# MDFahimAnjum/AliasFree-Diffusion-Models-PyTorch

Measured on AMD Instinct MI355X. Metric: train_step_images_per_sec, higher is better.
Workload: dtype f32; 1 GPU; CIFAR-10 32x32x3 synthetic, UNet variant=3 (Config D), batch 256/GPU, T=1000, AdamW lr 3e-4, random-init weights (seed 42); global_batch=256, parallelism=dp1, hip_graph=True, launch_mode=lanes

## Files before the change

### aliasfree-diffusion-models-pytorch_amd/csrc/tok.hip

```cpp
#include "tok_common.h"
#include "tok_h2.h"
#include <algorithm>
#include <cstdint>
#include <mutex>
#include <set>

namespace afd {

template <int KB>
__device__ __forceinline__ f32x16 t_block(const float* __restrict__ Ws, int nb, int l31, int half, const TT<KB>& z, f32x16 acc) {
  constexpr int WS = 32 * KB + 4;
  const float* __restrict__ wr = Ws + (nb * 32 + l31) * WS + 4 * half;
#pragma unroll
  for (int j = 0; j < KB; ++j)
#pragma unroll
    for (int q = 0; q < 4; ++q) {
      const float4 a = *reinterpret_cast<const float4*>(wr + 32 * j + 8 * q);
      acc = __builtin_amdgcn_mfma_f32_32x32x2f32(a.x, z.b[j][4 * q + 0], acc, 0, 0, 0);
      acc = __builtin_amdgcn_mfma_f32_32x32x2f32(a.y, z.b[j][4 * q + 1], acc, 0, 0, 0);
      acc = __builtin_amdgcn_mfma_f32_32x32x2f32(a.z, z.b[j][4 * q + 2], acc, 0, 0, 0);
      acc = __builtin_amdgcn_mfma_f32_32x32x2f32(a.w, z.b[j][4 * q + 3], acc, 0, 0, 0);
    }
  return acc;
}

template <int K>
__device__ __forceinline__ void stage_w(float* __restrict__ Ws, const float* __restrict__ w, int rows, int ldw, int n0, int k0,
                                        bool transposed) {
  constexpr int WS = K + 4;
  if (!transposed) {
    for (int i = threadIdx.x; i < rows * K; i += 256) {
      const int n = i / K, k = i - n * K;
      Ws[n * WS + k] = w[(long)(n0 + n) * ldw + k0 + k];
    }
  } else {
    for (int i = threadIdx.x; i < rows * K; i += 256) {
      const int n = i / K, k = i - n * K;
      Ws[n * WS + k] = w[(long)(k0 + k) * ldw + n0 + n];
    }
  }
}

template <int C>
__global__ __launch_bounds__(256) void tok_head_fwd(const float* __restrict__ x, const float* __restrict__ gamma,
                                                    const float* __restrict__ beta, const float* __restrict__ w,
                                                    const float* __restrict__ bias, float* __restrict__ h_out,
                                                    float* __restrict__ stats_out, float* __restrict__ y, int B, int N, int P,
                                                    float eps, int n_per_wg) {
  constexpr int KB = C / 32, WS = C + 4;
  extern __shared__ __attribute__((aligned(16))) float smem[];
  float* Ws = smem;
  float* bsm = Ws + n_per_wg * WS;
  float* gs = bsm + n_per_wg;
  float* bes = gs + C;
  const int nbase = blockIdx.y * n_per_wg;
  stage_w<C>(Ws, w, n_per_wg, C, nbase, 0, false);
  for (int i = threadIdx.x; i < n_per_wg; i += 256) bsm[i] = bias ? bias[nbase + i] : 0.f;
  for (int i = threadIdx.x; i < C; i += 256) { gs[i] = gamma[i]; bes[i] = beta[i]; }
  __syncthreads();

  const int lane = threadIdx.x & 63, wv = threadIdx.x >> 6, half = lane >> 5, l31 = lane & 31;
  const unsigned total = (unsigned)B * (unsigned)P;
  const int ntile = (int)((total + 31u) / 32u);
  const int tstride = gridDim.x * 4;
  const bool lead = blockIdx.y == 0;
  const int nblk = n_per_wg / 32;

  TT<KB> xc, xn;
  Pix pc, pn;
  int t = blockIdx.x * 4 + wv;
  if (t < ntile) { pc = pix_of(t, l31, total, P); t_load(xc, x, tbase(pc, C, P, half), P, pc.live); }
  for (; t < ntile; t += tstride) {
    const int tn = t + tstride;
    if (tn < ntile) { pn = pix_of(tn, l31, total, P); t_load(xn, x, tbase(pn, C, P, half), P, pn.live); }
    TT<KB> h;
    float mean, rstd;
    t_ln_fwd<KB>(xc, gs, bes, half, eps, h, mean, rstd);
    if (lead) {
      if (h_out) t_store(h, h_out, tbase(pc, C, P, half), P, pc.live);
      if (stats_out && pc.live && half == 0) { stats_out[2 * pc.f] = mean; stats_out[2 * pc.f + 1] = rstd; }
    }
    const unsigned yb = tbase(pc, N, P, half);
    for (int nb = 0; nb < nblk; ++nb) {
      const f32x16 acc = t_block<KB>(Ws, nb, l31, half, h, zero16());
      if (pc.live) {
#pragma unroll
        for (int r = 0; r < 16; ++r) {
          const int nl = nb * 32 + tch(0, r) + 4 * half;
          y[yb + (unsigned)(nbase + nb * 32 + tch(0, r)) * (unsigned)P] = acc[r] + bsm[nl];
        }
      }
    }
    xc = xn; pc = pn;
  }
}

template <int C> struct Chain {
  static constexpr int KB = C / 32, WS = C + 4, SLOT = C * WS;
  static constexpr bool RELOAD = C > 64;
  static constexpr int NSLOT = RELOAD ? 2 : 3;
};

template <int C, bool TRAIN>
__global__ __launch_bounds__(256) void tok_tail_fwd(const float* __restrict__ att, const float* __restrict__ xres,
                                                    const float* __restrict__ wo, const float* __restrict__ bo,
                                                    const float* __restrict__ gamma, const float* __restrict__ beta,
                                                    const float* __restrict__ w1, const float* __restrict__ b1,
                                                    const float* __restrict__ w2, const float* __restrict__ b2,
                                                    float* __restrict__ a_out, float* __restrict__ stats_out,
                                                    float* __restrict__ f_out, float* __restrict__ u_out, float* __restrict__ g_out,
                                                    float* __restrict__ out, int B, int P, float eps) {
  using CH = Chain<C>;
  constexpr int KB = CH::KB;
  extern __shared__ __attribute__((aligned(16))) float smem[];
  float* s0 = smem;
  float* s1 = smem + CH::SLOT;
  float* s2 = CH::RELOAD ? s0 : smem + 2 * CH::SLOT;
  float* vec = smem + CH::NSLOT * CH::SLOT;
  stage_w<C>(s0, wo, C, C, 0, 0, false);
  stage_w<C>(s1, w1, C, C, 0, 0, false);
  if (!CH::RELOAD) stage_w<C>(s2, w2, C, C, 0, 0, false);
  for (int i = threadIdx.x; i < C; i += 256) {
    vec[i] = bo[i]; vec[C + i] = gamma[i]; vec[2 * C + i] = beta[i]; vec[3 * C + i] = b1[i]; vec[4 * C + i] = b2[i];
  }
  __syncthreads();

  const int lane = threadIdx.x & 63, wv = threadIdx.x >> 6, half = lane >> 5, l31 = lane & 31;
  const unsigned total = (unsigned)B * (unsigned)P;
  const int ntile = (int)((total + 31u) / 32u);
  const int tstride = gridDim.x * 4;
  const int t0 = blockIdx.x * 4;
  const int npass = t0 < ntile ? (ntile - t0 + tstride - 1) / tstride : 0;
  for (int pass = 0; pass < npass; ++pass) {
    const int t = t0 + wv + pass * tstride;
    const bool active = t < ntile;
    if (CH::RELOAD && pass > 0) { __syncthreads(); stage_w<C>(s0, wo, C, C, 0, 0, false); __syncthreads(); }
    Pix pc = pix_of(active ? t : 0, l31, total, P);
    pc.live = pc.live && active;
    const unsigned base = tbase(pc, C, P, half);
    TT<KB> a, z;
    if (active) {
      TT<KB> xr;
      t_load(z, att, base, P, pc.live);
      t_load(xr, xres, base, P, pc.live);
#pragma unroll
      for (int nb = 0; nb < KB; ++nb) {
        const f32x16 acc = t_block<KB>(s0, nb, l31, half, z, zero16());
#pragma unroll
        for (int r = 0; r < 16; ++r) a.b[nb][r] = acc[r] + vec[nb * 32 + tch(0, r) + 4 * half] + xr.b[nb][r];
      }
      float mean, rstd;
      t_ln_fwd<KB>(a, vec + C, vec + 2 * C, half, eps, z, mean, rstd);
      if (TRAIN) {
        t_store(a, a_out, base, P, pc.live);
        t_store(z, f_out, base, P, pc.live);
        if (pc.live && half == 0) { stats_out[2 * pc.f] = mean; stats_out[2 * pc.f + 1] = rstd; }
      }
    }
    if (CH::RELOAD) { __syncthreads(); stage_w<C>(s0, w2, C, C, 0, 0, false); }
    TT<KB> g;
    if (active) {
#pragma unroll
      for (int nb = 0; nb < KB; ++nb) {
        const f32x16 acc = t_block<KB>(s1, nb, l31, half, z, zero16());
#pragma unroll
        for (int r = 0; r < 16; ++r) {
          const float u = acc[r] + vec[3 * C + nb * 32 + tch(0, r) + 4 * half];
          if (TRAIN && pc.live) u_out[base + (unsigned)tch(nb, r) * (unsigned)P] = u;
          g.b[nb][r] = gelu_erf(u);
        }
      }
      if (TRAIN) t_store(g, g_out, base, P, pc.live);
    }
    if (CH::RELOAD) __syncthreads();
    if (active) {
#pragma unroll
      for (int nb = 0; nb < KB; ++nb) {
        const f32x16 acc = t_block<KB>(s2, nb, l31, half, g, zero16());
        if (pc.live) {
#pragma unroll
          for (int r = 0; r < 16; ++r)
            out[base + (unsigned)tch(nb, r) * (unsigned)P] = acc[r] + vec[4 * C + nb * 32 + tch(0, r) + 4 * half] + a.b[nb][r];
        }
      }
    }
  }
}

template <int C>
__global__ __launch_bounds__(256) void tok_tail_bwd(const float* __restrict__ dout, const float* __restrict__ u_in,
                                                    const float* __restrict__ a_in, const float* __restrict__ stats,
                                                    const float* __restrict__ gamma, const float* __restrict__ w2,
                                                    const float* __restrict__ w1, const float* __restrict__ wo,
                                                    float* __restrict__ du_out, float* __restrict__ df_out,
                                                    float* __restrict__ da_out, float* __restrict__ datt_out, int B, int P) {
  using CH = Chain<C>;
  constexpr int KB = CH::KB;
  extern __shared__ __attribute__((aligned(16))) float smem[];
  float* s0 = smem;
  float* s1 = smem + CH::SLOT;
  float* s2 = CH::RELOAD ? s0 : smem + 2 * CH::SLOT;
  float* gs = smem + CH::NSLOT * CH::SLOT;
  stage_w<C>(s0, w2, C, C, 0, 0, true);
  stage_w<C>(s1, w1, C, C, 0, 0, true);
  if (!CH::RELOAD) stage_w<C>(s2, wo, C, C, 0, 0, true);
  for (int i = threadIdx.x; i < C; i += 256) gs[i] = gamma[i];
  __syncthreads();

  const int lane = threadIdx.x & 63, wv = threadIdx.x >> 6, half = lane >> 5, l31 = lane & 31;
  const unsigned total = (unsigned)B * (unsigned)P;
  const int ntile = (int)((total + 31u) / 32u);
  const int tstride = gridDim.x * 4;
  const int t0 = blockIdx.x * 4;
  const int npass = t0 < ntile ? (ntile - t0 + tstride - 1) / tstride : 0;
  for (int pass = 0; pass < npass; ++pass) {
    const int t = t0 + wv + pass * tstride;
    const bool active = t < ntile;
    if (CH::RELOAD && pass > 0) { __syncthreads(); stage_w<C>(s0, w2, C, C, 0, 0, true); __syncthreads(); }
    Pix pc = pix_of(active ? t : 0, l31, total, P);
    pc.live = pc.live && active;
    const unsigned base = tbase(pc, C, P, half);
    TT<KB> dy, z;
    if (active) {
      TT<KB> uu;
      t_load(dy, dout, base, P, pc.live);
      t_load(uu, u_in, base, P, pc.live);
#pragma unroll
      for (int nb = 0; nb < KB; ++nb) {
        const f32x16 acc = t_block<KB>(s0, nb, l31, half, dy, zero16());
#pragma unroll
        for (int r = 0; r < 16; ++r) z.b[nb][r] = acc[r] * gelu_erf_grad(uu.b[nb][r]);
      }
      t_store(z, du_out, base, P, pc.live);
    }
    if (CH::RELOAD) { __syncthreads(); stage_w<C>(s0, wo, C, C, 0, 0, true); }
    if (active) {
      TT<KB> df, aa;
      t_load(aa, a_in, base, P, pc.live);
#pragma unroll
      for (int nb = 0; nb < KB; ++nb) df.b[nb] = t_block<KB>(s1, nb, l31, half, z, zero16());
      t_store(df, df_out, base, P, pc.live);
      const float mean = pc.live ? stats[2 * pc.f] : 0.f, rstd = pc.live ? stats[2 * pc.f + 1] : 0.f;
      t_ln_bwd<KB>(df, aa, gs, half, mean, rstd, dy);
      t_store(df, da_out, base, P, pc.live);
      z = df;
    }
    if (CH::RELOAD) __syncthreads();
    if (active) {
#pragma unroll
      for (int nb = 0; nb < KB; ++nb) {
        const f32x16 acc = t_block<KB>(s2, nb, l31, half, z, zero16());
        if (pc.live) {
#pragma unroll
          for (int r = 0; r < 16; ++r) datt_out[base + (unsigned)tch(nb, r) * (unsigned)P] = acc[r];
        }
      }
    }
  }
}

template <int C>
__global__ __launch_bounds__(256) void tok_head_bwd(const float* __restrict__ dqkv, const float* __restrict__ x,
                                                    const float* __restrict__ stats, const float* __restrict__ gamma,
                                                    const float* __restrict__ w_in, const float* __restrict__ dres,
                                                    float* __restrict__ dh_out, float* __restrict__ dx_out, int B, int P) {
  using CH = Chain<C>;
  constexpr int KB = CH::KB;
  extern __shared__ __attribute__((aligned(16))) float smem[];
  float* s0 = smem;
  float* s1 = smem + CH::SLOT;
  float* s2 = CH::RELOAD ? s0 : smem + 2 * CH::SLOT;
  float* gs = smem + CH::NSLOT * CH::SLOT;
  stage_w<C>(s0, w_in, C, C, 0, 0, true);
  stage_w<C>(s1, w_in, C, C, 0, C, true);
  if (!CH::RELOAD) stage_w<C>(s2, w_in, C, C, 0, 2 * C, true);
  for (int i = threadIdx.x; i < C; i += 256) gs[i] = gamma[i];
  __syncthreads();

  const int lane = threadIdx.x & 63, wv = threadIdx.x >> 6, half = lane >> 5, l31 = lane & 31;
  const unsigned total = (unsigned)B * (unsigned)P;
  const int ntile = (int)((total + 31u) / 32u);
  const int tstride = gridDim.x * 4;
  const int t0 = blockIdx.x * 4;
  const int npass = t0 < ntile ? (ntile - t0 + tstride - 1) / tstride : 0;
  for (int pass = 0; pass < npass; ++pass) {
    const int t = t0 + wv + pass * tstride;
    const bool active = t < ntile;
    if (CH::RELOAD && pass > 0) { __syncthreads(); stage_w<C>(s0, w_in, C, C, 0, 0, true); __syncthreads(); }
    Pix pc = pix_of(active ? t : 0, l31, total, P);
    pc.live = pc.live && active;
    const unsigned base = tbase(pc, C, P, half);
    const unsigned qb = tbase(pc, 3 * C, P, half);
    TT<KB> dh, z;
    if (active) {
      t_load(z, dqkv, qb, P, pc.live);
#pragma unroll
      for (int nb = 0; nb < KB; ++nb) dh.b[nb] = t_block<KB>(s0, nb, l31, half, z, zero16());
    }
    if (CH::RELOAD) { __syncthreads(); stage_w<C>(s0, w_in, C, C, 0, 2 * C, true); }
    if (active) {
      t_load(z, dqkv, qb + (unsigned)C * (unsigned)P, P, pc.live);
#pragma unroll
      for (int nb = 0; nb < KB; ++nb) dh.b[nb] = t_block<KB>(s1, nb, l31, half, z, dh.b[nb]);
    }
// ... 58 lines not shown
#pragma unroll
    for (int r = 0; r < 16; ++r) z.b[j][r] = X[(tch(j, r) + 4 * half) * 32 + l31];
}
__device__ __forceinline__ f32x16 b_load(const float* __restrict__ src, unsigned base, unsigned P, bool live) {
  f32x16 v;
#pragma unroll
  for (int r = 0; r < 16; ++r) v[r] = live ? src[base + (unsigned)tch(0, r) * P] : 0.f;
  return v;
}
__device__ __forceinline__ void b_store(const f32x16& v, float* __restrict__ dst, unsigned base, unsigned P, bool live) {
  if (!live) return;
#pragma unroll
  for (int r = 0; r < 16; ++r) dst[base + (unsigned)tch(0, r) * P] = v[r];
}
template <int KB>
__device__ __forceinline__ void t_ln_stats(const TT<KB>& x, float eps, float& mean, float& rstd) {
  constexpr float invC = 1.0f / (32 * KB);
  float s = 0.f;
#pragma unroll
  for (int j = 0; j < KB; ++j)
#pragma unroll
    for (int r = 0; r < 16; ++r) s += x.b[j][r];
  s += __shfl_xor(s, 32, 64);
  mean = s * invC;
  float q = 0.f;
#pragma unroll
  for (int j = 0; j < KB; ++j)
#pragma unroll
    for (int r = 0; r < 16; ++r) { const float d = x.b[j][r] - mean; q = fmaf(d, d, q); }
  q += __shfl_xor(q, 32, 64);
  rstd = 1.0f / sqrtf(q * invC + eps);
}
template <int KB>
__device__ __forceinline__ void t_ln_bwd_core(TT<KB>& dy, const TT<KB>& x, const float* __restrict__ gs, int half, float mean,
                                              float rstd, float& m1, float& m2) {
  constexpr float invC = 1.0f / (32 * KB);
  float s1 = 0.f, s2 = 0.f;
#pragma unroll
  for (int j = 0; j < KB; ++j)
#pragma unroll
    for (int r = 0; r < 16; ++r) {
      const float gv = gs[tch(j, r) + 4 * half] * dy.b[j][r];
      const float xh = (x.b[j][r] - mean) * rstd;
      dy.b[j][r] = gv;
      s1 += gv;
      s2 = fmaf(gv, xh, s2);
    }
  s1 += __shfl_xor(s1, 32, 64);
  s2 += __shfl_xor(s2, 32, 64);
  m1 = s1 * invC; m2 = s2 * invC;
#pragma unroll
  for (int j = 0; j < KB; ++j)
#pragma unroll
    for (int r = 0; r < 16; ++r) {
      const float xh = (x.b[j][r] - mean) * rstd;
      dy.b[j][r] = rstd * (dy.b[j][r] - m1 - xh * m2);
    }
}

template <int C> struct Wide {
  static constexpr int KB = C / 32, NS = C / 32, TPW = 4 / NS;
};

template <int C, int NBW>
__global__ __launch_bounds__(256) void tok_head_fwd_wide(const float* __restrict__ x, const float* __restrict__ gamma,
                                                         const float* __restrict__ beta, const float* __restrict__ w,
                                                         const float* __restrict__ bias, float* __restrict__ h_out,
                                                         float* __restrict__ stats_out, float* __restrict__ y, int B, int P,
                                                         float eps) {
  constexpr int KB = C / 32, N = 3 * C, NGRP = N / 32 / NBW;
  __shared__ float vec[5 * C];
  for (int i = threadIdx.x; i < C; i += 256) { vec[i] = gamma[i]; vec[C + i] = beta[i]; }
  for (int i = threadIdx.x; i < N; i += 256) vec[2 * C + i] = bias ? bias[i] : 0.f;
  const int lane = threadIdx.x & 63, wv = threadIdx.x >> 6, half = lane >> 5, l31 = lane & 31;
  const unsigned total = (unsigned)B * (unsigned)P;
  const int ntile = (int)((total + 31u) / 32u);
  const long gw = (long)blockIdx.x * 4 + wv;
  const int tile = (int)(gw / NGRP), nb0 = (int)(gw - (long)tile * NGRP) * NBW;
  const bool active = tile < ntile;
  Pix pc = pix_of(active ? tile : 0, l31, total, P);
  pc.live = pc.live && active;
  TT<KB> xt, h;
  WA<KB> wa, wb;
  t_load(xt, x, tbase(pc, C, P, half), P, pc.live);
  wa_load(wa, w, nb0 * 32, C, 0, l31, half);
  __syncthreads();
  float mean, rstd;
  t_ln_fwd<KB>(xt, vec, vec + C, half, eps, h, mean, rstd);
  if (nb0 == 0) {
    if (h_out) t_store(h, h_out, tbase(pc, C, P, half), P, pc.live);
    if (stats_out && pc.live && half == 0) { stats_out[2 * pc.f] = mean; stats_out[2 * pc.f + 1] = rstd; }
  }
  const unsigned yb = tbase(pc, N, P, half);
#pragma unroll
  for (int i = 0; i < NBW; ++i) {
    const int nb = nb0 + i;
    if (i + 1 < NBW) wa_load((i & 1) ? wa : wb, w, (nb + 1) * 32, C, 0, l31, half);
    f32x16 acc = wa_block<KB>((i & 1) ? wb : wa, h, zero16());
#pragma unroll
    for (int r = 0; r < 16; ++r) acc[r] += vec[2 * C + nb * 32 + tch(0, r) + 4 * half];
    b_store(acc, y, yb + (unsigned)(nb * 32) * (unsigned)P, P, pc.live);
  }
}

template <int C, bool TRAIN>
__global__ __launch_bounds__(256) void tok_tail_fwd_wide(const float* __restrict__ att, const float* __restrict__ xres,
                                                         const float* __restrict__ wo, const float* __restrict__ bo,
                                                         const float* __restrict__ gamma, const float* __restrict__ beta,
                                                         const float* __restrict__ w1, const float* __restrict__ b1,
                                                         const float* __restrict__ w2, const float* __restrict__ b2,
                                                         float* __restrict__ a_out, float* __restrict__ stats_out,
                                                         float* __restrict__ f_out, float* __restrict__ u_out,
                                                         float* __restrict__ g_out, float* __restrict__ out, int B, int P, float eps) {
  using WD = Wide<C>;
  constexpr int KB = WD::KB;
  __shared__ float X[WD::TPW][C * 32];
  __shared__ float vec[5 * C];
  for (int i = threadIdx.x; i < C; i += 256) {
    vec[i] = bo[i]; vec[C + i] = gamma[i]; vec[2 * C + i] = beta[i]; vec[3 * C + i] = b1[i]; vec[4 * C + i] = b2[i];
  }
  const int lane = threadIdx.x & 63, wv = threadIdx.x >> 6, half = lane >> 5, l31 = lane & 31;
  const int ts = wv / WD::NS, nbk = wv % WD::NS;
  const unsigned total = (unsigned)B * (unsigned)P;
  const int ntile = (int)((total + 31u) / 32u);
  const int tile = blockIdx.x * WD::TPW + ts;
  const bool active = tile < ntile;
  Pix pc = pix_of(active ? tile : 0, l31, total, P);
  pc.live = pc.live && active;
  const unsigned base = tbase(pc, C, P, half), bb = base + (unsigned)(nbk * 32) * (unsigned)P;
  const int cb = nbk * 32 + 4 * half;
  float* Xt = X[ts];
  TT<KB> z;
  WA<KB> wa, wb;
  t_load(z, att, base, P, pc.live);
  const f32x16 xr = b_load(xres, bb, P, pc.live);
  wa_load(wa, wo, nbk * 32, C, 0, l31, half);
  __syncthreads();
  f32x16 ab = wa_block<KB>(wa, z, zero16());
  wa_load(wb, w1, nbk * 32, C, 0, l31, half);
#pragma unroll
  for (int r = 0; r < 16; ++r) ab[r] += vec[cb + tch(0, r)] + xr[r];
  x_put(Xt, nbk, l31, half, ab);
  if (TRAIN) b_store(ab, a_out, bb, P, pc.live);
  __syncthreads();
  x_get<KB>(Xt, l31, half, z);
  float mean, rstd;
  t_ln_stats<KB>(z, eps, mean, rstd);
#pragma unroll
  for (int j = 0; j < KB; ++j)
#pragma unroll
    for (int r = 0; r < 16; ++r) {
      const int c = tch(j, r) + 4 * half;
      z.b[j][r] = (z.b[j][r] - mean) * rstd * vec[C + c] + vec[2 * C + c];
    }
  if (TRAIN) {
    f32x16 fb;
#pragma unroll
    for (int r = 0; r < 16; ++r) fb[r] = (ab[r] - mean) * rstd * vec[C + cb + tch(0, r)] + vec[2 * C + cb + tch(0, r)];
    b_store(fb, f_out, bb, P, pc.live);
    if (nbk == 0 && pc.live && half == 0) { stats_out[2 * pc.f] = mean; stats_out[2 * pc.f + 1] = rstd; }
  }
  __syncthreads();
  f32x16 gb = wa_block<KB>(wb, z, zero16());
  wa_load(wa, w2, nbk * 32, C, 0, l31, half);
#pragma unroll
  for (int r = 0; r < 16; ++r) gb[r] += vec[3 * C + cb + tch(0, r)];
  if (TRAIN) b_store(gb, u_out, bb, P, pc.live);
#pragma unroll
  for (int r = 0; r < 16; ++r) gb[r] = gelu_erf(gb[r]);
  if (TRAIN) b_store(gb, g_out, bb, P, pc.live);
  x_put(Xt, nbk, l31, half, gb);
  __syncthreads();
  x_get<KB>(Xt, l31, half, z);
  f32x16 ob = wa_block<KB>(wa, z, zero16());
#pragma unroll
  for (int r = 0; r < 16; ++r) ob[r] += vec[4 * C + cb + tch(0, r)] + ab[r];
  b_store(ob, out, bb, P, pc.live);
}

template <int C>
__global__ __launch_bounds__(256) void tok_tail_bwd_wide(const float* __restrict__ dout, const float* __restrict__ u_in,
                                                         const float* __restrict__ a_in, const float* __restrict__ stats,
                                                         const float* __restrict__ gamma, const float* __restrict__ w2,
                                                         const float* __restrict__ w1, const float* __restrict__ wo,
                                                         float* __restrict__ du_out, float* __restrict__ df_out,
                                                         float* __restrict__ da_out, float* __restrict__ datt_out, int B, int P) {
  using WD = Wide<C>;
  constexpr int KB = WD::KB;
  __shared__ float X[WD::TPW][C * 32];
  __shared__ float gs[C];
  for (int i = threadIdx.x; i < C; i += 256) gs[i] = gamma[i];
  const int lane = threadIdx.x & 63, wv = threadIdx.x >> 6, half = lane >> 5, l31 = lane & 31;
  const int ts = wv / WD::NS, nbk = wv % WD::NS;
  const unsigned total = (unsigned)B * (unsigned)P;
  const int ntile = (int)((total + 31u) / 32u);
  const int tile = blockIdx.x * WD::TPW + ts;
  const bool active = tile < ntile;
  Pix pc = pix_of(active ? tile : 0, l31, total, P);
  pc.live = pc.live && active;
  const unsigned base = tbase(pc, C, P, half), bb = base + (unsigned)(nbk * 32) * (unsigned)P;
  const int cb = nbk * 32 + 4 * half;
  float* Xt = X[ts];
  TT<KB> z, aa;
  WA<KB> wa, wb;
  t_load(z, dout, base, P, pc.live);
  const f32x16 ub = b_load(u_in, bb, P, pc.live);
  wa_load_t(wa, w2, nbk * 32, C, 0, l31, half);
  f32x16 dub = wa_block<KB>(wa, z, zero16());
  wa_load_t(wb, w1, nbk * 32, C, 0, l31, half);
#pragma unroll
  for (int r = 0; r < 16; ++r) dub[r] *= gelu_erf_grad(ub[r]);
  b_store(dub, du_out, bb, P, pc.live);
  x_put(Xt, nbk, l31, half, dub);
  __syncthreads();
  x_get<KB>(Xt, l31, half, z);
  const f32x16 dfb = wa_block<KB>(wb, z, zero16());
  wa_load_t(wa, wo, nbk * 32, C, 0, l31, half);
  b_store(dfb, df_out, bb, P, pc.live);
  t_load(aa, a_in, base, P, pc.live);
  __syncthreads();
  x_put(Xt, nbk, l31, half, dfb);
  __syncthreads();
  x_get<KB>(Xt, l31, half, z);
  const float mean = pc.live ? stats[2 * pc.f] : 0.f, rstd = pc.live ? stats[2 * pc.f + 1] : 0.f;
  float m1, m2;
  t_ln_bwd_core<KB>(z, aa, gs, half, mean, rstd, m1, m2);
  t_load(aa, dout, base, P, pc.live);
#pragma unroll
  for (int j = 0; j < KB; ++j)
#pragma unroll
    for (int r = 0; r < 16; ++r) z.b[j][r] += aa.b[j][r];
  {
    const f32x16 ab = b_load(a_in, bb, P, pc.live), dob = b_load(dout, bb, P, pc.live);
    f32x16 dab;
#pragma unroll
    for (int r = 0; r < 16; ++r) {
      const float xh = (ab[r] - mean) * rstd;
      dab[r] = rstd * (gs[cb + tch(0, r)] * dfb[r] - m1 - xh * m2) + dob[r];
    }
    b_store(dab, da_out, bb, P, pc.live);
  }
  const f32x16 db = wa_block<KB>(wa, z, zero16());
  b_store(db, datt_out, bb, P, pc.live);
}

template <int C>
__global__ __launch_bounds__(256) void tok_head_bwd_wide(const float* __restrict__ dqkv, const float* __restrict__ x,
                                                         const float* __restrict__ stats, const float* __restrict__ gamma,
                                                         const float* __restrict__ w_in, const float* __restrict__ dres,
                                                         float* __restrict__ dh_out, float* __restrict__ dx_out, int B, int P) {
  using WD = Wide<C>;
  constexpr int KB = WD::KB;
  __shared__ float X[WD::TPW][C * 32];
  __shared__ float gs[C];
  for (int i = threadIdx.x; i < C; i += 256) gs[i] = gamma[i];
  const int lane = threadIdx.x & 63, wv = threadIdx.x >> 6, half = lane >> 5, l31 = lane & 31;
  const int ts = wv / WD::NS, nbk = wv % WD::NS;
  const unsigned total = (unsigned)B * (unsigned)P;
  const int ntile = (int)((total + 31u) / 32u);
  const int tile = blockIdx.x * WD::TPW + ts;
  const bool active = tile < ntile;
  Pix pc = pix_of(active ? tile : 0, l31, total, P);
  pc.live = pc.live && active;
  const unsigned base = tbase(pc, C, P, half), bb = base + (unsigned)(nbk * 32) * (unsigned)P;
  const unsigned qb = tbase(pc, 3 * C, P, half);
  const int cb = nbk * 32 + 4 * half;
  float* Xt = X[ts];
  TT<KB> z;
  WA<KB> wa;
  f32x16 dhb = zero16();
#pragma unroll
  for (int sct = 0; sct < 3; ++sct) {
    t_load(z, dqkv, qb + (unsigned)(sct * C) * (unsigned)P, P, pc.live);
    wa_load_t(wa, w_in, nbk * 32, C, sct * C, l31, half);
    dhb = wa_block<KB>(wa, z, dhb);
  }
  if (dh_out) b_store(dhb, dh_out, bb, P, pc.live);
  x_put(Xt, nbk, l31, half, dhb);
  TT<KB> xx;
  t_load(xx, x, base, P, pc.live);
  __syncthreads();
  x_get<KB>(Xt, l31, half, z);
  const float mean = pc.live ? stats[2 * pc.f] : 0.f, rstd = pc.live ? stats[2 * pc.f + 1] : 0.f;
  float m1, m2;
  t_ln_bwd_core<KB>(z, xx, gs, half, mean, rstd, m1, m2);
  const f32x16 xb = b_load(x, bb, P, pc.live), rb = b_load(dres, bb, P, pc.live);
  f32x16 dxb;
#pragma unroll
  for (int r = 0; r < 16; ++r) {
    const float xh = (xb[r] - mean) * rstd;
    dxb[r] = rstd * (gs[cb + tch(0, r)] * dhb[r] - m1 - xh * m2) + rb[r];
  }
  b_store(dxb, dx_out, bb, P, pc.live);
}

static bool tok_ok(int C) { return C == 32 || C == 64 || C == 128; }
static size_t chain_lds(int C, int nvec) {
  const int nslot = C > 64 ? 2 : 3;
  return sizeof(float) * ((size_t)nslot * C * (C + 4) + (size_t)nvec * C);
}
template <class K> static int set_lds(K kern, size_t lds) { return lds_opt_in(kern, lds); }
static int g_tok_max_wg = 0;
static int g_tok_path = 0;
static bool use_h2(int C, long ntile, int kern) {
  if (C != 64 && C != 128) return false;
  if (g_tok_path >= 4) return true;
  if (g_tok_path != 0) return false;
  if (C == 64) return ntile >= 1024 || (kern == 2 && ntile >= 512);
  return kern != 1 && ntile >= 512;
}
static bool use_wide(int C, long ntile) {
  if (C != 64 && C != 128) return false;
  if (g_tok_max_wg > 0 || g_tok_path == 1) return false;
  if (g_tok_path == 2) return true;
  return C == 128 || ntile < 1024;
}
static unsigned chain_grid(int C, long ntile) {
  const long wg = (ntile + 3) / 4;
  const long cap = g_tok_max_wg > 0 ? g_tok_max_wg : (C > 64 ? 8192 : 1024);
  return (unsigned)std::min<long>(wg, cap);
}

}

using namespace afd;

extern "C" {

int afd_tok_supported(int C) { return tok_ok(C) ? 1 : 0; }
int afd_debug_tok_grid(int max_workgroups) { g_tok_max_wg = max_workgroups; return AFD_OK; }
int afd_debug_tok_path(int mode) {
  AFD_REQUIRE(mode >= 0 && mode <= 6, "afd_debug_tok_path: mode %d not in 0..6", mode);
  g_tok_path = mode;
  tok_h2_debug_tpw(mode == 5 ? 2 : (mode == 6 ? 4 : 0));
  return AFD_OK;
}

int afd_tok_head_fwd(const float* x, const float* gamma, const float* beta, const float* w, const float* bias, float* h_out,
                     float* stats_out, float* qkv, int B, int C, int P, float eps, afd_stream_t st) {
  AFD_REQUIRE(x && gamma && beta && w && qkv && B > 0 && P > 0, "afd_tok_head_fwd: NULL pointer or empty shape");
  AFD_REQUIRE(tok_ok(C), "afd_tok_head_fwd: C=%d not covered (32, 64, 128)", C);
  AFD_REQUIRE((long)B * P * 3 * C < (1L << 31), "afd_tok_head_fwd: tensor too large for 32-bit offsets");
  const int N = 3 * C;
  const long ntile = ((long)B * P + 31) / 32, wg_tiles = (ntile + 3) / 4;
  if (use_h2(C, ntile, 0)) return tok_h2_head_fwd(x, gamma, beta, w, bias, h_out, stats_out, qkv, B, C, P, eps, g_tok_max_wg, as_stream(st));
  if (use_wide(C, ntile) && aligned16(w) && (ntile <= 256 || g_tok_path == 2)) {
    const long waves = ntile * (N / 32);
    const dim3 wgrid((unsigned)((waves + 3) / 4));
    hipStream_t s = as_stream(st);
    if (C == 64) hipLaunchKernelGGL((tok_head_fwd_wide<64, 1>), wgrid, dim3(256), 0, s, x, gamma, beta, w, bias, h_out, stats_out, qkv, B, P, eps);
    else         hipLaunchKernelGGL((tok_head_fwd_wide<128, 1>), wgrid, dim3(256), 0, s, x, gamma, beta, w, bias, h_out, stats_out, qkv, B, P, eps);
    return check_launch("afd_tok_head_fwd");
  }
  int npw = 32;
  for (int cand : {N, 192, 128, 96, 64, 32}) {
    if (cand > N || N % cand != 0) continue;
    if (sizeof(float) * ((size_t)cand * (C + 5) + 2 * C) > 64 * 1024) continue;
    npw = cand;
    if (wg_tiles * (N / cand) >= 256) break;
  }
  const size_t lds = sizeof(float) * ((size_t)npw * (C + 5) + 2 * C);
  const dim3 grid((unsigned)std::min<long>(wg_tiles, g_tok_max_wg > 0 ? g_tok_max_wg : 1024), (unsigned)(N / npw));
  hipStream_t s = as_stream(st);
  switch (C) {
    case 32:  hipLaunchKernelGGL(tok_head_fwd<32>, grid, dim3(256), lds, s, x, gamma, beta, w, bias, h_out, stats_out, qkv, B, N, P, eps, npw); break;
    case 64:  hipLaunchKernelGGL(tok_head_fwd<64>, grid, dim3(256), lds, s, x, gamma, beta, w, bias, h_out, stats_out, qkv, B, N, P, eps, npw); break;
    default:  hipLaunchKernelGGL(tok_head_fwd<128>, grid, dim3(256), lds, s, x, gamma, beta, w, bias, h_out, stats_out, qkv, B, N, P, eps, npw); break;
  }
  return check_launch("afd_tok_head_fwd");
}

int afd_tok_tail_fwd(const float* att, const float* x, const float* wo, const float* bo, const float* gamma, const float* beta,
                     const float* w1, const float* b1, const float* w2, const float* b2, float* a_out, float* stats_out,
                     float* f_out, float* u_out, float* g_out, float* out, int B, int C, int P, float eps, afd_stream_t st) {
  AFD_REQUIRE(att && x && wo && bo && gamma && beta && w1 && b1 && w2 && b2 && out && B > 0 && P > 0,
              "afd_tok_tail_fwd: NULL pointer or empty shape");
  AFD_REQUIRE(tok_ok(C), "afd_tok_tail_fwd: C=%d not covered (32, 64, 128)", C);
  AFD_REQUIRE((long)B * P * C < (1L << 31), "afd_tok_tail_fwd: tensor too large for 32-bit offsets");
  const bool train = a_out != nullptr;
  AFD_REQUIRE(!train || (stats_out && f_out && u_out && g_out), "afd_tok_tail_fwd: a_out given but a saved-tensor pointer is NULL");
  const long ntile = ((long)B * P + 31) / 32;
  hipStream_t s = as_stream(st);
  if (use_h2(C, ntile, 1))
    return tok_h2_tail_fwd(att, x, wo, bo, gamma, beta, w1, b1, w2, b2, a_out, stats_out, f_out, u_out, g_out, out, B, C, P, eps, g_tok_max_wg, s);
  if (use_wide(C, ntile) && aligned16(wo) && aligned16(w1) && aligned16(w2)) {
    const dim3 wgrid((unsigned)((ntile + Wide<64>::TPW - 1) / Wide<64>::TPW)), wgrid128((unsigned)ntile);
#define AFD_TAILW(C_, T_, G_) hipLaunchKernelGGL((tok_tail_fwd_wide<C_, T_>), G_, dim3(256), 0, s, att, x, wo, bo, gamma, beta, w1, b1, w2, b2, \
                                                  a_out, stats_out, f_out, u_out, g_out, out, B, P, eps)
    if (C == 64) { if (train) AFD_TAILW(64, true, wgrid); else AFD_TAILW(64, false, wgrid); }
    else         { if (train) AFD_TAILW(128, true, wgrid128); else AFD_TAILW(128, false, wgrid128); }
#undef AFD_TAILW
    return check_launch("afd_tok_tail_fwd");
  }
  const size_t lds = chain_lds(C, 5);
  const dim3 grid(chain_grid(C, ntile));
#define AFD_TAIL(C_, T_) do { if (int rc = set_lds(tok_tail_fwd<C_, T_>, lds)) return rc; \
    hipLaunchKernelGGL((tok_tail_fwd<C_, T_>), grid, dim3(256), lds, s, att, x, wo, bo, gamma, beta, w1, b1, w2, b2, a_out, stats_out, \
                       f_out, u_out, g_out, out, B, P, eps); } while (0)
  switch (C) {
    case 32:  if (train) AFD_TAIL(32, true); else AFD_TAIL(32, false); break;
    case 64:  if (train) AFD_TAIL(64, true); else AFD_TAIL(64, false); break;
    default:  if (train) AFD_TAIL(128, true); else AFD_TAIL(128, false); break;
  }
#undef AFD_TAIL
  return check_launch("afd_tok_tail_fwd");
}

int afd_tok_tail_bwd(const float* d_out, const float* u, const float* a, const float* stats, const float* gamma, const float* w2,
                     const float* w1, const float* wo, float* du_out, float* df_out, float* da_out, float* datt_out, int B, int C,
                     int P, afd_stream_t st) {
  AFD_REQUIRE(d_out && u && a && stats && gamma && w2 && w1 && wo && du_out && df_out && da_out && datt_out && B > 0 && P > 0,
              "afd_tok_tail_bwd: NULL pointer or empty shape");
  AFD_REQUIRE(tok_ok(C), "afd_tok_tail_bwd: C=%d not covered (32, 64, 128)", C);
  AFD_REQUIRE((long)B * P * C < (1L << 31), "afd_tok_tail_bwd: tensor too large for 32-bit offsets");
  const long ntile = ((long)B * P + 31) / 32;
  hipStream_t s = as_stream(st);
  if (use_h2(C, ntile, 2)) return tok_h2_tail_bwd(d_out, u, a, stats, gamma, w2, w1, wo, du_out, df_out, da_out, datt_out, B, C, P, g_tok_max_wg, s);
  if (use_wide(C, ntile)) {
    if (C == 64) hipLaunchKernelGGL(tok_tail_bwd_wide<64>, dim3((unsigned)((ntile + 1) / 2)), dim3(256), 0, s, d_out, u, a, stats, gamma, w2, w1, wo, du_out, df_out, da_out, datt_out, B, P);
    else         hipLaunchKernelGGL(tok_tail_bwd_wide<128>, dim3((unsigned)ntile), dim3(256), 0, s, d_out, u, a, stats, gamma, w2, w1, wo, du_out, df_out, da_out, datt_out, B, P);
    return check_launch("afd_tok_tail_bwd");
  }
  const size_t lds = chain_lds(C, 1);
  const dim3 grid(chain_grid(C, ntile));
#define AFD_TB(C_) do { if (int rc = set_lds(tok_tail_bwd<C_>, lds)) return rc; \
    hipLaunchKernelGGL(tok_tail_bwd<C_>, grid, dim3(256), lds, s, d_out, u, a, stats, gamma, w2, w1, wo, du_out, df_out, da_out, datt_out, B, P); } while (0)
  switch (C) { case 32: AFD_TB(32); break; case 64: AFD_TB(64); break; default: AFD_TB(128); break; }
#undef AFD_TB
  return check_launch("afd_tok_tail_bwd");
}

int afd_tok_head_bwd(const float* dqkv, const float* x, const float* stats, const float* gamma, const float* w_in,
                     const float* d_res, float* dh_out, float* dx_out, int B, int C, int P, afd_stream_t st) {
  AFD_REQUIRE(dqkv && x && stats && gamma && w_in && d_res && dx_out && B > 0 && P > 0, "afd_tok_head_bwd: NULL pointer or empty shape");
  AFD_REQUIRE(tok_ok(C), "afd_tok_head_bwd: C=%d not covered (32, 64, 128)", C);
  AFD_REQUIRE((long)B * P * 3 * C < (1L << 31), "afd_tok_head_bwd: tensor too large for 32-bit offsets");
  const long ntile = ((long)B * P + 31) / 32;
  hipStream_t s = as_stream(st);
  if (use_h2(C, ntile, 3)) return tok_h2_head_bwd(dqkv, x, stats, gamma, w_in, d_res, dh_out, dx_out, B, C, P, g_tok_max_wg, s);
  if (use_wide(C, ntile)) {
    if (C == 64) hipLaunchKernelGGL(tok_head_bwd_wide<64>, dim3((unsigned)((ntile + 1) / 2)), dim3(256), 0, s, dqkv, x, stats, gamma, w_in, d_res, dh_out, dx_out, B, P);
    else         hipLaunchKernelGGL(tok_head_bwd_wide<128>, dim3((unsigned)ntile), dim3(256), 0, s, dqkv, x, stats, gamma, w_in, d_res, dh_out, dx_out, B, P);
    return check_launch("afd_tok_head_bwd");
  }
  const size_t lds = chain_lds(C, 1);
  const dim3 grid(chain_grid(C, ntile));
#define AFD_HB(C_) do { if (int rc = set_lds(tok_head_bwd<C_>, lds)) return rc; \
    hipLaunchKernelGGL(tok_head_bwd<C_>, grid, dim3(256), lds, s, dqkv, x, stats, gamma, w_in, d_res, dh_out, dx_out, B, P); } while (0)
  switch (C) { case 32: AFD_HB(32); break; case 64: AFD_HB(64); break; default: AFD_HB(128); break; }
#undef AFD_HB
  return check_launch("afd_tok_head_bwd");
}

}
```

### aliasfree-diffusion-models-pytorch_amd/csrc/tok_h2.h

```cpp
#pragma once
#include "common.h"

namespace afd {

int tok_h2_head_fwd(const float* x, const float* gamma, const float* beta, const float* w, const float* bias, float* h_out,
                    float* stats_out, float* qkv, int B, int C, int P, float eps, int max_wg, hipStream_t s);
int tok_h2_tail_fwd(const float* att, const float* x, const float* wo, const float* bo, const float* gamma, const float* beta,
                    const float* w1, const float* b1, const float* w2, const float* b2, float* a_out, float* stats_out,
                    float* f_out, float* u_out, float* g_out, float* out, int B, int C, int P, float eps, int max_wg, hipStream_t s);
int tok_h2_tail_bwd(const float* d_out, const float* u, const float* a, const float* stats, const float* gamma, const float* w2,
                    const float* w1, const float* wo, float* du_out, float* df_out, float* da_out, float* datt_out, int B, int C,
                    int P, int max_wg, hipStream_t s);
int tok_h2_head_bwd(const float* dqkv, const float* x, const float* stats, const float* gamma, const float* w_in,
                    const float* d_res, float* dh_out, float* dx_out, int B, int C, int P, int max_wg, hipStream_t s);
void tok_h2_debug_tpw(int tpw);

}
```

### aliasfree-diffusion-models-pytorch_amd/csrc/tok_h2.hip

```cpp
#include "tok_common.h"
#include "h2_common.h"
#include "tok_h2.h"
#include <algorithm>

namespace afd {

template <int NB>
__device__ __forceinline__ void h_load(TT<NB>& z, const float* __restrict__ src, unsigned base, int P) {
#pragma unroll
  for (int j = 0; j < NB; ++j)
#pragma unroll
    for (int r = 0; r < 16; ++r) z.b[j][r] = (src + (size_t)tch(j, r) * P)[base];
}
template <int NB>
__device__ __forceinline__ void h_store(const TT<NB>& z, float* __restrict__ dst, unsigned base, int P, bool live) {
  if (!live) return;
#pragma unroll
  for (int j = 0; j < NB; ++j)
#pragma unroll
    for (int r = 0; r < 16; ++r) (dst + (size_t)tch(j, r) * P)[base] = z.b[j][r];
}

template <int KB> struct HP { h8 a[2 * KB], b[2 * KB]; };

template <int KB>
__device__ __forceinline__ float hp_split(const TT<KB>& z, HP<KB>& p) {
  float m = 0.f;
#pragma unroll
  for (int j = 0; j < KB; ++j)
#pragma unroll
    for (int r = 0; r < 16; ++r) m = fmaxf(m, fabsf(z.b[j][r]));
  m = fmaxf(m, __shfl_xor(m, 32, 64));
  const float s = h2_scale_for(m);
#pragma unroll
  for (int k = 0; k < 2 * KB; ++k) {
    float x[8];
#pragma unroll
    for (int e = 0; e < 8; ++e) x[e] = z.b[k >> 1][8 * (k & 1) + e];
    h2_split8(x, s, p.a[k], p.b[k]);
  }
  return h2_inv_pow2(s);
}

template <int KB>
__device__ __forceinline__ f32x16 hp_block(const h8* __restrict__ img, int nb, int l31, int half, const HP<KB>& z) {
  constexpr int C = 32 * KB, NG = C / 8;
  const h8* __restrict__ w0 = img + half * C + nb * 32 + l31;
  const h8* __restrict__ w1 = w0 + NG * C;
  f32x16 acc = zero16();
#pragma unroll
  for (int k = 0; k < 2 * KB; ++k) {
    const h8 a1 = w0[2 * k * C], a2 = w1[2 * k * C];
    acc = __builtin_amdgcn_mfma_f32_32x32x16_f16(a2, z.a[k], acc, 0, 0, 0);
    acc = __builtin_amdgcn_mfma_f32_32x32x16_f16(a1, z.b[k], acc, 0, 0, 0);
    acc = __builtin_amdgcn_mfma_f32_32x32x16_f16(a1, z.a[k], acc, 0, 0, 0);
  }
  return acc;
}

template <int C> struct H2Lds {
  static constexpr int NG = C / 8, REC = 2 * NG * C;
  static constexpr bool RELOAD = C > 64;
  static constexpr int NSLOT = RELOAD ? 2 : 3;
  h8* img[3];
  float* winv[3];
  unsigned* rmax[3];
  float* vec;
  __device__ __forceinline__ void init(unsigned char* base) {
    h8* i0 = reinterpret_cast<h8*>(base);
    float* w0 = reinterpret_cast<float*>(i0 + NSLOT * REC);
    unsigned* r0 = reinterpret_cast<unsigned*>(w0 + NSLOT * C);
#pragma unroll
    for (int m = 0; m < 3; ++m) {
      const int s = m % NSLOT;
      img[m] = i0 + s * REC; winv[m] = w0 + s * C; rmax[m] = r0 + s * C;
    }
    vec = reinterpret_cast<float*>(r0 + NSLOT * C);
  }
  static size_t bytes(int nvec) { return (size_t)NSLOT * REC * 16 + (size_t)NSLOT * C * 8 + (size_t)nvec * C * 4; }
};

struct WSrc { const float* w; int ldw, n0, k0; };

template <int C, int NT> struct Stg {
  static constexpr int NG = C / 8, NR = C * NG / NT;
  float x[NR][8];
  static __device__ __forceinline__ void rec(int r, bool transposed, int& n, int& G) {
    const int i = (int)threadIdx.x + r * NT;
    if (transposed) { n = i % C; G = i / C; }
    else {
      const int lo = i & 63, hi = i >> 6;
      n = (hi % (C / 8)) * 8 + (lo & 7);
      G = (hi / (C / 8)) * 8 + (lo >> 3);
    }
  }
  __device__ __forceinline__ void load(const WSrc& q, bool transposed) {
#pragma unroll
    for (int r = 0; r < NR; ++r) {
      int n, G;
      rec(r, transposed, n, G);
      const int kb = 16 * (G >> 1) + 4 * (G & 1);
#pragma unroll
      for (int e = 0; e < 8; ++e) {
        const int k = kb + 8 * (e >> 2) + (e & 3);
        x[r][e] = transposed ? q.w[(long)(q.k0 + k) * q.ldw + q.n0 + n] : q.w[(long)(q.n0 + n) * q.ldw + q.k0 + k];
      }
    }
  }
  __device__ __forceinline__ void maxima(unsigned* __restrict__ rmax, bool transposed) const {
#pragma unroll
    for (int r = 0; r < NR; ++r) {
      int n, G;
      rec(r, transposed, n, G);
      float m = 0.f;
#pragma unroll
      for (int e = 0; e < 8; ++e) m = fmaxf(m, fabsf(x[r][e]));
      atomicMax(&rmax[n], __float_as_uint(m));
    }
  }
  __device__ __forceinline__ void store(h8* __restrict__ img, float* __restrict__ winv, const unsigned* __restrict__ rmax,
                                        bool transposed) const {
#pragma unroll
    for (int r = 0; r < NR; ++r) {
      int n, G;
      rec(r, transposed, n, G);
      const float sc = h2_scale_for(__uint_as_float(rmax[n]));
      h8 p0, p1;
      h2_split8(x[r], sc, p0, p1);
      img[G * C + n] = p0;
      img[(NG + G) * C + n] = p1;
      if (G == 0) winv[n] = h2_inv_pow2(sc);
    }
  }
};

template <int C, int NT, int M0, int CNT>
__device__ __forceinline__ void h2_stage(const H2Lds<C>& L, const WSrc* src, bool transposed) {
  Stg<C, NT> st[CNT];
#pragma unroll
  for (int i = 0; i < CNT; ++i) st[i].load(src[i], transposed);
#pragma unroll
  for (int i = 0; i < CNT; ++i)
    for (int c = threadIdx.x; c < C; c += NT) L.rmax[M0 + i][c] = 0u;
  __syncthreads();
#pragma unroll
  for (int i = 0; i < CNT; ++i) st[i].maxima(L.rmax[M0 + i], transposed);
  __syncthreads();
#pragma unroll
  for (int i = 0; i < CNT; ++i) st[i].store(L.img[M0 + i], L.winv[M0 + i], L.rmax[M0 + i], transposed);
  __builtin_amdgcn_sched_barrier(0);
}
template <int C, int NT>
__device__ __forceinline__ void h2_stage_first(const H2Lds<C>& L, const WSrc* src, bool transposed) {
  if (H2Lds<C>::RELOAD) h2_stage<C, NT, 0, 2>(L, src, transposed);
  else h2_stage<C, NT, 0, 3>(L, src, transposed);
}
template <int C, int NT, int M>
__device__ __forceinline__ void h2_stage_one(const H2Lds<C>& L, const WSrc* src, bool transposed) {
  h2_stage<C, NT, M, 1>(L, src + M, transposed);
}

struct Walk { int lane, wv, half, l31, ntile, tstride, t0, npass; unsigned total; };
template <int TPW> __device__ __forceinline__ Walk walk_of(int B, int P) {
  Walk k;
  k.lane = threadIdx.x & 63; k.wv = threadIdx.x >> 6; k.half = k.lane >> 5; k.l31 = k.lane & 31;
  k.total = (unsigned)B * (unsigned)P;
  k.ntile = (int)((k.total + 31u) / 32u);
  k.tstride = gridDim.x * TPW;
  k.t0 = blockIdx.x * TPW;
  k.npass = k.t0 < k.ntile ? (k.ntile - k.t0 + k.tstride - 1) / k.tstride : 0;
  return k;
}

extern __shared__ __attribute__((aligned(16))) unsigned char h2_smem[];

template <int C, int TPW>
__global__ __launch_bounds__(64 * TPW) void tok_h2_head_fwd_k(const float* __restrict__ x, const float* __restrict__ gamma,
                                                               const float* __restrict__ beta, const float* __restrict__ w,
                                                               const float* __restrict__ bias, float* __restrict__ h_out,
                                                               float* __restrict__ stats_out, float* __restrict__ y, int B, int P,
                                                               float eps) {
  using LD = H2Lds<C>;
  constexpr int KB = C / 32, NT = 64 * TPW;
  LD L;
  L.init(h2_smem);
  float* vec = L.vec;
  const Walk k = walk_of<TPW>(B, P);
  const int half = k.half, l31 = k.l31;
  const WSrc src[3] = {{w, C, 0, 0}, {w, C, C, 0}, {w, C, 2 * C, 0}};
  h2_stage_first<C, NT>(L, src, false);
  for (int i = threadIdx.x; i < C; i += NT) { vec[i] = gamma[i]; vec[C + i] = beta[i]; }
  for (int i = threadIdx.x; i < 3 * C; i += NT) vec[2 * C + i] = bias ? bias[i] : 0.f;
  __syncthreads();
  for (int pass = 0; pass < k.npass; ++pass) {
    const int t = k.t0 + k.wv + pass * k.tstride;
    const bool active = t < k.ntile;
    if (LD::RELOAD && pass > 0) { __syncthreads(); h2_stage_one<C, NT, 0>(L, src, false); __syncthreads(); }
    Pix pc = pix_of(active ? t : 0, l31, k.total, P);
    pc.live = pc.live && active;
    const unsigned yb = tbase(pc, 3 * C, P, half);
    HP<KB> hp;
    float is = 0.f;
    if (active) {
      const unsigned base = tbase(pc, C, P, half);
      TT<KB> xc, h;
      h_load(xc, x, base, P);
      float mean, rstd;
      t_ln_fwd<KB>(xc, vec, vec + C, half, eps, h, mean, rstd);
      if (h_out) h_store(h, h_out, base, P, pc.live);
      if (stats_out && pc.live && half == 0) { stats_out[2 * pc.f] = mean; stats_out[2 * pc.f + 1] = rstd; }
      is = hp_split<KB>(h, hp);
    }
#pragma unroll
    for (int sl = 0; sl < 3; ++sl) {
      if (LD::RELOAD && sl == 1) { __syncthreads(); h2_stage_one<C, NT, 2>(L, src, false); }
      if (LD::RELOAD && sl == 2) __syncthreads();
      if (active) {
#pragma unroll
        for (int nb = 0; nb < KB; ++nb) {
          const f32x16 acc = hp_block<KB>(L.img[sl], nb, l31, half, hp);
          if (pc.live) {
#pragma unroll
            for (int r = 0; r < 16; ++r) {
              const int c = nb * 32 + tch(0, r) + 4 * half;
              (y + (size_t)(sl * C + nb * 32 + tch(0, r)) * P)[yb] = acc[r] * is * L.winv[sl][c] + vec[2 * C + sl * C + c];
            }
          }
        }
      }
    }
  }
}

template <int C, int TPW, bool TRAIN>
__global__ __launch_bounds__(64 * TPW) void tok_h2_tail_fwd_k(const float* __restrict__ att, const float* __restrict__ xres,
                                                               const float* __restrict__ wo, const float* __restrict__ bo,
                                                               const float* __restrict__ gamma, const float* __restrict__ beta,
                                                               const float* __restrict__ w1, const float* __restrict__ b1,
                                                               const float* __restrict__ w2, const float* __restrict__ b2,
                                                               float* __restrict__ a_out, float* __restrict__ stats_out,
                                                               float* __restrict__ f_out, float* __restrict__ u_out,
                                                               float* __restrict__ g_out, float* __restrict__ out, int B, int P,
                                                               float eps) {
  using LD = H2Lds<C>;
  constexpr int KB = C / 32, NT = 64 * TPW;
  LD L;
  L.init(h2_smem);
  float* vec = L.vec;
  const Walk k = walk_of<TPW>(B, P);
  const int half = k.half, l31 = k.l31;
  const WSrc src[3] = {{wo, C, 0, 0}, {w1, C, 0, 0}, {w2, C, 0, 0}};
  h2_stage_first<C, NT>(L, src, false);
  for (int i = threadIdx.x; i < C; i += NT) {
    vec[i] = bo[i]; vec[C + i] = gamma[i]; vec[2 * C + i] = beta[i]; vec[3 * C + i] = b1[i]; vec[4 * C + i] = b2[i];
  }
  __syncthreads();
  for (int pass = 0; pass < k.npass; ++pass) {
    const int t = k.t0 + k.wv + pass * k.tstride;
    const bool active = t < k.ntile;
    if (LD::RELOAD && pass > 0) { __syncthreads(); h2_stage_one<C, NT, 0>(L, src, false); __syncthreads(); }
    Pix pc = pix_of(active ? t : 0, l31, k.total, P);
    pc.live = pc.live && active;
    const unsigned base = tbase(pc, C, P, half);
    TT<KB> a;
    HP<KB> hp;
    float is = 0.f;
    if (active) {
      TT<KB> z, xr;
      h_load(z, att, base, P);
      h_load(xr, xres, base, P);
      is = hp_split<KB>(z, hp);
#pragma unroll
      for (int nb = 0; nb < KB; ++nb) {
        const f32x16 acc = hp_block<KB>(L.img[0], nb, l31, half, hp);
#pragma unroll
        for (int r = 0; r < 16; ++r) {
          const int c = nb * 32 + tch(0, r) + 4 * half;
          a.b[nb][r] = acc[r] * is * L.winv[0][c] + vec[c] + xr.b[nb][r];
        }
      }
      float mean, rstd;
      t_ln_fwd<KB>(a, vec + C, vec + 2 * C, half, eps, z, mean, rstd);
      if (TRAIN) {
        h_store(a, a_out, base, P, pc.live);
        h_store(z, f_out, base, P, pc.live);
        if (pc.live && half == 0) { stats_out[2 * pc.f] = mean; stats_out[2 * pc.f + 1] = rstd; }
      }
      is = hp_split<KB>(z, hp);
    }
    if (LD::RELOAD) { __syncthreads(); h2_stage_one<C, NT, 2>(L, src, false); }
    if (active) {
      TT<KB> g;
#pragma unroll
      for (int nb = 0; nb < KB; ++nb) {
        const f32x16 acc = hp_block<KB>(L.img[1], nb, l31, half, hp);
        TT<1> ub;
#pragma unroll
        for (int r = 0; r < 16; ++r) {
          const int c = nb * 32 + tch(0, r) + 4 * half;
          ub.b[0][r] = acc[r] * is * L.winv[1][c] + vec[3 * C + c];
          g.b[nb][r] = gelu_erf(ub.b[0][r]);
        }
        if (TRAIN) h_store(ub, u_out + (size_t)(32 * nb) * P, base, P, pc.live);
      }
      if (TRAIN) h_store(g, g_out, base, P, pc.live);
      is = hp_split<KB>(g, hp);
    }
    if (LD::RELOAD) __syncthreads();
    if (active) {
#pragma unroll
      for (int nb = 0; nb < KB; ++nb) {
        TT<1> ar;
        if (TRAIN && KB > 2) h_load(ar, a_out + (size_t)(32 * nb) * P, base, P);
        else ar.b[0] = a.b[nb];
        const f32x16 acc = hp_block<KB>(L.img[2], nb, l31, half, hp);
        if (pc.live) {
#pragma unroll
          for (int r = 0; r < 16; ++r) {
            const int c = nb * 32 + tch(0, r) + 4 * half;
            (out + (size_t)tch(nb, r) * P)[base] = acc[r] * is * L.winv[2][c] + vec[4 * C + c] + ar.b[0][r];
          }
        }
      }
    }
  }
}

template <int C, int TPW>
__global__ __launch_bounds__(64 * TPW) void tok_h2_tail_bwd_k(const float* __restrict__ dout, const float* __restrict__ u_in,
                                                               const float* __restrict__ a_in, const float* __restrict__ stats,
                                                               const float* __restrict__ gamma, const float* __restrict__ w2,
                                                               const float* __restrict__ w1, const float* __restrict__ wo,
                                                               float* __restrict__ du_out, float* __restrict__ df_out,
                                                               float* __restrict__ da_out, float* __restrict__ datt_out, int B,
                                                               int P) {
  using LD = H2Lds<C>;
  constexpr int KB = C / 32, NT = 64 * TPW;
  LD L;
  L.init(h2_smem);
  float* gs = L.vec;
  const Walk k = walk_of<TPW>(B, P);
  const int half = k.half, l31 = k.l31;
  const WSrc src[3] = {{w2, C, 0, 0}, {w1, C, 0, 0}, {wo, C, 0, 0}};
  h2_stage_first<C, NT>(L, src, true);
  for (int i = threadIdx.x; i < C; i += NT) gs[i] = gamma[i];
  __syncthreads();
  for (int pass = 0; pass < k.npass; ++pass) {
    const int t = k.t0 + k.wv + pass * k.tstride;
    const bool active = t < k.ntile;
    if (LD::RELOAD && pass > 0) { __syncthreads(); h2_stage_one<C, NT, 0>(L, src, true); __syncthreads(); }
    Pix pc = pix_of(active ? t : 0, l31, k.total, P);
    pc.live = pc.live && active;
    const unsigned base = tbase(pc, C, P, half);
    HP<KB> hp;
    float is = 0.f;
    if (active) {
      TT<KB> z, uu;
      h_load(z, dout, base, P);
      h_load(uu, u_in, base, P);
      is = hp_split<KB>(z, hp);
#pragma unroll
      for (int nb = 0; nb < KB; ++nb) {
        const f32x16 acc = hp_block<KB>(L.img[0], nb, l31, half, hp);
#pragma unroll
        for (int r = 0; r < 16; ++r)
          z.b[nb][r] = acc[r] * is * L.winv[0][nb * 32 + tch(0, r) + 4 * half] * gelu_erf_grad(uu.b[nb][r]);
      }
      h_store(z, du_out, base, P, pc.live);
      is = hp_split<KB>(z, hp);
    }
    if (LD::RELOAD) { __syncthreads(); h2_stage_one<C, NT, 2>(L, src, true); }
    if (active) {
      TT<KB> df, aa, dd;
#pragma unroll
      for (int nb = 0; nb < KB; ++nb) {
        const f32x16 acc = hp_block<KB>(L.img[1], nb, l31, half, hp);
#pragma unroll
        for (int r = 0; r < 16; ++r) df.b[nb][r] = acc[r] * is * L.winv[1][nb * 32 + tch(0, r) + 4 * half];
      }
      h_store(df, df_out, base, P, pc.live);
      h_load(dd, dout, base, P);
      h_load(aa, a_in, base, P);
      const float mean = pc.live ? stats[2 * pc.f] : 0.f, rstd = pc.live ? stats[2 * pc.f + 1] : 0.f;
      t_ln_bwd<KB>(df, aa, gs, half, mean, rstd, dd);
      h_store(df, da_out, base, P, pc.live);
      is = hp_split<KB>(df, hp);
    }
    if (LD::RELOAD) __syncthreads();
    if (active) {
#pragma unroll
      for (int nb = 0; nb < KB; ++nb) {
        const f32x16 acc = hp_block<KB>(L.img[2], nb, l31, half, hp);
        if (pc.live) {
#pragma unroll
          for (int r = 0; r < 16; ++r)
            (datt_out + (size_t)tch(nb, r) * P)[base] = acc[r] * is * L.winv[2][nb * 32 + tch(0, r) + 4 * half];
        }
      }
    }
  }
}

template <int C, int TPW>
__global__ __launch_bounds__(64 * TPW) void tok_h2_head_bwd_k(const float* __restrict__ dqkv, const float* __restrict__ x,
                                                               const float* __restrict__ stats, const float* __restrict__ gamma,
                                                               const float* __restrict__ w_in, const float* __restrict__ dres,
                                                               float* __restrict__ dh_out, float* __restrict__ dx_out, int B,
                                                               int P) {
  using LD = H2Lds<C>;
  constexpr int KB = C / 32, NT = 64 * TPW;
  LD L;
  L.init(h2_smem);
  float* gs = L.vec;
  const Walk k = walk_of<TPW>(B, P);
  const int half = k.half, l31 = k.l31;
  const WSrc src[3] = {{w_in, C, 0, 0}, {w_in, C, 0, C}, {w_in, C, 0, 2 * C}};
  h2_stage_first<C, NT>(L, src, true);
  for (int i = threadIdx.x; i < C; i += NT) gs[i] = gamma[i];
  __syncthreads();
  for (int pass = 0; pass < k.npass; ++pass) {
    const int t = k.t0 + k.wv + pass * k.tstride;
    const bool active = t < k.ntile;
    if (LD::RELOAD && pass > 0) { __syncthreads(); h2_stage_one<C, NT, 0>(L, src, true); __syncthreads(); }
    Pix pc = pix_of(active ? t : 0, l31, k.total, P);
    pc.live = pc.live && active;
    const unsigned base = tbase(pc, C, P, half);
    const unsigned qb = tbase(pc, 3 * C, P, half);
    TT<KB> dh;
#pragma unroll
    for (int sl = 0; sl < 3; ++sl) {
      if (LD::RELOAD && sl == 1) { __syncthreads(); h2_stage_one<C, NT, 2>(L, src, true); }
      if (LD::RELOAD && sl == 2) __syncthreads();
      if (active) {
        TT<KB> z;
        HP<KB> hp;
        h_load(z, dqkv + (size_t)(sl * C) * P, qb, P);
        const float is = hp_split<KB>(z, hp);
#pragma unroll
        for (int nb = 0; nb < KB; ++nb) {
          const f32x16 acc = hp_block<KB>(L.img[sl], nb, l31, half, hp);
#pragma unroll
          for (int r = 0; r < 16; ++r) {
            const float v = acc[r] * is * L.winv[sl][nb * 32 + tch(0, r) + 4 * half];
            dh.b[nb][r] = sl == 0 ? v : dh.b[nb][r] + v;
          }
        }
      }
    }
    if (active) {
      if (dh_out) h_store(dh, dh_out, base, P, pc.live);
      TT<KB> xx, rr;
      h_load(xx, x, base, P);
      h_load(rr, dres, base, P);
      const float mean = pc.live ? stats[2 * pc.f] : 0.f, rstd = pc.live ? stats[2 * pc.f + 1] : 0.f;
      t_ln_bwd<KB>(dh, xx, gs, half, mean, rstd, rr);
      h_store(dh, dx_out, base, P, pc.live);
    }
  }
}

static int g_h2_tpw = 0;
void tok_h2_debug_tpw(int tpw) { g_h2_tpw = tpw; }
static int h2_tpw(long ntile) { (void)ntile; return g_h2_tpw ? g_h2_tpw : 4; }
static unsigned h2_grid(int C, long ntile, int tpw, int max_wg) {
  const long wg = (ntile + tpw - 1) / tpw;
  const long cap = max_wg > 0 ? max_wg : (C > 64 ? 256 : 768);
  return (unsigned)std::min<long>(wg, cap);
}

#define AFD_H2_LAUNCH(KERN, NVEC, ...)                                                                              \
  do {                                                                                                              \
    const size_t lds = H2Lds<KC>::bytes(NVEC);                                                                      \
    if (int rc = lds_opt_in(KERN, lds)) return rc;                                                                  \
    hipLaunchKernelGGL(KERN, dim3(h2_grid(KC, ntile, KT, max_wg)), dim3(64 * KT), lds, s, __VA_ARGS__);             \
  } while (0)
#define AFD_H2_SWITCH(BODY)                                                                                         \
  do {                                                                                                              \
    if (C == 64) { constexpr int KC = 64; if (tpw == 4) { constexpr int KT = 4; BODY; } else { constexpr int KT = 2; BODY; } } \
    else         { constexpr int KC = 128; constexpr int KT = 4; BODY; }                                             \
  } while (0)

int tok_h2_head_fwd(const float* x, const float* gamma, const float* beta, const float* w, const float* bias, float* h_out,
                    float* stats_out, float* qkv, int B, int C, int P, float eps, int max_wg, hipStream_t s) {
  const long ntile = ((long)B * P + 31) / 32;
  const int tpw = h2_tpw(ntile);
  AFD_H2_SWITCH(AFD_H2_LAUNCH((tok_h2_head_fwd_k<KC, KT>), 5, x, gamma, beta, w, bias, h_out, stats_out, qkv, B, P, eps));
  return check_launch("afd_tok_head_fwd");
}

int tok_h2_tail_fwd(const float* att, const float* x, const float* wo, const float* bo, const float* gamma, const float* beta,
                    const float* w1, const float* b1, const float* w2, const float* b2, float* a_out, float* stats_out,
                    float* f_out, float* u_out, float* g_out, float* out, int B, int C, int P, float eps, int max_wg, hipStream_t s) {
  const long ntile = ((long)B * P + 31) / 32;
  const int tpw = h2_tpw(ntile);
  if (a_out)
    AFD_H2_SWITCH(AFD_H2_LAUNCH((tok_h2_tail_fwd_k<KC, KT, true>), 5, att, x, wo, bo, gamma, beta, w1, b1, w2, b2, a_out, stats_out,
                                f_out, u_out, g_out, out, B, P, eps));
  else
    AFD_H2_SWITCH(AFD_H2_LAUNCH((tok_h2_tail_fwd_k<KC, KT, false>), 5, att, x, wo, bo, gamma, beta, w1, b1, w2, b2, a_out, stats_out,
                                f_out, u_out, g_out, out, B, P, eps));
  return check_launch("afd_tok_tail_fwd");
}

int tok_h2_tail_bwd(const float* d_out, const float* u, const float* a, const float* stats, const float* gamma, const float* w2,
                    const float* w1, const float* wo, float* du_out, float* df_out, float* da_out, float* datt_out, int B, int C,
                    int P, int max_wg, hipStream_t s) {
  const long ntile = ((long)B * P + 31) / 32;
  const int tpw = h2_tpw(ntile);
  AFD_H2_SWITCH(AFD_H2_LAUNCH((tok_h2_tail_bwd_k<KC, KT>), 1, d_out, u, a, stats, gamma, w2, w1, wo, du_out, df_out, da_out, datt_out,
                              B, P));
  return check_launch("afd_tok_tail_bwd");
}

int tok_h2_head_bwd(const float* dqkv, const float* x, const float* stats, const float* gamma, const float* w_in,
                    const float* d_res, float* dh_out, float* dx_out, int B, int C, int P, int max_wg, hipStream_t s) {
  const long ntile = ((long)B * P + 31) / 32;
  const int tpw = h2_tpw(ntile);
  AFD_H2_SWITCH(AFD_H2_LAUNCH((tok_h2_head_bwd_k<KC, KT>), 1, dqkv, x, stats, gamma, w_in, d_res, dh_out, dx_out, B, P));
  return check_launch("afd_tok_head_bwd");
}

#undef AFD_H2_SWITCH
#undef AFD_H2_LAUNCH

}
```

### aliasfree-diffusion-models-pytorch_amd/csrc/wino.hip

```cpp
#include <cstdlib>
#include "conv_forms.h"
#include "bf3_weights.h"
#include "h2_common.h"

namespace afd {

using f32x4 = __attribute__((ext_vector_type(4))) float;
using f32x2 = __attribute__((ext_vector_type(2))) float;

template <int S, int NT> struct WGeo {
  static constexpr int W = S, TPR = S / 2, TPI = TPR * TPR;
  static constexpr int TI = NT <= TPI ? 1 : NT / TPI;
  static constexpr int TROWS = NT <= TPI ? NT / TPR : TPR;
  static constexpr int GPI = NT <= TPI ? TPI / NT : 1;
  static constexpr int PXR = 2 * TROWS, Wp = S + 2, IMG = (PXR + 2) * Wp, RS = TI * IMG;
  static constexpr int RSP = RS + ((32 - RS % 64) + 64) % 64;
  static_assert(NT % TPR == 0 && (NT <= TPI ? TPI % NT == 0 : NT % TPI == 0), "tile group must be whole tile rows or whole images");
};

template <int OFF0, int OFF1>
__device__ __forceinline__ void lds_issue_pair(f32x2& a, f32x2& b, unsigned base) {
  asm volatile("ds_read_b64 %0, %2 offset:%3\n\tds_read_b64 %1, %2 offset:%4" : "=&v"(a), "=&v"(b) : "v"(base), "n"(OFF0), "n"(OFF1));
}
template <int N>
__device__ __forceinline__ void lds_wait(f32x2& a, f32x2& b) {
  asm volatile("s_waitcnt lgkmcnt(%2)" : "+v"(a), "+v"(b) : "n"(N));
}

__device__ __forceinline__ int kperm8(int k) { return 2 * (k & 3) + (k >> 2); }

__device__ __forceinline__ void wino_weights_block(const float* __restrict__ w, float* __restrict__ Uf, float* __restrict__ Ud,
                                                   int Cin, int Cout, int blk, int lane) {
  const int nci8 = Cin >> 3;
  if (blk >= nci8 * (Cout >> 3)) return;
  const int ci = (blk % nci8) * 8 + (lane & 7), co = (blk / nci8) * 8 + (lane >> 3);
  const float* p = w + ((long)co * Cin + ci) * 9;
  float g[9];
#pragma unroll
  for (int t = 0; t < 9; ++t) g[t] = p[t];
  float t[4][3], u[16];
#pragma unroll
  for (int c = 0; c < 3; ++c) {
    const float g0 = g[c], g1 = g[3 + c], g2 = g[6 + c];
    t[0][c] = g0;
    t[1][c] = 0.5f * (g0 + g1 + g2);
    t[2][c] = 0.5f * (g0 - g1 + g2);
    t[3][c] = g2;
  }
#pragma unroll
  for (int i = 0; i < 4; ++i) {
    const float a = t[i][0], b = t[i][1], c = t[i][2];
    u[4 * i + 0] = a;
    u[4 * i + 1] = 0.5f * (a + b + c);
    u[4 * i + 2] = 0.5f * (a - b + c);
    u[4 * i + 3] = c;
  }
  if (Uf) {
    float* o = Uf + ((long)(ci >> 3) * 16 * Cout + co) * 8 + kperm8(ci & 7);
    const long xs = (long)Cout * 8;
#pragma unroll
    for (int xi = 0; xi < 16; ++xi) o[xi * xs] = u[xi];
  }
  if (Ud) {
    float* o = Ud + ((long)(co >> 3) * 16 * Cin + ci) * 8 + kperm8(co & 7);
    const long xs = (long)Cin * 8;
#pragma unroll
    for (int i = 0; i < 4; ++i)
#pragma unroll
      for (int j = 0; j < 4; ++j) {
        const int pi = i == 0 ? 3 : (i == 3 ? 0 : i), pj = j == 0 ? 3 : (j == 3 ? 0 : j);
        o[(4 * i + j) * xs] = u[4 * pi + pj];
      }
  }
}

__global__ __launch_bounds__(256) void wino_weights(const float* __restrict__ w, float* __restrict__ Uf, float* __restrict__ Ud,
                                                    int Cin, int Cout) {
  wino_weights_block(w, Uf, Ud, Cin, Cout, blockIdx.x * 4 + (threadIdx.x >> 6), threadIdx.x & 63);
}


__global__ __launch_bounds__(256) void wino_weights_batched(const afd_wino_desc* __restrict__ descs, const int* __restrict__ wg_desc) {
  const afd_wino_desc d = descs[wg_desc[blockIdx.x]];
  const int blk = (blockIdx.x - d.first_wg) * 4 + (threadIdx.x >> 6), lane = threadIdx.x & 63;
  float* wf = (d.kinds & 1) ? nullptr : d.u_fwd; float* wd = (d.kinds & 2) ? nullptr : d.u_dgrad;
  if (wf || wd) wino_weights_block(d.w, wf, wd, d.Cin, d.Cout, blk, lane);
  void* bf = (d.kinds & 1) ? d.u_fwd : nullptr; void* bd = (d.kinds & 2) ? d.u_dgrad : nullptr;
  if (bf || bd) {
    if (d.kinds & 4) bf3_weights_block(d.w, static_cast<__bf16*>(bf), static_cast<__bf16*>(bd), d.Cin, d.Cout, blk, lane);
    else h2_weights_block(d.w, bf, bd, d.Cin, d.Cout, blk, lane);
  }
}
__global__ __launch_bounds__(256) void h2_wscale_batched(const afd_wino_desc* __restrict__ descs, const int* __restrict__ wg_desc) {
  const afd_wino_desc d = descs[wg_desc[blockIdx.x]];
  if (d.kinds & 4) return;
  void* bf = (d.kinds & 1) ? d.u_fwd : nullptr; void* bd = (d.kinds & 2) ? d.u_dgrad : nullptr;
  const int nw = 4 * ((d.Cin * d.Cout / 64 + 3) / 4);
  if (bf || bd) h2_wscale_rows(d.w, bf, bd, d.Cin, d.Cout, (blockIdx.x - d.first_wg) * 4 + (threadIdx.x >> 6), nw, threadIdx.x & 63);
}

template <int GEO, int BN, int NT>
__global__ __launch_bounds__(BN * NT / 8, BN * NT == 4096 ? 1 : 2) void conv_wino(const float* __restrict__ x, const float* __restrict__ U,
                                                    const float* __restrict__ bias, const float* __restrict__ res,
                                                    float* __restrict__ y, int B, int K, int N, int act, int items) {
  using G = WGeo<GEO, NT>;
  constexpr int KC = 8, SU = 10, NTH = BN * NT / 8;
  constexpr int W = G::W, H = G::W, HW = W * W, Wp = G::Wp, IMG = G::IMG, RS = G::RS, RSP = G::RSP;
  constexpr int NPOS = (RS + NTH - 1) / NTH;
  constexpr int NUV = 16 * BN * 2 / NTH;
  extern __shared__ __attribute__((aligned(16))) float smem[];
  constexpr int BUF = 16 * BN * SU + KC * RSP;
  float* Us = smem;
  float* Rs = Us + 16 * BN * SU;
  const int tid = threadIdx.x, lane = tid & 63, wv = tid >> 6;
  const int NB = N / BN;

  unsigned rsrc[NPOS]; unsigned rvalid = 0; unsigned usrc0 = 0;
  constexpr int XSTEP = NTH / (2 * BN);
  static_assert(NTH % (2 * BN) == 0 && XSTEP * NUV == 16, "U chunk must split into whole xi planes per pass");
  const int u_h = tid & 1, u_n = (tid >> 1) % BN, u_xi = tid / (2 * BN);
  const int udst0 = (((u_n >> 4) * 16 + u_xi) * 16 + (u_n & 15)) * SU + 4 * u_h;
  const long ustep = (long)XSTEP * N * 8;
  auto plan = [&](int w) {
    const int tg = w / NB, n0 = (w % NB) * BN;
    const int b0 = (G::TI == 1) ? tg / G::GPI : tg * G::TI;
    const int row0 = (G::TI == 1) ? (tg % G::GPI) * G::PXR : 0;
    rvalid = 0;
#pragma unroll
    for (int e = 0; e < NPOS; ++e) {
      const int pos = tid + NTH * e;
      bool ok = false; unsigned src = 0;
      if (pos < RS) {
        const int ti = pos / IMG, rem = pos % IMG;
        const int yy = row0 + rem / Wp - 1, xx = rem % Wp - 1, b = b0 + ti;
        ok = b < B && yy >= 0 && yy < H && xx >= 0 && xx < W;
        if (ok) src = (unsigned)(b * K) * (unsigned)HW + (unsigned)(yy * W + xx);
      }
      rsrc[e] = src; rvalid |= (ok ? 1u : 0u) << e;
    }
    usrc0 = (unsigned)((u_xi * N + n0 + u_n) * 8 + 4 * u_h);
  };
  const int wn = wv % (BN / 32), wt = wv / (BN / 32);
  const int li = lane & 15, lq = lane >> 4;
  const int tt = wt * 16 + li;
  const int poff = (tt / (G::TROWS * G::TPR)) * IMG + 2 * ((tt / G::TPR) % G::TROWS) * Wp + 2 * (tt % G::TPR);

  struct Regs { float r[NPOS][KC]; f32x4 u[NUV]; unsigned ok; };
  Regs S0, S1;
  auto fetch = [&](Regs& S, int c) {
    const float* __restrict__ xk = x + (long)c * KC * HW;
    const float* __restrict__ uk = U + (long)c * 16 * N * 8;
#pragma unroll
    for (int e = 0; e < NUV; ++e) S.u[e] = *reinterpret_cast<const f32x4*>(uk + e * ustep + usrc0);
#pragma unroll
    for (int e = 0; e < NPOS; ++e)
      if (tid + NTH * e < RS) {
#pragma unroll
        for (int kc = 0; kc < KC; ++kc) S.r[e][kc] = (xk + kc * HW)[rsrc[e]];
      }
    S.ok = rvalid;
  };
  auto commit = [&](const Regs& S, int stage) {
    float* Us = smem + stage * BUF;
    float* Rs = Us + 16 * BN * SU;
#pragma unroll
    for (int e = 0; e < NUV; ++e) {
      float2* d = reinterpret_cast<float2*>(Us + udst0 + e * (XSTEP * 16 * SU));
      d[0] = make_float2(S.u[e][0], S.u[e][1]);
      d[1] = make_float2(S.u[e][2], S.u[e][3]);
    }
#pragma unroll
    for (int e = 0; e < NPOS; ++e)
      if (tid + NTH * e < RS) {
        const bool ok = (S.ok >> e) & 1u;
#pragma unroll
        for (int kc = 0; kc < KC; ++kc) Rs[kc * RSP + tid + NTH * e] = ok ? S.r[e][kc] : 0.f;
      }
  };
  auto patch = [&](const float* Rs, int k, float (&v)[16]) {
    const float* r = Rs + k * RSP + poff;
    float d[4][4];
#pragma unroll
    for (int a = 0; a < 4; ++a) {
      const float2 lo = *reinterpret_cast<const float2*>(r + a * Wp);
      const float2 hi = *reinterpret_cast<const float2*>(r + a * Wp + 2);
      d[a][0] = lo.x; d[a][1] = lo.y; d[a][2] = hi.x; d[a][3] = hi.y;
    }
    float w[4][4];
#pragma unroll
    for (int j = 0; j < 4; ++j) {
      w[0][j] = d[0][j] - d[2][j];
      w[1][j] = d[1][j] + d[2][j];
      w[2][j] = d[2][j] - d[1][j];
      w[3][j] = d[1][j] - d[3][j];
    }
#pragma unroll
    for (int i = 0; i < 4; ++i) {
      v[4 * i + 0] = w[i][0] - w[i][2];
      v[4 * i + 1] = w[i][1] + w[i][2];
      v[4 * i + 2] = w[i][2] - w[i][1];
      v[4 * i + 3] = w[i][1] - w[i][3];
    }
  };
  const unsigned ap = (unsigned)(size_t)(Us + (wn * 2 * 256 + li) * SU + 2 * lq);
  const int o_ti = tt / (G::TROWS * G::TPR), o_ty = (tt / G::TPR) % G::TROWS, o_tx = tt % G::TPR;
  const int nchunks = K / KC;

  for (int w = blockIdx.x; w < items; w += gridDim.x) {
    plan(w);
    fetch(S0, 0);
    if (nchunks > 1) fetch(S1, 1);
    f32x4 acc[16][2];
#pragma unroll
    for (int xi = 0; xi < 16; ++xi)
#pragma unroll
      for (int h = 0; h < 2; ++h) acc[xi][h] = f32x4{0.f, 0.f, 0.f, 0.f};

    auto multiply = [&](int st) {
      const float* Rc = Rs + st * BUF;
      const unsigned apc = ap + (unsigned)(st * BUF * 4);
      f32x2 alo[2], ahi[2];
      lds_issue_pair<0, 256 * SU * 4>(alo[0], ahi[0], apc);
      float v0[16], v1[16];
      patch(Rc, lq, v0);
      patch(Rc, lq + 4, v1);
#pragma unroll
      for (int xi = 0; xi < 16; ++xi) {
        constexpr int STEP = 16 * SU * 4;
        f32x2& lo = alo[xi & 1]; f32x2& hi = ahi[xi & 1];
        if (xi < 15) {
          switch (xi) {
#define AFD_NEXT(X) case X: lds_issue_pair<(X + 1) * STEP, (X + 1) * STEP + 256 * SU * 4>(alo[(X + 1) & 1], ahi[(X + 1) & 1], apc); break;
            AFD_NEXT(0) AFD_NEXT(1) AFD_NEXT(2) AFD_NEXT(3) AFD_NEXT(4) AFD_NEXT(5) AFD_NEXT(6) AFD_NEXT(7)
            AFD_NEXT(8) AFD_NEXT(9) AFD_NEXT(10) AFD_NEXT(11) AFD_NEXT(12) AFD_NEXT(13) AFD_NEXT(14)
#undef AFD_NEXT
          }
          lds_wait<2>(lo, hi);
        } else {
          lds_wait<0>(lo, hi);
        }
        acc[xi][0] = __builtin_amdgcn_mfma_f32_16x16x4f32(lo[0], v0[xi], acc[xi][0], 0, 0, 0);
        acc[xi][1] = __builtin_amdgcn_mfma_f32_16x16x4f32(hi[0], v0[xi], acc[xi][1], 0, 0, 0);
        acc[xi][0] = __builtin_amdgcn_mfma_f32_16x16x4f32(lo[1], v1[xi], acc[xi][0], 0, 0, 0);
        acc[xi][1] = __builtin_amdgcn_mfma_f32_16x16x4f32(hi[1], v1[xi], acc[xi][1], 0, 0, 0);
      }
    };

    __syncthreads();
    commit(S0, 0);
    if (nchunks > 2) fetch(S0, 2);
    __syncthreads();
    for (int c = 0; c < nchunks; c += 2) {
      multiply(0);
      if (c + 1 < nchunks) {
        commit(S1, 1);
        if (c + 3 < nchunks) fetch(S1, c + 3);
        __syncthreads();
        multiply(1);
        if (c + 2 < nchunks) {
          commit(S0, 0);
          if (c + 4 < nchunks) fetch(S0, c + 4);
          __syncthreads();
        }
      }
    }

    const int tg = w / NB, n0 = (w % NB) * BN;
    const int ob = ((G::TI == 1) ? tg / G::GPI : tg * G::TI) + o_ti;
    const int row0 = (G::TI == 1) ? (tg % G::GPI) * G::PXR : 0;
    if (ob < B) {
      const int opix = (row0 + 2 * o_ty) * W + 2 * o_tx;
#pragma unroll
      for (int h = 0; h < 2; ++h)
#pragma unroll
        for (int r = 0; r < 4; ++r) {
          const int n = n0 + wn * 32 + 16 * h + 4 * lq + r;
          float tcol[4][2];
#pragma unroll
          for (int i = 0; i < 4; ++i) {
            const float m0 = acc[4 * i + 0][h][r], m1 = acc[4 * i + 1][h][r], m2 = acc[4 * i + 2][h][r], m3 = acc[4 * i + 3][h][r];
            tcol[i][0] = (m0 + m1) + m2;
            tcol[i][1] = (m1 - m2) - m3;
          }
          float y00 = (tcol[0][0] + tcol[1][0]) + tcol[2][0], y01 = (tcol[0][1] + tcol[1][1]) + tcol[2][1];
          float y10 = (tcol[1][0] - tcol[2][0]) - tcol[3][0], y11 = (tcol[1][1] - tcol[2][1]) - tcol[3][1];
          const unsigned idx = (unsigned)((ob * N + n) * HW + opix);
          if (bias) { const float bb = bias[n]; y00 += bb; y01 += bb; y10 += bb; y11 += bb; }
          if (act == 1) { y00 = gelu_erf(y00); y01 = gelu_erf(y01); y10 = gelu_erf(y10); y11 = gelu_erf(y11); }
          if (res) {
            const float2 r0 = *reinterpret_cast<const float2*>(res + idx), r1 = *reinterpret_cast<const float2*>(res + idx + W);
            y00 += r0.x; y01 += r0.y; y10 += r1.x; y11 += r1.y;
          }
          *reinterpret_cast<float2*>(y + idx) = make_float2(y00, y01);
          *reinterpret_cast<float2*>(y + idx + W) = make_float2(y10, y11);
        }
    }
  }
}

template <int S>
__global__ __launch_bounds__(256, 2) void conv_wino_sk(const float* __restrict__ x, const float* __restrict__ U,
                                                       const float* __restrict__ bias, const float* __restrict__ res,
                                                       float* __restrict__ y, int B, int K, int N, int act) {
  using G = WGeo<S, 16>;
  static_assert(G::GPI == 1, "tile groups must be whole images");
  constexpr int KC = 8, W = S, HW = S * S, Wp = G::Wp, IMG = G::IMG, RS = G::RS, RSP = G::RSP, TI = G::TI;
  constexpr int UPC = TI * S * (S / 4);
  static_assert(UPC == 16, "one chunk = 128 float4 pieces per wave");
  constexpr int DEPTH = 8;
  extern __shared__ __attribute__((aligned(16))) float smem[];
  const int lane = threadIdx.x & 63, wv = threadIdx.x >> 6;
  float* Rs = smem + wv * (KC * RSP);
  float* red = smem + 4 * KC * RSP;
  const int n0 = blockIdx.x * 32, tg = blockIdx.y, b0 = tg * TI;
  const int li = lane & 15, lq = lane >> 4;
  const int poff = (li / (G::TROWS * G::TPR)) * IMG + 2 * ((li / G::TPR) % G::TROWS) * Wp + 2 * (li % G::TPR);
  const int KS = K / 4, nchunks = KS / KC, kw = wv * KS;

  for (int i = lane; i < KC * RSP; i += 64) Rs[i] = 0.f;

  unsigned rsrc[2]; int rdst[2]; bool rok[2];
#pragma unroll
  for (int e = 0; e < 2; ++e) {
    const int u = lane + 64 * e, ch = u / UPC, q = u % UPC;
    const int ti = q / (S * (S / 4)), rr = (q / (S / 4)) % S, x4 = q % (S / 4);
    rok[e] = b0 + ti < B;
    rsrc[e] = rok[e] ? (unsigned)(((b0 + ti) * K + kw + ch) * HW + rr * W + 4 * x4) : 0u;
    rdst[e] = ch * RSP + ti * IMG + (rr + 1) * Wp + 1 + 4 * x4;
  }
  f32x4 rreg[2];
  auto fetch = [&](int c) {
    const float* xk = x + (long)c * KC * HW;
#pragma unroll
    for (int e = 0; e < 2; ++e) rreg[e] = *reinterpret_cast<const f32x4*>(xk + rsrc[e]);
  };
  auto commit = [&]() {
#pragma unroll
    for (int e = 0; e < 2; ++e) {
      float* d = Rs + rdst[e];
      const bool ok = rok[e];
      d[0] = ok ? rreg[e][0] : 0.f; d[1] = ok ? rreg[e][1] : 0.f; d[2] = ok ? rreg[e][2] : 0.f; d[3] = ok ? rreg[e][3] : 0.f;
    }
  };
  auto patch = [&](int k, float (&v)[16]) {
    const float* r = Rs + k * RSP + poff;
    float d[4][4];
#pragma unroll
    for (int a = 0; a < 4; ++a) {
      const float2 lo = *reinterpret_cast<const float2*>(r + a * Wp);
      const float2 hi = *reinterpret_cast<const float2*>(r + a * Wp + 2);
      d[a][0] = lo.x; d[a][1] = lo.y; d[a][2] = hi.x; d[a][3] = hi.y;
    }
    float w[4][4];
#pragma unroll
    for (int j = 0; j < 4; ++j) {
      w[0][j] = d[0][j] - d[2][j];
      w[1][j] = d[1][j] + d[2][j];
      w[2][j] = d[2][j] - d[1][j];
      w[3][j] = d[1][j] - d[3][j];
    }
#pragma unroll
    for (int i = 0; i < 4; ++i) {
      v[4 * i + 0] = w[i][0] - w[i][2];
      v[4 * i + 1] = w[i][1] + w[i][2];
      v[4 * i + 2] = w[i][2] - w[i][1];
      v[4 * i + 3] = w[i][1] - w[i][3];
    }
  };
  const float* ua = U + ((long)(kw / KC) * 16 * N + n0 + li) * 8 + 2 * lq;
  const long xstep = (long)N * 8;
  const int total = nchunks * 16;
  f32x2 abuf[DEPTH][2];
  auto aload = [&](int g, int slot) {
    const float* p = ua + (long)g * xstep;
    abuf[slot][0] = *reinterpret_cast<const f32x2*>(p);
    abuf[slot][1] = *reinterpret_cast<const f32x2*>(p + 128);
  };

  f32x4 acc[16][2];
#pragma unroll
  for (int xi = 0; xi < 16; ++xi)
#pragma unroll
    for (int h = 0; h < 2; ++h) acc[xi][h] = f32x4{0.f, 0.f, 0.f, 0.f};

#pragma unroll
  for (int g = 0; g < DEPTH; ++g) aload(g, g);
  fetch(0);
  for (int c = 0; c < nchunks; ++c) {
    commit();
    if (c + 1 < nchunks) fetch(c + 1);
    float v0[16], v1[16];
    patch(lq, v0);
    patch(lq + 4, v1);
#pragma unroll
    for (int xi = 0; xi < 16; ++xi) {
      const f32x2 lo = abuf[xi % DEPTH][0], hi = abuf[xi % DEPTH][1];
      const int gn = c * 16 + xi + DEPTH;
      if (gn < total) aload(gn, xi % DEPTH);
      __builtin_amdgcn_sched_barrier(0);
      acc[xi][0] = __builtin_amdgcn_mfma_f32_16x16x4f32(lo[0], v0[xi], acc[xi][0], 0, 0, 0);
// ... 371 lines not shown
```

### aliasfree-diffusion-models-pytorch_amd/ops.py

```python
import weakref

import numpy as np
import os
import torch

from ._lib import AfdError, lib

GN_EPS = 1e-5
LN_EPS = 1e-5
NULL_LABEL = -1


_raw_stream = getattr(torch._C, "_cuda_getCurrentRawStream", None)
_get_device = getattr(torch._C, "_cuda_getDevice", None) or torch.cuda.current_device


def _stream():
    if _raw_stream is not None:
        return _raw_stream(_get_device())
    return torch.cuda.current_stream().cuda_stream


def _chk(*tensors):
    for t in tensors:
# ... 116 lines not shown
    def backward(ctx, dy):
        (x,) = ctx.saved_tensors
        B, C, H, W = x.shape
        dy = _c(dy)
        dx = torch.empty_like(x)
        ws = _act_ws(B, C, H, W, ctx.tu.N, 1, x.device)
        lib().afd_filt_act_bwd(_p(x), _p(dy), _p(dx), B, C, H, W, None, None, None, None,
                               ctx.tu.ptr, ctx.td.ptr, ctx.tu.N, _p(ws), None, _stream())
        return dx, None, None


class _GradMode:
    inplace = False
    side = None
    sides = []
    turn = 0
    pending = []
    launched = []
    batch = 8
    on_write = None
    fold_hint = None
    folds = []
    fold_writes = []
    flushes = 0
    lane_of = {}
    fold_every = 2


def _wrote(*params):
    cb = _GradMode.on_write
    if cb is not None:
        cb([q for q in params if q is not None])


FOLD_DESC = "<QQqqqqii"


def fold_desc(part_ptr, dst_ptr, n, splits, stride=None, inner=None, rstride=1, accumulate=1):
    import struct
    return struct.pack(FOLD_DESC, part_ptr, dst_ptr, n, n if stride is None else stride, n if inner is None else inner, rstride,
                       splits, accumulate)


def fold_now(descs, stream=None):
    import ctypes
    buf = ctypes.create_string_buffer(descs, len(descs))
    lib().afd_fold_batched(ctypes.addressof(buf), len(descs) // 56, _stream() if stream is None else stream)


def defer_to_side_stream(fn, *keep, writes=()):
    _GradMode.pending.append((fn, keep, writes))
    if len(_GradMode.pending) >= _GradMode.batch:
        flush_wgrads()


FOLD_MAX = 56


def fold_batches(descs, limit=FOLD_MAX):
    assert len(descs) % 56 == 0 and limit > 0
    out, cur, seen = [], [], set()
    for o in range(0, len(descs), 56):
        d = descs[o:o + 56]
        dst = d[8:16]
        if dst in seen or len(cur) == limit:
            out.append(b"".join(cur))
            cur, seen = [], set()
        cur.append(d)
        seen.add(dst)
    if cur:
        out.append(b"".join(cur))
    return out


def deal_lane(keys, lane_of, turn, n_lanes):
    known = [lane_of[k] for k in keys if k in lane_of]
    lane = known[0] if known else turn % n_lanes
    conflict = any(l != lane for l in known)
    for k in keys:
        lane_of[k] = lane
    return lane, conflict


def _grad_keys(params):
    return [q.grad.data_ptr() for q in params if q is not None and q.grad is not None]


def _launch_folds():
    G = _GradMode
    for k, side in enumerate(G.sides):
        if G.folds[k]:
            for batch in fold_batches(b"".join(G.folds[k])):
                fold_now(batch, side.cuda_stream)
            G.folds[k] = []
    done = G.fold_writes
    G.fold_writes, G.flushes = [], 0
    return done


def _launch_lanes(lanes, done):
    G = _GradMode
    cur = torch.cuda.current_stream()
    for k, (side, items) in enumerate(zip(G.sides, lanes)):
        if not items:
            continue
        side.wait_stream(cur)
        with torch.cuda.stream(side):
            h = side.cuda_stream
            for fn, keep, ws in items:
                descs = fn(h) if fn is not None else keep[0]
                if descs and G.fold_every == 0:
                    for batch in fold_batches(descs):
                        fold_now(batch, h)
                    done.extend(ws)
                elif descs:
                    G.folds[k].append(descs)
                    G.fold_writes.extend(ws)
                else:
                    done.extend(ws)


def flush_wgrads(final=False):
    G = _GradMode
    sides, q = G.sides, G.pending
    if not q and not (final and any(G.folds)):
        return
    if len(G.folds) != len(sides):
        G.folds = [[] for _ in sides]
    done = []
    lanes = [[] for _ in sides]
    for item in q:
        lane, conflict = deal_lane(_grad_keys(item[2]), G.lane_of, G.turn, len(sides))
        G.turn += 1
        if conflict:
            _launch_lanes(lanes, done)
            done.extend(_launch_folds())
            lanes = [[] for _ in sides]
            for a in sides:
                for b in sides:
                    if a is not b:
                        a.wait_stream(b)
        lanes[lane].append(item)
    _launch_lanes(lanes, done)
    G.launched.extend(q)
    G.pending = []
    G.flushes += 1
    if any(G.folds) and (final or G.flushes >= max(1, G.fold_every) or (G.fold_hint is not None and G.fold_hint(G.fold_writes + done))):
        done.extend(_launch_folds())
    if G.on_write is not None and done:
        _wrote(*done)


class inplace_param_grads:

    def __init__(self, side_stream=None, batch=8, on_write=None, fold_hint=None, fold_every=None):
        self.side_stream, self.batch, self.on_write, self.fold_hint = side_stream, batch, on_write, fold_hint
        self.fold_every = int(os.environ.get("AFD_FOLD_EVERY", 2)) if fold_every is None else fold_every

    def __enter__(self):
        G = _GradMode
        self.prev = (G.inplace, G.side, G.sides, G.on_write, G.fold_hint, G.fold_every)
        ss = self.side_stream
        self.streams = [] if ss is None else (list(ss) if isinstance(ss, (list, tuple)) else [ss])
        G.inplace, G.batch, G.on_write, G.fold_hint, G.fold_every = True, self.batch, self.on_write, self.fold_hint, max(0, self.fold_every)
        G.sides, G.side, G.turn = self.streams, (self.streams[0] if self.streams else None), 0
        G.folds, G.fold_writes, G.flushes, G.lane_of = [[] for _ in self.streams], [], 0, {}

    def __exit__(self, exc_type, *a):
        G = _GradMode
        if self.streams:
            if exc_type is not None:
                G.pending, G.folds, G.fold_writes = [], [[] for _ in self.streams], []
            flush_wgrads(final=True)
            for st in self.streams:
                torch.cuda.current_stream().wait_stream(st)
            G.launched = []
        G.lane_of = {}
        G.inplace, G.side, G.sides, G.on_write, G.fold_hint, G.fold_every = self.prev


def _direct(*params):
    if not _GradMode.inplace:
        return False
    for q in params:
        if q is None:
            continue
        g = q.grad
        if g is None or not g.is_contiguous() or g.dtype != torch.float32:
            return False
    return True


def _gn_param_targets(C, gamma, beta, device):
    if gamma is not None and beta is not None and _direct(gamma, beta):
        return gamma.grad, beta.grad, 1, (None, None)
    out = torch.empty(2, C, device=device, dtype=torch.float32)
    return out[0], out[1], 0, (out[0], out[1])


class GroupNorm1(_Fn):

    @staticmethod
    def forward(ctx, x, gamma, beta, res, emb, act):
        _chk(x, gamma, beta, res, emb)
        x, res, emb = _c(x), _c(res), _c(emb)
        B, C, H, W = x.shape
        y = torch.empty_like(x)
        stats = torch.empty(B, 2, device=x.device, dtype=torch.float32)
        lib().afd_groupnorm1_fwd(_p(x), _p(y), _p(stats), B, C, H * W, GN_EPS, _p(gamma), _p(beta), _p(res), act,
                                 _p(emb), _stream())
        ctx.save_for_backward(x, gamma, beta, res, stats)
        ctx.act, ctx.has_emb = act, emb is not None
        return y

    @staticmethod
    def backward(ctx, dy):
        x, gamma, beta, res, stats = ctx.saved_tensors
        B, C, H, W = x.shape
        dy = _c(dy)
        dx = torch.empty_like(x)
        dres = None
        if res is not None:
            dres = dy if ctx.act == 0 else torch.empty_like(x)
        part = torch.empty(B * C * 2, device=x.device, dtype=torch.float32)
        demb = torch.empty(B, C, device=x.device, dtype=torch.float32) if ctx.has_emb else None
        dg, db, acc, (dgamma, dbeta) = _gn_param_targets(C, gamma, beta, x.device)
        defer = acc and _GradMode.side is not None
        lib().afd_groupnorm1_bwd(_p(x), _p(dy), _p(stats), B, C, H * W, _p(gamma), _p(beta), _p(res), ctx.act,
                                 _p(dx), _p(dres) if (res is not None and ctx.act == 1) else None, _p(part), _p(demb), 0,
                                 None if defer else _p(dg), None if defer else _p(db), acc, _stream())
        if defer:
            pp = _p(part)
            defer_to_side_stream(None, fold_desc(pp, _p(dg), C, B, stride=2 * C) + fold_desc(pp + 4 * C, _p(db), C, B, stride=2 * C),
                                 part, writes=(gamma, beta))
        elif acc:
            _wrote(gamma, beta)
        return dx, dgamma, dbeta, dres, demb, None


class GroupNormFiltAct(_Fn):

    @staticmethod
    def forward(ctx, x, gamma, beta, res, tu, td):
        _chk(x, gamma, beta, res)
        x, res = _c(x), _c(res)
        B, C, H, W = x.shape
        stats = torch.empty(B, 2, device=x.device, dtype=torch.float32)
        L = lib()
        y = torch.empty_like(x)
        if L.afd_filt_act_fwd_gn_supported(C, H, W, tu.N):
            L.afd_filt_act_fwd_gn(_p(x), _p(y), B, C, H, W, GN_EPS, _p(stats), _p(gamma), _p(beta), _p(res), tu.ptr, td.ptr, tu.N,
                                  _stream())
        else:
            L.afd_groupnorm1_fwd(_p(x), None, _p(stats), B, C, H * W, GN_EPS, None, None, None, 0, None, _stream())
            ws = _act_ws(B, C, H, W, tu.N, 0, x.device)
            L.afd_filt_act_fwd(_p(x), _p(y), B, C, H, W, _p(stats), _p(gamma), _p(beta), _p(res), tu.ptr, td.ptr, tu.N,
                               _p(ws), _stream())
        ctx.save_for_backward(x, gamma, beta, res, stats)
        ctx.tu, ctx.td = tu, td
        return y

    @staticmethod
    def backward(ctx, dy):
        x, gamma, beta, res, stats = ctx.saved_tensors
        B, C, H, W = x.shape
        dy = _c(dy)
        L = lib()
        if L.afd_filt_act_fwd_gn_supported(C, H, W, ctx.tu.N):
            dx = torch.empty_like(x)
            dres = torch.empty_like(x) if res is not None else None
            part = torch.empty(B * C * 2, device=x.device, dtype=torch.float32)
            L.afd_filt_act_bwd_gn(_p(x), _p(dy), _p(dx), _p(dres), B, C, H, W, _p(stats), _p(gamma), _p(beta), _p(res),
                                  ctx.tu.ptr, ctx.td.ptr, ctx.tu.N, _p(part), _stream())
            dg, db, acc, (dgamma, dbeta) = _gn_param_targets(C, gamma, beta, x.device)
            if acc and _GradMode.side is not None:
                pp = _p(part)
                defer_to_side_stream(None, fold_desc(pp, _p(dg), C, B, stride=2 * C) + fold_desc(pp + 4 * C, _p(db), C, B, stride=2 * C),
                                     part, writes=(gamma, beta))
            else:
                L.afd_colsum2(_p(part), _p(dg), _p(db), B, C, acc, _stream())
                if acc:
                    _wrote(gamma, beta)
            return dx, dgamma, dbeta, dres, None, None
        dv = torch.empty_like(x)
        ws = _act_ws(B, C, H, W, ctx.tu.N, 1, x.device)
        part = torch.empty(B * C * 2, device=x.device, dtype=torch.float32)
        fused = ws is None
        L.afd_filt_act_bwd(_p(x), _p(dy), _p(dv), B, C, H, W, _p(stats), _p(gamma), _p(beta), _p(res),
                           ctx.tu.ptr, ctx.td.ptr, ctx.tu.N, _p(ws), _p(part) if fused else None, _stream())
        dx = torch.empty_like(x)
        dg, db, acc, (dgamma, dbeta) = _gn_param_targets(C, gamma, beta, x.device)
        L.afd_groupnorm1_bwd(_p(x), _p(dv), _p(stats), B, C, H * W, _p(gamma), _p(beta), None, 0,
                             _p(dx), None, _p(part), None, 1 if fused else 0, _p(dg), _p(db), acc, _stream())
        if acc:
            _wrote(gamma, beta)
        return dx, dgamma, dbeta, (dv if res is not None else None), None, None


def _kind_of(kinds, dgrad):
    direct = kinds >> dgrad & 1
    return direct | (kinds & 4 if direct else 0)


class _WinoWeights:
    epoch = 0
    store = {}
    max_entries = 4096
    recording = None
    active_plan = None

    @classmethod
    def get(cls, w, nbytes, dgrad, kinds=0):
        plan = cls.active_plan
        if plan is not None:
            u = plan.lookup(w, nbytes, dgrad, kinds)
            if u is not None:
                return u, 1
        if cls.recording is not None:
            rec = cls.recording.setdefault(id(w), [w, 0, 0, 0])
            rec[1 + dgrad] = nbytes
            rec[3] = kinds
        capturing = torch.cuda.is_current_stream_capturing()
        key = (id(w), dgrad, _stream())
        stamp = (w._version, cls.epoch, w.data_ptr(), nbytes, _kind_of(kinds, dgrad))
        if not capturing:
            hit = cls.store.get(key)
            if hit is not None and hit[0]() is w and hit[2] == stamp:
                return hit[1], 1
        u = torch.empty(nbytes // 4, device=w.device, dtype=torch.float32)
        if not capturing:
            if len(cls.store) > cls.max_entries:
                cls.store.clear()
            try:
                cls.store[key] = (weakref.ref(w), u, stamp)
            except TypeError:
                pass
        return u, 0


class WinoStepPlan:

    def __init__(self, requests):
        import struct
        reqs = [r for r in requests.values() if r[1] or r[2]]
        self.ok = bool(reqs)
        if not self.ok:
            return
        dev = reqs[0][0].device
        self.buf = torch.empty(sum(r[1] + r[2] for r in reqs) // 4, device=dev, dtype=torch.float32)
        self.map, descs, wg, off = {}, b"", [], 0
        for i, (w, nf, nd, kinds) in enumerate(reqs):
            Cout, Cin = w.shape[0], w.shape[1]
            uf = self.buf[off:off + nf // 4] if nf else None
            off += nf // 4
            ud = self.buf[off:off + nd // 4] if nd else None
            off += nd // 4
            self.map[id(w)] = (weakref.ref(w), w.data_ptr(), uf, ud, kinds)
            n_wg = (Cin * Cout // 64 + 3) // 4
            descs += struct.pack("<QQQiiii", w.data_ptr(), uf.data_ptr() if nf else 0, ud.data_ptr() if nd else 0, Cin, Cout, len(wg), kinds)
            wg += [i] * n_wg
        self.n_wg = len(wg)
        self.descs = torch.frombuffer(bytearray(descs), dtype=torch.uint8).to(dev)
        self.wg = torch.tensor(wg, dtype=torch.int32).to(dev)

    def valid(self):
        return self.ok and all(r() is not None and r().data_ptr() == ptr for (r, ptr, _, _, _) in self.map.values())

    def launch(self):
        lib().afd_conv3x3_wino_weights_batched(_p(self.descs), _p(self.wg), self.n_wg, _stream())

    def lookup(self, w, nbytes, dgrad, kinds=0):
        e = self.map.get(id(w))
        if e is None or e[0]() is not w or _kind_of(e[4], dgrad) != _kind_of(kinds, dgrad):
            return None
        u = e[3] if dgrad else e[2]
        return u if (u is not None and u.numel() * 4 == nbytes) else None


def bump_param_epoch():
    _WinoWeights.epoch += 1
    if _WinoWeights.store:
        _WinoWeights.store.clear()


def _conv_fwd(x, w, bias, res, y, B, Cin, Cout, H, W, ks, act, want_dgrad=False):
    L = lib()
    nb = L.afd_conv3x3_wino_workspace_bytes(B, Cin, Cout, H, W, 0) if ks == 3 else 0
    nd = L.afd_conv3x3_wino_workspace_bytes(B, Cin, Cout, H, W, 1) if (ks == 3 and want_dgrad) else 0
    ud = None
    if nb:
        kinds = L.afd_conv3x3_weight_kinds(B, Cin, Cout, H, W)
        u, ready = _WinoWeights.get(w, nb, 0, kinds)
        if nd:
            ud, dready = _WinoWeights.get(w, nd, 1, kinds)
            if not (ready and dready):
                L.afd_conv3x3_wino_weights(_p(w), _p(u), _p(ud), Cin, Cout, kinds, _stream())
                ready = 1
        L.afd_conv3x3_wino_fwd(_p(x), _p(w), _p(bias), _p(res), _p(y), B, Cin, Cout, H, W, act, _p(u), ready, kinds, _stream())
    else:
        L.afd_conv_fwd(_p(x), _p(w), _p(bias), _p(res), _p(y), B, Cin, Cout, H, W, ks, act, _stream())
    return (ud, kinds) if ud is not None else None


class Conv(_Fn):

    @staticmethod
    def forward(ctx, x, w, bias, res, w_param=None, b_param=None, fork=False):
        _chk(x, w, bias, res)
        x, w, res = _c(x), _c(w), _c(res)
        B, Cin, H, W = x.shape
        Cout, ks = w.shape[0], w.shape[-1]
        y = torch.empty(B, Cout, H, W, device=x.device, dtype=torch.float32)
        ctx.u_dgrad = _conv_fwd(x, w, bias, res, y, B, Cin, Cout, H, W, ks, 0, want_dgrad=x.requires_grad)
        ctx.save_for_backward(x, w)
        ctx.has_bias, ctx.has_res = bias is not None, res is not None
        ctx.w_param, ctx.b_param = w_param, b_param
        return (y, x.view_as(x)) if fork else y

    @staticmethod
    def backward(ctx, dy, dfork=None):
        x, w = ctx.saved_tensors
        B, Cin, H, W = x.shape
        Cout, ks = w.shape[0], w.shape[-1]
        dy = _c(dy)
        L = lib()
        dx = dw = db = None
        if ctx.needs_input_grad[0]:
            dx = torch.empty_like(x)
            dfork = _c(dfork)
            nb = L.afd_conv3x3_wino_workspace_bytes(B, Cin, Cout, H, W, 1) if ks == 3 else 0
            if nb:
                if ctx.u_dgrad is not None:
                    (u, kinds), ready = ctx.u_dgrad, 1
                else:
                    kinds = L.afd_conv3x3_weight_kinds(B, Cin, Cout, H, W)
                    u, ready = _WinoWeights.get(w, nb, 1, kinds)
                L.afd_conv3x3_wino_dgrad(_p(dy), _p(w), _p(dx), _p(dfork), B, Cin, Cout, H, W, _p(u), ready, kinds, _stream())
            else:
                L.afd_conv_dgrad(_p(dy), _p(w), _p(dx), B, Cin, Cout, H, W, ks, _stream())
                if dfork is not None:
                    L.afd_add(_p(dx), _p(dfork), _p(dx), dx.numel(), _stream())
        if ctx.needs_input_grad[1] or (ctx.has_bias and ctx.needs_input_grad[2]):
            nbytes = L.afd_conv_wgrad_workspace_bytes(B, Cin, Cout, H, W, ks)
            ws = torch.empty(max(nbytes // 4, 1), device=x.device, dtype=torch.float32)
            wp, bp = ctx.w_param, ctx.b_param
            if wp is not None and (bp is not None or not ctx.has_bias) and _direct(wp, bp) and wp.grad.numel() == w.numel():
                side = _GradMode.side
                if side is None:
                    L.afd_conv_wgrad(_p(x), _p(dy), _p(wp.grad), _p(bp.grad) if bp is not None else None,
                                     B, Cin, Cout, H, W, ks, 1, _p(ws), _stream())
                    _wrote(wp, bp)
                else:
                    dwp, dbp = _p(wp.grad), (_p(bp.grad) if bp is not None else None)
                    defer_to_side_stream(lambda st, x=x, dy=dy, ws=ws: _wgrad_partials(x, dy, dwp, dbp, B, Cin, Cout, H, W, ks, ws, st),
                                         x, dy, ws, writes=(wp, bp))
            else:
                dw = torch.empty_like(w)
                db = torch.empty(Cout, device=x.device, dtype=torch.float32) if ctx.has_bias else None
                L.afd_conv_wgrad(_p(x), _p(dy), _p(dw), _p(db), B, Cin, Cout, H, W, ks, 0, _p(ws), _stream())
        return dx, dw, db, (dy if ctx.has_res else None), None, None, None


def conv(x, w, bias=None, res=None, w_param=None, b_param=None, fork=False):
    if w_param is None and isinstance(w, torch.nn.Parameter):
        w_param = w
    if b_param is None and isinstance(bias, torch.nn.Parameter):
        b_param = bias
    return Conv.apply(x, w, bias, res, w_param, b_param, fork)


def conv_infer(x, w, bias=None, res=None, act=0):
    _chk(x, w, bias, res)
    x, w, res = _c(x), _c(w), _c(res)
    B, Cin, H, W = x.shape
    Cout, ks = w.shape[0], w.shape[-1]
    y = torch.empty(B, Cout, H, W, device=x.device, dtype=torch.float32)
    _conv_fwd(x, w, bias, res, y, B, Cin, Cout, H, W, ks, act)
    return y


class LayerNormC(_Fn):

    @staticmethod
    def forward(ctx, x, gamma, beta):
        _chk(x, gamma, beta)
        x = _c(x)
        B, C, H, W = x.shape
        y = torch.empty_like(x)
        stats = torch.empty(B, H * W, 2, device=x.device, dtype=torch.float32)
        lib().afd_layernorm_c_fwd(_p(x), _p(y), _p(stats), B, C, H * W, LN_EPS, _p(gamma), _p(beta), _stream())
        ctx.save_for_backward(x, gamma, stats)
        ctx.beta_param = beta
        return y, x.view_as(x)

    @staticmethod
    def backward(ctx, dy, dres):
        x, gamma, stats = ctx.saved_tensors
        B, C, H, W = x.shape
        if dy is None:
            return dres, None, None
        dy, dres = _c(dy), _c(dres)
        dx = torch.empty_like(x)
        L = lib()
        if _direct(gamma, ctx.beta_param):
            L.afd_layernorm_c_bwd(_p(x), _p(dy), _p(stats), B, C, H * W, _p(gamma), _p(dx), _p(dres), None, None, None, 0, _stream())
            _ln_param_grads(x, dy, stats, gamma, ctx.beta_param, B, C, H * W)
            return dx, None, None
        part = torch.empty(B, 2, C, device=x.device, dtype=torch.float32)
        dg, db, acc, (dgamma, dbeta) = _gn_param_targets(C, gamma, ctx.beta_param, x.device)
        L.afd_layernorm_c_bwd(_p(x), _p(dy), _p(stats), B, C, H * W, _p(gamma), _p(dx), _p(dres), _p(part), _p(dg), _p(db), acc,
                              _stream())
        return dx, dgamma, dbeta


def layernorm_c(x, gamma, beta):
    return LayerNormC.apply(x, gamma, beta)[0]


class Attention(_Fn):

    @staticmethod
    def forward(ctx, qkv, heads):
        _chk(qkv)
        qkv = _c(qkv)
        B, C3, H, W = qkv.shape
        C, L = C3 // 3, H * W
        o = torch.empty(B, C, H, W, device=qkv.device, dtype=torch.float32)
        lse = torch.empty(B, heads, L, device=qkv.device, dtype=torch.float32)
        lib().afd_attn_fwd(_p(qkv), _p(o), _p(lse), B, heads, C // heads, L, _stream())
        ctx.save_for_backward(qkv, o, lse)
        ctx.heads = heads
        return o

    @staticmethod
    def backward(ctx, do):
        qkv, o, lse = ctx.saved_tensors
        B, C3, H, W = qkv.shape
        C, L = C3 // 3, H * W
        do = _c(do)
        dqkv = torch.empty_like(qkv)
        delta = torch.empty_like(lse)
        lib().afd_attn_bwd(_p(qkv), _p(o), _p(do), _p(lse), _p(dqkv), _p(delta), B, ctx.heads, C // ctx.heads, L, _stream())
        return dqkv, None


def tok_supported(C):
    return bool(lib().afd_tok_supported(int(C)))


def _wgrad_partials(x, dy, dwp, dbp, B, Cin, Cout, H, W, ks, ws, st):
    import ctypes
    buf = ctypes.create_string_buffer(112)
    n = ctypes.c_int(0)
    lib().afd_conv_wgrad_partials(_p(x), _p(dy), dwp, dbp, B, Cin, Cout, H, W, ks, 1, _p(ws), ctypes.addressof(buf), ctypes.addressof(n), st)
    return buf.raw[:56 * n.value]


def _linear_grads(x, dy, w, b, B, C_in, C_out, H, W, need_w=True):
    L = lib()
    nbytes = L.afd_conv_wgrad_workspace_bytes(B, C_in, C_out, H, W, 1)
    ws = torch.empty(max(nbytes // 4, 1), device=x.device, dtype=torch.float32)
    if _direct(w, b):
        dwp, dbp = _p(w.grad), (_p(b.grad) if b is not None else None)
        if _GradMode.side is not None:
            defer_to_side_stream(lambda st, x=x, dy=dy, ws=ws: _wgrad_partials(x, dy, dwp, dbp, B, C_in, C_out, H, W, 1, ws, st),
                                 x, dy, ws, writes=(w, b))
        else:
            L.afd_conv_wgrad(_p(x), _p(dy), dwp, dbp, B, C_in, C_out, H, W, 1, 1, _p(ws), _stream())
            _wrote(w, b)
        return None, None
    dw = torch.empty_like(w)
    db = torch.empty(C_out, device=x.device, dtype=torch.float32) if b is not None else None
    L.afd_conv_wgrad(_p(x), _p(dy), _p(dw), _p(db), B, C_in, C_out, H, W, 1, 0, _p(ws), _stream())
    return dw, db


def _ln_param_grads(x, dy, stats, gamma, beta, B, C, HW):
    L = lib()
    part = torch.empty(B, 2, C, device=x.device, dtype=torch.float32)
    dg, db, acc, (dgamma, dbeta) = _gn_param_targets(C, gamma, beta, x.device)
    pdg, pdb = _p(dg), _p(db)
    if acc and _GradMode.side is not None:
        def fn(st, x=x, dy=dy, stats=stats, part=part):
            L.afd_layernorm_c_bwd_partials(_p(x), _p(dy), _p(stats), B, C, HW, _p(part), st)
            pp = _p(part)
            return fold_desc(pp, pdg, C, B, stride=2 * C) + fold_desc(pp + 4 * C, pdb, C, B, stride=2 * C)
        defer_to_side_stream(fn, x, dy, stats, part, writes=(gamma, beta))
    else:
        L.afd_layernorm_c_bwd_params(_p(x), _p(dy), _p(stats), B, C, HW, _p(part), pdg, pdb, acc, _stream())
        if acc:
            _wrote(gamma, beta)
    return dgamma, dbeta


class AttnHead(_Fn):

    @staticmethod
    def forward(ctx, x, gamma, beta, w_in, b_in):
        _chk(x, gamma, beta, w_in, b_in)
        x = _c(x)
        B, C, H, W = x.shape
        train = not isinstance(ctx, _NoCtx)
        qkv = torch.empty(B, 3 * C, H, W, device=x.device, dtype=torch.float32)
        h = torch.empty_like(x) if train else None
        stats = torch.empty(B, H * W, 2, device=x.device, dtype=torch.float32) if train else None
        lib().afd_tok_head_fwd(_p(x), _p(gamma), _p(beta), _p(w_in), _p(b_in), _p(h), _p(stats), _p(qkv), B, C, H * W, LN_EPS, _stream())
        ctx.save_for_backward(x, h, stats, gamma, w_in)
        ctx.params = (beta, b_in)
        return qkv, x.view_as(x)

    @staticmethod
    def backward(ctx, dqkv, dres):
        x, h, stats, gamma, w_in = ctx.saved_tensors
        beta, b_in = ctx.params
        B, C, H, W = x.shape
        dqkv = _c(dqkv)
        if dres is None:
            dres = torch.zeros_like(x)
        dres = _c(dres)
        dx = torch.empty_like(x)
        dh = torch.empty_like(x)
        lib().afd_tok_head_bwd(_p(dqkv), _p(x), _p(stats), _p(gamma), _p(w_in), _p(dres), _p(dh), _p(dx), B, C, H * W, _stream())
        dw, db = _linear_grads(h, dqkv, w_in, b_in, B, C, 3 * C, H, W)
        dgamma, dbeta = _ln_param_grads(x, dh, stats, gamma, beta, B, C, H * W)
        return dx, dgamma, dbeta, dw, db


class AttnTail(_Fn):

    @staticmethod
    def forward(ctx, att, x, wo, bo, gamma, beta, w1, b1, w2, b2):
        _chk(att, x, wo, bo, gamma, beta, w1, b1, w2, b2)
        att, x = _c(att), _c(x)
        B, C, H, W = att.shape
        out = torch.empty_like(att)
        if not isinstance(ctx, _NoCtx):
            a, f, u, g = (torch.empty_like(att) for _ in range(4))
            stats = torch.empty(B, H * W, 2, device=att.device, dtype=torch.float32)
        else:
            a = f = u = g = stats = None
        lib().afd_tok_tail_fwd(_p(att), _p(x), _p(wo), _p(bo), _p(gamma), _p(beta), _p(w1), _p(b1), _p(w2), _p(b2),
                               _p(a), _p(stats), _p(f), _p(u), _p(g), _p(out), B, C, H * W, LN_EPS, _stream())
        ctx.save_for_backward(att, a, stats, f, u, g, gamma, wo, w1, w2)
        ctx.params = (bo, beta, b1, b2)
        return out

    @staticmethod
    def backward(ctx, dout):
        att, a, stats, f, u, g, gamma, wo, w1, w2 = ctx.saved_tensors
        bo, beta, b1, b2 = ctx.params
        B, C, H, W = att.shape
        dout = _c(dout)
        du, df, da, datt = (torch.empty_like(att) for _ in range(4))
        lib().afd_tok_tail_bwd(_p(dout), _p(u), _p(a), _p(stats), _p(gamma), _p(w2), _p(w1), _p(wo),
                               _p(du), _p(df), _p(da), _p(datt), B, C, H * W, _stream())
        dw2, db2 = _linear_grads(g, dout, w2, b2, B, C, C, H, W)
        dw1, db1 = _linear_grads(f, du, w1, b1, B, C, C, H, W)
        dwo, dbo = _linear_grads(att, da, wo, bo, B, C, C, H, W)
        dgamma, dbeta = _ln_param_grads(a, df, stats, gamma, beta, B, C, H * W)
        return datt, da, dwo, dbo, dgamma, dbeta, dw1, db1, dw2, db2


class Gelu(_Fn):
    @staticmethod
    def forward(ctx, x):
        _chk(x)
        x = _c(x)
        y = torch.empty_like(x)
        lib().afd_gelu_fwd(_p(x), _p(y), x.numel(), _stream())
        ctx.save_for_backward(x)
        return y

    @staticmethod
    def backward(ctx, dy):
        (x,) = ctx.saved_tensors
        dy = _c(dy)
        dx = torch.empty_like(x)
        lib().afd_gelu_bwd(_p(x), _p(dy), _p(dx), x.numel(), _stream())
        return dx


class MaxPool2(_Fn):
    @staticmethod
    def forward(ctx, x):
        _chk(x)
        x = _c(x)
        B, C, H, W = x.shape
        y = torch.empty(B, C, H // 2, W // 2, device=x.device, dtype=torch.float32)
        lib().afd_maxpool2_fwd(_p(x), _p(y), B, C, H, W, _stream())
        ctx.save_for_backward(x)
        return y

    @staticmethod
    def backward(ctx, dy):
        (x,) = ctx.saved_tensors
        B, C, H, W = x.shape
        dy = _c(dy)
        dx = torch.empty_like(x)
        lib().afd_maxpool2_bwd(_p(x), _p(dy), _p(dx), B, C, H, W, _stream())
        return dx


class UpCat(_Fn):

    @staticmethod
    def forward(ctx, x, skip, taps, mode):
        _chk(x, skip)
        x, skip = _c(x), _c(skip)
        B, C, H, W = x.shape
        Cs = skip.shape[1]
        assert skip.shape[2] == 2 * H and skip.shape[3] == 2 * W
        plane = 4 * H * W
        out = torch.empty(B, Cs + C, 2 * H, 2 * W, device=x.device, dtype=torch.float32)
        L = lib()
        up_ptr = out.data_ptr() + 4 * Cs * plane
        bs = (Cs + C) * plane
        if mode == "filt":
            L.afd_filt_up2_fwd(_p(x), up_ptr, B, C, H, W, 0, bs, taps.ptr, taps.N, _stream())
        else:
            L.afd_bilinear_up2_fwd(_p(x), up_ptr, B, C, H, W, bs, _stream())
        L.afd_copy_batched(_p(skip), _p(out), B, Cs * plane, 0, bs, _stream())
        ctx.taps, ctx.mode, ctx.dims = taps, mode, (B, C, Cs, H, W)
        return out

    @staticmethod
    def backward(ctx, dout):
        B, C, Cs, H, W = ctx.dims
        dout = _c(dout)
        plane = 4 * H * W
        bs = (Cs + C) * plane
        L = lib()
        dx = torch.empty(B, C, H, W, device=dout.device, dtype=torch.float32)
        up_ptr = dout.data_ptr() + 4 * Cs * plane
        if ctx.mode == "filt":
            L.afd_filt_up2_bwd(up_ptr, _p(dx), B, C, H, W, bs, 0, ctx.taps.ptr, ctx.taps.N, _stream())
        else:
            L.afd_bilinear_up2_bwd(up_ptr, _p(dx), B, C, H, W, bs, _stream())
        return dx, dout[:, :Cs], None, None


def pos_encoding(t, inv_freq):
    if not t.is_cuda:
        raise AfdError("afdm: timesteps must live on the HIP device")
    t = t.contiguous()
    B, half = t.shape[0], inv_freq.shape[0]
    out = torch.empty(B, 2 * half, device=t.device, dtype=torch.float32)
    lib().afd_pos_encoding(_p(t), _p(inv_freq), _p(out), B, half, _stream())
    return out


class EmbedAdd(_Fn):

    @staticmethod
    def forward(ctx, temb, table, y):
        _chk(temb, table)
        if not y.is_cuda or y.dtype != torch.long:
            raise AfdError("afdm: class labels must be an int64 tensor on the HIP device")
        temb, table, y = _c(temb), _c(table), _c(y)
        B, D = temb.shape
        if table.shape[1] != D or y.shape[0] != B:
            raise AfdError(f"afdm: label embedding shape mismatch (temb {tuple(temb.shape)}, table {tuple(table.shape)}, y {tuple(y.shape)})")
        out = torch.empty_like(temb)
        lib().afd_label_embed_add_fwd(_p(temb), _p(table), _p(y), _p(out), B, D, table.shape[0], _stream())
        ctx.save_for_backward(y)
        ctx.table = table if isinstance(table, torch.nn.Parameter) else None
        ctx.K = table.shape[0]
        return out

    @staticmethod
    def backward(ctx, dout):
        (y,) = ctx.saved_tensors
        dout = _c(dout)
        B, D = dout.shape
        dtemb = dout if ctx.needs_input_grad[0] else None
        if not ctx.needs_input_grad[1]:
            return dtemb, None, None
        tp = ctx.table
        if tp is not None and _direct(tp):
            lib().afd_embed_add_bwd(_p(dout), _p(y), _p(tp.grad), B, D, ctx.K, 1, _stream())
            _wrote(tp)
            return dtemb, None, None
        dtable = torch.empty(ctx.K, D, device=dout.device, dtype=torch.float32)
        lib().afd_embed_add_bwd(_p(dout), _p(y), _p(dtable), B, D, ctx.K, 0, _stream())
        return dtemb, dtable, None


class SiluLinear(_Fn):

    @staticmethod
    def forward(ctx, temb, w, bias):
        _chk(temb, w, bias)
        temb, w = _c(temb), _c(w)
        B, K = temb.shape
        N = w.shape[0]
        out = torch.empty(B, N, device=temb.device, dtype=torch.float32)
        lib().afd_silu_linear_fwd(_p(temb), _p(w), _p(bias), _p(out), B, K, N, _stream())
        ctx.save_for_backward(temb, w)
        ctx.params = (w if isinstance(w, torch.nn.Parameter) else None, bias if isinstance(bias, torch.nn.Parameter) else None)
        ctx.has_bias = bias is not None
        return out

    @staticmethod
    def backward(ctx, dout):
        temb, w = ctx.saved_tensors
        dout = _c(dout)
        dtemb = torch.zeros_like(temb) if ctx.needs_input_grad[0] else None
        return (dtemb,) + _silu_linear_param_grads(temb, w, dout, dtemb, ctx.params, ctx.has_bias)


def _silu_linear_param_grads(temb, w, dout, dtemb, params, has_bias):
    B, K = temb.shape
    N = w.shape[0]
    wp, bp = params
    if wp is not None and (bp is not None or not has_bias) and _direct(wp, bp):
        pw, pb = _p(wp.grad), (_p(bp.grad) if bp is not None else None)
        if dtemb is None and _GradMode.side is not None:
            defer_to_side_stream(lambda st, temb=temb, w=w, dout=dout: lib().afd_silu_linear_bwd(
                _p(temb), _p(w), _p(dout), pw, pb, None, B, K, N, 1, st), temb, w, dout, writes=(wp, bp))
        else:
            lib().afd_silu_linear_bwd(_p(temb), _p(w), _p(dout), pw, pb, _p(dtemb), B, K, N, 1, _stream())
            _wrote(wp, bp)
        return None, None
    dw = torch.empty_like(w)
    db = torch.empty(N, device=w.device, dtype=torch.float32) if has_bias else None
    lib().afd_silu_linear_bwd(_p(temb), _p(w), _p(dout), _p(dw), _p(db), _p(dtemb), B, K, N, 0, _stream())
    return dw, db


def silu_linear_batched(temb, layers):
    import ctypes, struct
    ws, bs = [w for w, _ in layers], [b for _, b in layers]
    _chk(temb, *ws, *bs)
    temb = _c(temb)
    B, K = temb.shape
    with torch.no_grad():
        outs = [torch.empty(B, w.shape[0], device=temb.device, dtype=torch.float32) for w in ws]
    desc = b"".join(struct.pack("<QQQi4x", _p(w) or 0, _p(b) or 0, _p(o), w.shape[0]) for w, b, o in zip(ws, bs, outs))
    buf = ctypes.create_string_buffer(desc, len(desc))
    lib().afd_silu_linear_fwd_batched(_p(temb), ctypes.addressof(buf), len(ws), B, K, _stream())
    return outs


def gather_rows_batched(idx, tables):
    import ctypes, struct
    _chk(*tables)
    B, rows = idx.shape[0], tables[0].shape[0]
    outs = [torch.empty(B, t.shape[1], device=t.device, dtype=torch.float32) for t in tables]
    desc = b"".join(struct.pack("<QQQi4x", _p(t), 0, _p(o), t.shape[1]) for t, o in zip(tables, outs))
    buf = ctypes.create_string_buffer(desc, len(desc))
    lib().afd_gather_rows_batched(_p(idx), ctypes.addressof(buf), len(tables), B, rows, _stream())
    return outs


class SiluLinearPre(_Fn):

    @staticmethod
    def forward(ctx, out, temb, w, bias):
        ctx.save_for_backward(temb, w)
        ctx.params = (w if isinstance(w, torch.nn.Parameter) else None, bias if isinstance(bias, torch.nn.Parameter) else None)
        ctx.has_bias = bias is not None
        return out.view_as(out)

    @staticmethod
    def backward(ctx, dout):
        temb, w = ctx.saved_tensors
        return (None, None) + _silu_linear_param_grads(temb, w, _c(dout), None, ctx.params, ctx.has_bias)


def noise_images(x, eps, t, alpha_hat):
    _chk(x, eps, alpha_hat)
    x, eps = _c(x), _c(eps)
    out = torch.empty_like(x)
    lib().afd_noise_images(_p(x), _p(eps), _p(t.contiguous()), _p(alpha_hat), _p(out), x.shape[0],
                           x.numel() // x.shape[0], _stream())
    return out


def _step_args(what, x, eps, noise, table, out, out2=None, guided=False, x0=None, mask=None, masked=False):
    _chk(x, eps, noise, table, out, out2, x0)
    n = x.numel()
    ne = 2 * n if guided else n
    if eps.numel() != ne:
        raise AfdError(f"afdm: {what} needs eps{'2' if guided else ''} of {ne} elements (got {eps.numel()})")
    for o in (x, eps, noise, table, out, out2):
        if o is not None and not o.is_contiguous():
            raise AfdError(f"afdm: {what}: every tensor must be contiguous")
        if o is not None and o is not eps and o is not table and o.numel() != n:
            raise AfdError(f"afdm: {what}: x / noise / outputs must hold {n} elements")
    if masked:
        if x0.numel() != n or not x0.is_contiguous():
            raise AfdError(f"afdm: {what}: x0 must be a contiguous tensor of {n} elements")
        if not mask.is_cuda or mask.dtype != torch.uint8 or mask.numel() != n or not mask.is_contiguous():
            raise AfdError(f"afdm: {what}: mask must be a contiguous uint8 device tensor of {n} elements")
    return n


def _ddim_host_t(what, alpha_hat, t, t_prev, eta):
    t, t_prev, eta = int(t), int(t_prev), float(eta)
    if not 0 <= t_prev < t < alpha_hat.numel():
        raise AfdError(f"afdm: {what} needs 0 <= t_prev < t < {alpha_hat.numel()} (got t = {t}, t_prev = {t_prev})")
    if not eta >= 0:
        raise AfdError(f"afdm: {what} needs eta >= 0 (got {eta})")
    return t, t_prev, eta


def _ddim_dev_t(what, t_dev, t_prev_dev):
    for v in (t_dev, t_prev_dev):
        if not v.is_cuda or v.dtype != torch.long or v.numel() < 1:
            raise AfdError(f"afdm: {what}: t_dev / t_prev_dev must be int64 device tensors (element 0 is read)")


def _step(what, x, eps, noise, tables, index, out, eta=None, cfg_scale=None, out2=None, x0=None, mask=None, masked=False, dev=False,
          var=False):
    ddim, guided = eta is not None, cfg_scale is not None
    out = torch.empty_like(x) if out is None else out
    n = _step_args(what, x, eps, noise, tables[0] if ddim else None, out, out2, guided, x0, mask, masked)
    if var:
        sig = tables[1]
        _chk(sig)
        if tuple(sig.shape) != tuple(tables[0].shape) or not sig.is_contiguous():
            raise AfdError(f"afdm: {what}: sig must be a contiguous table of alpha_hat's shape {tuple(tables[0].shape)}")
    if ddim and dev:
        _ddim_dev_t(what, *index)
        eta = float(eta)
    elif ddim:
        *index, eta = _ddim_host_t(what, tables[0], *index, eta)
    index = [_p(v) if dev else int(v) for v in index]
    name = ("afd_ddim_step" if ddim else "afd_denoise_step") + "_var" * var + "_masked" * masked + "_cfg" * guided + "_dev" * dev
    args = [_p(x), _p(eps), _p(noise)] + ([_p(x0), _p(mask)] if masked else []) + [_p(t) for t in tables] + index
    args += ([eta] if ddim else []) + ([float(cfg_scale)] if guided else []) + [_p(out)] + ([_p(out2)] if guided else [])
    getattr(lib(), name)(*args, n, _stream())
    return out


def denoise_step(x, eps_pred, noise, alpha, alpha_hat, beta, i, out=None):
    return _step("denoise step", _c(x), _c(eps_pred), _c(noise), (alpha, alpha_hat, beta), (i,), out)


def denoise_step_dev(x, eps_pred, noise, alpha, alpha_hat, beta, t_dev, out):
    return _step("denoise step", x, eps_pred, noise, (alpha, alpha_hat, beta), (t_dev,), out, dev=True)


def denoise_step_cfg(x, eps2, noise, alpha, alpha_hat, beta, i, cfg_scale, out=None, out2=None):
    return _step("guided denoise step", x, eps2, noise, (alpha, alpha_hat, beta), (i,), out, cfg_scale=cfg_scale, out2=out2)


def denoise_step_cfg_dev(x, eps2, noise, alpha, alpha_hat, beta, t_dev, cfg_scale, out, out2=None):
    return _step("guided denoise step", x, eps2, noise, (alpha, alpha_hat, beta), (t_dev,), out, cfg_scale=cfg_scale, out2=out2, dev=True)


def ddim_step(x, eps, noise, alpha_hat, t, t_prev, eta, out=None):
    return _step("DDIM step", x, eps, noise, (alpha_hat,), (t, t_prev), out, eta=eta)


def ddim_step_dev(x, eps, noise, alpha_hat, t_dev, t_prev_dev, eta, out):
    return _step("DDIM step", x, eps, noise, (alpha_hat,), (t_dev, t_prev_dev), out, eta=eta, dev=True)


# ... 1169 lines not shown
```

### include/afd.h

```cpp
#ifndef AFD_H_
#define AFD_H_

#include <stddef.h>
#include <stdint.h>

#ifdef __cplusplus
extern "C" {
#endif

#define AFD_OK 0
#define AFD_EINVAL 1
#define AFD_ELAUNCH 2
#define AFD_MAX_TAPS 15

typedef void* afd_stream_t;

const char* afd_version(void);
const char* afd_last_error(void);
int afd_device_count(void);

int afd_lowpass_kernel(double omega_c, int N, int has_beta, double beta, float* taps_out);

int afd_filt_up2_fwd(const float* x, float* y, int B, int C, int H, int W, long x_bstride, long y_bstride,
                     const float* taps, int N, afd_stream_t stream);
int afd_filt_up2_bwd(const float* dy, float* dx, int B, int C, int H, int W, long dy_bstride, long dx_bstride,
                     const float* taps, int N, afd_stream_t stream);

int afd_filt_down2_fwd(const float* x, float* y, int B, int C, int H, int W, long x_bstride, long y_bstride,
                       const float* taps, int N, afd_stream_t stream);
int afd_filt_down2_bwd(const float* dy, float* dx, int B, int C, int H, int W, long dy_bstride, long dx_bstride,
                       const float* taps, int N, afd_stream_t stream);

size_t afd_filt_act_workspace_bytes(int B, int C, int H, int W, int N, int backward);
int afd_filt_act_fwd(const float* x, float* y, int B, int C, int H, int W,
                     const float* stats, const float* gamma, const float* beta, const float* res,
                     const float* taps_up, const float* taps_down, int N,
                     void* workspace, afd_stream_t stream);
size_t afd_filt_act_fwd_gn_supported(int C, int H, int W, int N);
int afd_filt_act_fwd_gn(const float* x, float* y, int B, int C, int H, int W, float eps, float* stats_out,
                        const float* gamma, const float* beta, const float* res,
                        const float* taps_up, const float* taps_down, int N, afd_stream_t stream);
int afd_filt_act_bwd_gn(const float* x, const float* dy, float* dx, float* dres, int B, int C, int H, int W, const float* stats,
                        const float* gamma, const float* beta, const float* res, const float* taps_up, const float* taps_down, int N,
                        float* gn_partials, afd_stream_t stream);
int afd_filt_act_bwd(const float* x, const float* dy, float* dv, int B, int C, int H, int W,
                     const float* stats, const float* gamma, const float* beta, const float* res,
                     const float* taps_up, const float* taps_down, int N,
                     void* workspace, float* gn_partials, afd_stream_t stream);

int afd_groupnorm1_fwd(const float* x, float* y, float* stats_out, int B, int C, int HW, float eps,
                       const float* gamma, const float* beta, const float* res, int act, const float* emb,
                       afd_stream_t stream);
int afd_debug_norm_path(int mode);
int afd_groupnorm1_bwd(const float* x, const float* dy, const float* stats, int B, int C, int HW,
                       const float* gamma, const float* beta, const float* res, int act,
                       float* dx, float* dres, float* dgamma_dbeta_partial , float* demb ,
                       int have_partials ,
                       float* dgamma , float* dbeta , int accumulate, afd_stream_t stream);
int afd_colsum(const float* in, float* out, int rows, int cols, int accumulate, afd_stream_t stream);
int afd_colsum_strided(const float* in, long row_stride, float* out, int rows, int cols, int accumulate, afd_stream_t stream);
int afd_colsum2(const float* in, float* out_a, float* out_b, int rows, int C, int accumulate, afd_stream_t stream);

int afd_debug_conv_path(int mode);
int afd_debug_conv_state(long* values, int n);
int afd_conv_fwd(const float* x, const float* w, const float* bias, const float* res, float* y,
                 int B, int Cin, int Cout, int H, int W, int ksize, int act, afd_stream_t stream);
int afd_conv_dgrad(const float* dy, const float* w, float* dx,
                   int B, int Cin, int Cout, int H, int W, int ksize, afd_stream_t stream);
size_t afd_conv_wgrad_workspace_bytes(int B, int Cin, int Cout, int H, int W, int ksize);
int afd_conv_wgrad_form(int B, int Cin, int Cout, int H, int W, int ksize);
int afd_conv_wgrad3_plan(int B, int Cin, int Cout, int H, int W, int* info);
int afd_conv_wgrad(const float* x, const float* dy, float* dw, float* dbias ,
                   int B, int Cin, int Cout, int H, int W, int ksize, int accumulate,
                   void* workspace, afd_stream_t stream);

typedef struct afd_fold_desc {
  const float* part;
  float* dst;
  long n;
  long stride;
  long inner, rstride;
  int splits;
  int accumulate;
} afd_fold_desc;
int afd_fold_batched(const afd_fold_desc* descs, int n, afd_stream_t stream);
int afd_conv_wgrad_partials(const float* x, const float* dy, float* dw, float* dbias ,
                            int B, int Cin, int Cout, int H, int W, int ksize, int accumulate,
                            void* workspace, afd_fold_desc* folds_out, int* n_folds, afd_stream_t stream);

size_t afd_conv3x3_wino_workspace_bytes(int B, int Cin, int Cout, int H, int W, int dgrad);
int afd_conv3x3_wino_weights(const float* w, float* u_fwd, float* u_dgrad, int Cin, int Cout, int kinds, afd_stream_t stream);
int afd_conv3x3_weight_kinds(int B, int Cin, int Cout, int H, int W);
typedef struct afd_wino_desc {
  const float* w;
  float* u_fwd;
  float* u_dgrad;
  int Cin, Cout, first_wg, kinds;
} afd_wino_desc;
int afd_conv3x3_wino_weights_batched(const afd_wino_desc* descs, const int* wg_desc, int n_wg, afd_stream_t stream);
int afd_conv3x3_wino_fwd(const float* x, const float* w, const float* bias, const float* res, float* y,
                         int B, int Cin, int Cout, int H, int W, int act, void* workspace, int weights_ready, int kinds,
                         afd_stream_t stream);
int afd_conv3x3_wino_dgrad(const float* dy, const float* w, float* dx, const float* add_to_dx ,
                           int B, int Cin, int Cout, int H, int W, void* workspace, int weights_ready, int kinds,
                           afd_stream_t stream);

int afd_layernorm_c_fwd(const float* x, float* y, float* stats_out, int B, int C, int HW, float eps,
                        const float* gamma, const float* beta, afd_stream_t stream);
int afd_layernorm_c_bwd(const float* x, const float* dy, const float* stats, int B, int C, int HW,
                        const float* gamma, float* dx, const float* add_to_dx ,
                        float* dgamma_dbeta_partial ,
                        float* dgamma , float* dbeta , int accumulate,
                        afd_stream_t stream);
int afd_layernorm_c_bwd_params(const float* x, const float* dy, const float* stats, int B, int C, int HW,
                               float* dgamma_dbeta_partial , float* dgamma, float* dbeta, int accumulate,
                               afd_stream_t stream);
int afd_layernorm_c_bwd_partials(const float* x, const float* dy, const float* stats, int B, int C, int HW, float* part,
                                 afd_stream_t stream);

int afd_debug_attn_rows(int rows);
int afd_attn_fwd(const float* qkv, float* o, float* lse, int B, int heads, int d, int L, afd_stream_t stream);
int afd_attn_bwd(const float* qkv, const float* o, const float* d_o, const float* lse, float* dqkv,
                 float* delta_workspace , int B, int heads, int d, int L, afd_stream_t stream);

int afd_tok_supported(int C);
int afd_debug_tok_grid(int max_workgroups);
int afd_debug_tok_path(int mode);
int afd_tok_head_fwd(const float* x, const float* gamma, const float* beta, const float* w_in, const float* b_in,
                     float* h_out, float* stats_out, float* qkv, int B, int C, int P, float eps, afd_stream_t stream);
int afd_tok_tail_fwd(const float* att, const float* x, const float* w_o, const float* b_o, const float* gamma, const float* beta,
                     const float* w_1, const float* b_1, const float* w_2, const float* b_2,
                     float* a_out, float* stats_out, float* f_out, float* u_out, float* g_out, float* out,
                     int B, int C, int P, float eps, afd_stream_t stream);
int afd_tok_tail_bwd(const float* d_out, const float* u, const float* a, const float* stats, const float* gamma,
                     const float* w_2, const float* w_1, const float* w_o,
                     float* du_out, float* df_out, float* da_out, float* datt_out, int B, int C, int P, afd_stream_t stream);
int afd_tok_head_bwd(const float* dqkv, const float* x, const float* stats, const float* gamma, const float* w_in,
                     const float* d_res, float* dh_out, float* dx_out, int B, int C, int P, afd_stream_t stream);

int afd_gelu_fwd(const float* x, float* y, long n, afd_stream_t stream);
int afd_gelu_bwd(const float* x, const float* dy, float* dx, long n, afd_stream_t stream);
int afd_maxpool2_fwd(const float* x, float* y, int B, int C, int H, int W, afd_stream_t stream);
int afd_maxpool2_bwd(const float* x, const float* dy, float* dx, int B, int C, int H, int W, afd_stream_t stream);
int afd_bilinear_up2_fwd(const float* x, float* y, int B, int C, int H, int W, long y_bstride, afd_stream_t stream);
int afd_bilinear_up2_bwd(const float* dy, float* dx, int B, int C, int H, int W, long dy_bstride, afd_stream_t stream);
int afd_copy_batched(const float* src, float* dst, int B, long n, long src_bstride, long dst_bstride, afd_stream_t stream);
int afd_add(const float* a, const float* b, float* y, long n, afd_stream_t stream);

int afd_pos_encoding(const int64_t* t, const float* inv_freq, float* temb, int B, int half, afd_stream_t stream);
int afd_silu_linear_fwd(const float* temb, const float* w, const float* bias, float* out,
                        int B, int K, int N, afd_stream_t stream);
int afd_silu_linear_bwd(const float* temb, const float* w, const float* dout, float* dw, float* dbias,
                        float* dtemb , int B, int K, int N, int accumulate, afd_stream_t stream);
typedef struct afd_silu_desc {
  const float* w;
  const float* bias;
  float* out;
  int N;
} afd_silu_desc;
int afd_silu_linear_fwd_batched(const float* temb, const afd_silu_desc* descs, int n, int B, int K, afd_stream_t stream);
int afd_gather_rows_batched(const int64_t* idx, const afd_silu_desc* descs, int n, int B, int rows, afd_stream_t stream);

int afd_embed_add_fwd(const float* temb, const float* table, const int64_t* y, float* out, int B, int D, int num_classes,
                      afd_stream_t stream);
int afd_label_embed_add_fwd(const float* temb, const float* table, const int64_t* y, float* out, int B, int D, int num_classes,
                            afd_stream_t stream);
int afd_embed_add_bwd(const float* dout, const int64_t* y, float* dtable, int B, int D, int num_classes, int accumulate,
                      afd_stream_t stream);

int afd_noise_images(const float* x, const float* eps, const int64_t* t, const float* alpha_hat,
                     float* x_t, int B, long per_sample, afd_stream_t stream);
int afd_denoise_step(const float* x, const float* eps_pred, const float* noise ,
                     const float* alpha, const float* alpha_hat, const float* beta, int i,
                     float* x_out, long n, afd_stream_t stream);
int afd_denoise_step_dev(const float* x, const float* eps_pred, const float* noise,
                         const float* alpha, const float* alpha_hat, const float* beta, const int64_t* t_dev,
                         float* x_out, long n, afd_stream_t stream);
int afd_denoise_step_cfg(const float* x, const float* eps2, const float* noise ,
                         const float* alpha, const float* alpha_hat, const float* beta, int i, float cfg_scale,
                         float* x_out, float* x_out2, long n, afd_stream_t stream);
int afd_denoise_step_cfg_dev(const float* x, const float* eps2, const float* noise,
                             const float* alpha, const float* alpha_hat, const float* beta, const int64_t* t_dev, float cfg_scale,
                             float* x_out, float* x_out2, long n, afd_stream_t stream);
int afd_ddim_step(const float* x, const float* eps, const float* noise , const float* alpha_hat, int t, int t_prev,
                  float eta, float* x_out, long n, afd_stream_t stream);
int afd_ddim_step_dev(const float* x, const float* eps, const float* noise, const float* alpha_hat, const int64_t* t_dev,
                      const int64_t* t_prev_dev, float eta, float* x_out, long n, afd_stream_t stream);
int afd_ddim_step_cfg(const float* x, const float* eps2, const float* noise, const float* alpha_hat, int t, int t_prev, float eta,
                      float cfg_scale, float* x_out, float* x_out2, long n, afd_stream_t stream);
int afd_ddim_step_cfg_dev(const float* x, const float* eps2, const float* noise, const float* alpha_hat, const int64_t* t_dev,
                          const int64_t* t_prev_dev, float eta, float cfg_scale, float* x_out, float* x_out2, long n,
                          afd_stream_t stream);
int afd_ddim_step_var(const float* x, const float* eps, const float* noise , const float* alpha_hat,
                      const float* sig, int t, int t_prev, float eta, float* x_out, long n, afd_stream_t stream);
int afd_ddim_step_var_dev(const float* x, const float* eps, const float* noise, const float* alpha_hat, const float* sig,
                          const int64_t* t_dev, const int64_t* t_prev_dev, float eta, float* x_out, long n, afd_stream_t stream);
int afd_ddim_step_var_cfg(const float* x, const float* eps2, const float* noise, const float* alpha_hat, const float* sig, int t,
                          int t_prev, float eta, float cfg_scale, float* x_out, float* x_out2, long n, afd_stream_t stream);
int afd_ddim_step_var_cfg_dev(const float* x, const float* eps2, const float* noise, const float* alpha_hat, const float* sig,
                              const int64_t* t_dev, const int64_t* t_prev_dev, float eta, float cfg_scale, float* x_out,
                              float* x_out2, long n, afd_stream_t stream);
int afd_ddim_invert_step(const float* x, const float* eps, const float* alpha_hat, int s, int u, float* x_out, long n,
                         afd_stream_t stream);
int afd_ddim_invert_step_dev(const float* x, const float* eps, const float* alpha_hat, const int64_t* s_dev, const int64_t* u_dev,
                             float* x_out, long n, afd_stream_t stream);
int afd_ddim_invert_step_cfg(const float* x, const float* eps2, const float* alpha_hat, int s, int u, float cfg_scale, float* x_out,
                             float* x_out2, long n, afd_stream_t stream);
int afd_ddim_invert_step_cfg_dev(const float* x, const float* eps2, const float* alpha_hat, const int64_t* s_dev,
                                 const int64_t* u_dev, float cfg_scale, float* x_out, float* x_out2, long n, afd_stream_t stream);
int afd_dpmpp_step(const float* x, const float* eps, const float* x0_prev , const float* coef, float* x_out,
                   float* x0_out, long n, afd_stream_t stream);
int afd_dpmpp_step_cfg(const float* x, const float* eps2, const float* x0_prev, const float* coef, float cfg_scale, float* x_out,
                       float* x_out2, float* x0_out, long n, afd_stream_t stream);
int afd_unipc_step(const float* x, const float* eps, float* xc, float* hist, const float* coef, float* x_out, long n,
                   afd_stream_t stream);
int afd_unipc_step_cfg(const float* x, const float* eps2, float* xc, float* hist, const float* coef, float cfg_scale, float* x_out,
                       float* x_out2, long n, afd_stream_t stream);
int afd_noise_images_gather(const float* x0, long n_img, const int64_t* img, const float* eps, const int64_t* t, const float* alpha_hat,
                            float* x_t, long rows, long per, afd_stream_t stream);
int afd_vlb_terms(const float* x0, long n_img, const int64_t* img, const float* x_t, const float* eps, const float* eps_hat,
                  const int64_t* t, const double* coef, long T, const float* alpha, const float* alpha_hat, const float* beta,
                  double* term, double* sq, long rows, long per, afd_stream_t stream);
int afd_vlb_prior(const float* x0, double half_ah, double* out, long n_img, long per, afd_stream_t stream);
int afd_denoise_step_masked(const float* x, const float* eps_pred, const float* noise, const float* x0, const uint8_t* mask,
                            const float* alpha, const float* alpha_hat, const float* beta, int i, float* x_out, long n,
                            afd_stream_t stream);
int afd_denoise_step_masked_dev(const float* x, const float* eps_pred, const float* noise, const float* x0, const uint8_t* mask,
                                const float* alpha, const float* alpha_hat, const float* beta, const int64_t* t_dev, float* x_out,
                                long n, afd_stream_t stream);
int afd_denoise_step_masked_cfg(const float* x, const float* eps2, const float* noise, const float* x0, const uint8_t* mask,
                                const float* alpha, const float* alpha_hat, const float* beta, int i, float cfg_scale, float* x_out,
                                float* x_out2, long n, afd_stream_t stream);
int afd_denoise_step_masked_cfg_dev(const float* x, const float* eps2, const float* noise, const float* x0, const uint8_t* mask,
                                    const float* alpha, const float* alpha_hat, const float* beta, const int64_t* t_dev,
                                    float cfg_scale, float* x_out, float* x_out2, long n, afd_stream_t stream);
int afd_ddim_step_masked(const float* x, const float* eps, const float* noise, const float* x0, const uint8_t* mask,
                         const float* alpha_hat, int t, int t_prev, float eta, float* x_out, long n, afd_stream_t stream);
int afd_ddim_step_masked_dev(const float* x, const float* eps, const float* noise, const float* x0, const uint8_t* mask,
                             const float* alpha_hat, const int64_t* t_dev, const int64_t* t_prev_dev, float eta, float* x_out, long n,
                             afd_stream_t stream);
int afd_ddim_step_masked_cfg(const float* x, const float* eps2, const float* noise, const float* x0, const uint8_t* mask,
                             const float* alpha_hat, int t, int t_prev, float eta, float cfg_scale, float* x_out, float* x_out2, long n,
                             afd_stream_t stream);
int afd_ddim_step_masked_cfg_dev(const float* x, const float* eps2, const float* noise, const float* x0, const uint8_t* mask,
                                 const float* alpha_hat, const int64_t* t_dev, const int64_t* t_prev_dev, float eta, float cfg_scale,
                                 float* x_out, float* x_out2, long n, afd_stream_t stream);
int afd_renoise(const float* x, const float* noise, const float* alpha_hat, int t_from, int t_to, float* x_out, long n,
                afd_stream_t stream);
int afd_lowpass_refine(const float* x, const float* ref, const float* noise , const float* alpha_hat,
                       int t_prev, const float* taps , int N, int levels, float* x_out,
                       float* x_out2 , long planes, int S, afd_stream_t stream);
int afd_lowpass_refine_dev(const float* x, const float* ref, const float* noise, const float* alpha_hat, const int64_t* t_prev_dev,
                           const float* taps , int N, int levels, float* x_out, float* x_out2 ,
                           long planes, int S, afd_stream_t stream);
int afd_quantize_u8(const float* x, uint8_t* out, long n, afd_stream_t stream);

size_t afd_rotate_workspace_bytes(long planes, int H, int W);
int afd_affine_spline3_wrap(const float* x, float* y, long planes, int H, int W, const double* matrix4, const double* offset2,
                            void* workspace, afd_stream_t stream);
int afd_spline3_prefilter_wrap(const float* x, double* coef, long planes, int H, int W, afd_stream_t stream);
int afd_affine_spline3_wrap_rows(const double* coef, long n_src, const int64_t* img, const double* affine, long K, const int64_t* k,
                                 float* out, long rows, int C, int H, int W, afd_stream_t stream);
int afd_eq_terms(const double* coef, long n_src, const int64_t* img, const double* affine, long K, const int64_t* k, const float* g,
                 double margin, double* out, long rows, int C, int H, int W, afd_stream_t stream);

int afd_mse_fwd(const float* pred, const float* target, float* loss_out, float* workspace, long n, afd_stream_t stream);
int afd_mse_bwd(const float* pred, const float* target, const float* dloss, float* dpred, long n, afd_stream_t stream);

#define AFD_PRED_EPS 0
#define AFD_PRED_V 1
#define AFD_PRED_X0 2
int afd_objective_loss_fwd(const float* pred, const float* x0, const float* eps, const int64_t* t, const float* alpha_hat,
                           const float* w_or_null, int kind, float* loss_out, float* workspace, long B, long chw,
                           afd_stream_t stream);
int afd_objective_loss_bwd(const float* pred, const float* x0, const float* eps, const int64_t* t, const float* alpha_hat,
                           const float* w_or_null, int kind, const float* dloss, float* dpred, long B, long chw,
                           afd_stream_t stream);
int afd_pred_to_eps(const float* out, const float* x_t, const int64_t* t, const float* alpha_hat, int kind, float* eps_out, long B,
                    long chw, afd_stream_t stream);

int afd_distill_mid(const float* out1, const float* z_t, const int64_t* t, const int64_t* t_mid, const float* alpha_hat, int kind,
                    float* z_mid, long B, long chw, afd_stream_t stream);
int afd_distill_target(const float* out2, const float* z_mid, const float* z_t, const int64_t* t, const int64_t* t_mid,
                       const int64_t* t_prev, const float* alpha_hat, int kind, float* x_tilde, float* eps_tilde, long B, long chw,
                       afd_stream_t stream);

int afd_consistency_fn(const float* out, const float* z, const int64_t* t, const float* alpha_hat, const double* coef, int kind,
                       float* f_out, long B, long chw, afd_stream_t stream);
int afd_consistency_target(const float* out_tgt, const float* z_prev, const float* z_t, const int64_t* t, const int64_t* t_prev,
                           const float* alpha_hat, const double* coef, int kind, float* x_tilde, float* eps_tilde, long B, long chw,
                           afd_stream_t stream);
int afd_consistency_step(const float* out, const float* z, const float* noise_or_null, const float* alpha_hat, const double* coef,
                         int kind, int t, int t_next, float* x_out, long n_rows, long chw, afd_stream_t stream);
int afd_consistency_step_dev(const float* out, const float* z, const float* noise_or_null, const float* alpha_hat, const double* coef,
                             int kind, const int64_t* t_dev, const int64_t* t_next_dev, float* x_out, long n_rows, long chw,
                             afd_stream_t stream);

int afd_lvar_loss_fwd(const float* out2, const float* x0, const float* eps, const int64_t* t, const float* alpha,
                      const float* alpha_hat, const float* beta, const double* lv_coef, const float* w_or_null, int kind,
                      double vlb_scale, float* loss_out, double* sums_out_or_null, float* workspace, long B, long chw,
                      afd_stream_t stream);
int afd_lvar_loss_bwd(const float* out2, const float* x0, const float* eps, const int64_t* t, const float* alpha,
                      const float* alpha_hat, const float* beta, const double* lv_coef, const float* w_or_null, int kind,
                      double vlb_scale, const float* dloss, float* dout2, long B, long chw, afd_stream_t stream);
int afd_split_pred(const float* out2, const float* x_t, const int64_t* t, const float* alpha_hat, int kind, float* eps_out,
                   float* v_out_or_null, long B, long chw, afd_stream_t stream);
int afd_denoise_step_lvar(const float* x, const float* out2, const float* noise_or_null, const float* alpha, const float* alpha_hat,
                          const float* beta, const double* lv_coef, int kind, int i, float* x_out, long B, long chw,
                          afd_stream_t stream);
int afd_denoise_step_lvar_dev(const float* x, const float* out2, const float* noise_or_null, const float* alpha,
                              const float* alpha_hat, const float* beta, const double* lv_coef, int kind, const int64_t* t_dev,
                              float* x_out, long B, long chw, afd_stream_t stream);
int afd_denoise_step_lvar_cfg(const float* x, const float* out2, const float* noise_or_null, const float* alpha,
                              const float* alpha_hat, const float* beta, const double* lv_coef, int kind, int i, float cfg_scale,
                              float* x_out, float* x_out2, long B, long chw, afd_stream_t stream);
int afd_denoise_step_lvar_cfg_dev(const float* x, const float* out2, const float* noise_or_null, const float* alpha,
                                  const float* alpha_hat, const float* beta, const double* lv_coef, int kind, const int64_t* t_dev,
                                  float cfg_scale, float* x_out, float* x_out2, long B, long chw, afd_stream_t stream);
int afd_vlb_terms_lvar(const float* x0, long n_img, const int64_t* img, const float* x_t, const float* eps, const float* out2,
                       const int64_t* t, const double* lv_coef, long T, const float* alpha, const float* alpha_hat,
                       const float* beta, int kind, double* term, double* sq, long rows, long per, afd_stream_t stream);

int afd_loss_rows(const float* pred, const float* x0, const float* eps, const int64_t* t, const float* alpha_hat,
                  const float* w_or_null, int kind, double* rows, long B, long chw, afd_stream_t stream);
int afd_lvar_loss_rows(const float* out2, const float* x0, const float* eps, const int64_t* t, const float* alpha,
                       const float* alpha_hat, const float* beta, const double* lv_coef, const float* w_or_null, int kind,
                       double vlb_scale, double* rows, long B, long chw, afd_stream_t stream);
int afd_tsampler_tick(const int64_t* t, const double* rows, long B, double* hist, int* count, long T, long H, long lo,
                      double uniform_prob, const float* w_base_or_null, double* prob, double* cdf, float* wtab,
                      float* vwtab_or_null, int* warm, afd_stream_t stream);
int afd_tsampler_draw(const double* cdf, const double* u, long lo, long T, int64_t* t_out, long B, afd_stream_t stream);
int afd_lvar_loss_fwd_tw(const float* out2, const float* x0, const float* eps, const int64_t* t, const float* alpha,
                         const float* alpha_hat, const float* beta, const double* lv_coef, const float* w_or_null,
                         const float* vw_or_null, int kind, double vlb_scale, float* loss_out, double* sums_out_or_null,
                         float* workspace, long B, long chw, afd_stream_t stream);
int afd_lvar_loss_bwd_tw(const float* out2, const float* x0, const float* eps, const int64_t* t, const float* alpha,
                         const float* alpha_hat, const float* beta, const double* lv_coef, const float* w_or_null,
                         const float* vw_or_null, int kind, double vlb_scale, const float* dloss, float* dout2, long B, long chw,
                         afd_stream_t stream);
int afd_adamw_tick(float* state, float beta1, float beta2, afd_stream_t stream);
int afd_adamw_step(float* p, const float* g, float* m, float* v, long n, const float* state,
                   float lr, float beta1, float beta2, float eps, float weight_decay, float grad_scale,
                   afd_stream_t stream);

int afd_ema_step(float* ema, const float* p, long n, int copy, float beta, float one_minus_beta, afd_stream_t stream);
int afd_adamw_ema_tick(float* adam_state, float beta1, float beta2, int* ema_state, int start, afd_stream_t stream);
int afd_adamw_ema_step(float* p, const float* g, float* m, float* v, long n_active, const float* adam_state, float lr,
                       float beta1, float beta2, float eps, float weight_decay, float grad_scale, float* ema, long n_ema,
                       const int* ema_state, float beta, float one_minus_beta, afd_stream_t stream);

#define AFD_LR_CONSTANT 0
#define AFD_LR_LINEAR 1
#define AFD_LR_COSINE 2
typedef struct afd_opt_ctl {
  double base_lr;
  long warmup, total;
  int kind;
  double min_ratio;
  double max_norm;
  int skip_nonfinite;
} afd_opt_ctl;
int afd_grad_sqnorm_n_partials(void);
int afd_grad_sqnorm_partials(const float* g, long n, float grad_scale, double* partials, int n_partials, afd_stream_t stream);
int afd_adamw_ctl_tick(float* adam_state, float beta1, float beta2, int* ema_state, int ema_start, const double* partials,
                       int n_partials, const afd_opt_ctl* cfg, double* ctl, afd_stream_t stream);
int afd_adamw_ctl_step(float* p, const float* g, float* m, float* v, long n_active, const float* adam_state, const double* ctl,
                       float beta1, float beta2, float eps, float weight_decay, float grad_scale, float* ema, long n_ema,
                       const int* ema_state, float beta, float one_minus_beta, afd_stream_t stream);

int afd_replay_build(void* hip_graph, void** out_handle, int* counts);
int afd_replay_run(void* handle, afd_stream_t main_stream, afd_stream_t side_stream);
int afd_replay_free(void* handle);

int afd_batch_gather_u8(const uint8_t* data, long N, long C, long H, long W, const int64_t* idx, const uint8_t* flip_or_null,
                        const float* table, float* x, const int64_t* labels_or_null, int64_t* y_or_null, long B,
                        afd_stream_t stream);
int afd_batch_gather_f32(const float* data, long N, long C, long H, long W, const int64_t* idx, const uint8_t* flip_or_null,
                         float* x, const int64_t* labels_or_null, int64_t* y_or_null, long B, afd_stream_t stream);

size_t afd_nn_search_workspace_bytes(long N, long D, long n, long k, int f32);
int afd_nn_search_u8(const uint8_t* data, long N, long D, const uint8_t* queries, long n, const int64_t* exclude_or_null, long k,
                     int64_t* idx, int64_t* dist, void* workspace, size_t workspace_bytes, afd_stream_t stream);
int afd_nn_search_f32(const float* data, long N, long D, const float* queries, long n, const int64_t* exclude_or_null, long k,
                      int64_t* idx, float* dist, void* workspace, size_t workspace_bytes, afd_stream_t stream);

size_t afd_spectrum_workspace_bytes(long n, long C, long H, long W);
int afd_power_spectrum_u8(const uint8_t* images, const float* table, long n, long C, long H, long W, const double* win_h_or_null,
                          const double* win_w_or_null, int remove_mean, const int* bins_or_null, long R, double* power_or_null,
                          double* radial_or_null, void* workspace, size_t workspace_bytes, afd_stream_t stream);
int afd_power_spectrum_f32(const float* images, long n, long C, long H, long W, const double* win_h_or_null,
                           const double* win_w_or_null, int remove_mean, const int* bins_or_null, long R, double* power_or_null,
                           double* radial_or_null, void* workspace, size_t workspace_bytes, afd_stream_t stream);

size_t afd_feature_moments_workspace_bytes(long n, long D);
int afd_feature_moments_f32(const float* X, long n, long D, double* sum, double* outer, int accumulate, void* workspace,
                            size_t workspace_bytes, afd_stream_t stream);
size_t afd_poly_mmd_workspace_bytes(long S, long m, long D);
int afd_poly_mmd_sums_f32(const float* A, long na, const float* B, long nb, long D, const int64_t* ia, const int64_t* ib, long S, long m,
                          int degree, double gamma, double coef0, double* sums, void* workspace, size_t workspace_bytes,
                          afd_stream_t stream);

size_t afd_kth_neighbour_workspace_bytes(long n, long D, long k);
int afd_kth_neighbour_f32(const float* X, long n, long D, long k, double* radius2, void* workspace, size_t workspace_bytes,
                          afd_stream_t stream);
size_t afd_ball_membership_workspace_bytes(long nq, long nr, long D);
int afd_ball_membership_f32(const float* Q, long nq, const float* R, long nr, long D, const double* radius2,
                            const int64_t* exclude_or_null, int* count_or_null, int64_t* nearest_or_null, double* nearest_d2_or_null,
                            void* workspace, size_t workspace_bytes, afd_stream_t stream);

int afd_pair_quality_f32(const float* a, const float* b, long planes, int C, int H, int W, const double* win, int K, double c1,
                         double c2, const uint8_t* region_or_null, long region_rows, double* out, double* ssim_map_or_null,
                         afd_stream_t stream);
int afd_pair_quality_u8(const uint8_t* a, const uint8_t* b, long planes, int C, int H, int W, const double* win, int K, double c1,
                        double c2, const uint8_t* region_or_null, long region_rows, double* out, double* ssim_map_or_null,
                        afd_stream_t stream);

int afd_slerp_rows(const float* a, const float* b, const float* w, float* out, long pairs, long W, long row, afd_stream_t stream);

int afd_linop_apply(const float* x, float* y, const float* kernel , int K, int stride, const float* mask_or_null,
                    int mask_channels, long B, int C, int H, int W, afd_stream_t stream);
int afd_linop_adjoint(const float* r, float* g, const float* kernel , int K, int stride, const float* mask_or_null,
                      int mask_channels, long B, int C, int H, int W, afd_stream_t stream);
int afd_dps_residual(const float* x_t, const float* out, const int64_t* t_rows, const float* alpha_hat, int prediction, const float* y,
                     const float* kernel , int K, int stride, const float* mask_or_null, int mask_channels,
                     float* g, double* sums, long B, int C, int H, int W, afd_stream_t stream);
int afd_dps_correct(float* x, const float* g, const float* v, const double* sums, const int64_t* t_rows, const float* alpha_hat,
                    int prediction, double zeta, long B, int C, long HW, afd_stream_t stream);

int afd_ode_trace_rows(const float* v, const float* w_or_null, double cvv, double cvw, double* acc, long rows, long per,
                       afd_stream_t stream);
int afd_ode_heun_step(const float* x, const float* eps_s, const float* eps_u, const float* alpha_hat, int s, int u, float* x_out, long n,
                      afd_stream_t stream);

int afd_eps_sqnorm_rows(const float* eps, double* rows, long B, long chw, afd_stream_t stream);
int afd_eps_sqnorm_rows_cfg(const float* eps2, float cfg_scale, double* rows, long B, long chw, afd_stream_t stream);

#ifdef __cplusplus
}
#endif
#endif
```

Baseline: 40970 images/s.

## Prebuild split-half weight images for token kernels once per step

Token-block kernels (LN+QKV head, attention-out/MLP tail, and their backward passes) currently convert fp32 weights into split-fp16 LDS images inside every workgroup. The step plan now builds these images once per optimizer step in a shared buffer, and the kernels copy them straight into LDS. The h2 path selection also widens to cases where prebuilt images are available. This adds plan bookkeeping, per-slab descriptors and padding, and relies on the images staying in sync with weight updates.

```diff
diff --git a/aliasfree-diffusion-models-pytorch_amd/csrc/tok.hip b/aliasfree-diffusion-models-pytorch_amd/csrc/tok.hip
--- a/aliasfree-diffusion-models-pytorch_amd/csrc/tok.hip
+++ b/aliasfree-diffusion-models-pytorch_amd/csrc/tok.hip
@@ -1,5 +1,6 @@
 #include "tok_common.h"
 #include "tok_h2.h"
+#include "tok_image.h"
 #include <algorithm>
 #include <cstdint>
 #include <mutex>
@@ -664,12 +665,14 @@
 template <class K> static int set_lds(K kern, size_t lds) { return lds_opt_in(kern, lds); }
 static int g_tok_max_wg = 0;
 static int g_tok_path = 0;
-static bool use_h2(int C, long ntile, int kern) {
+static int g_tok_images = 1;
+static bool use_h2(int C, long ntile, int kern, bool fed) {
   if (C != 64 && C != 128) return false;
   if (g_tok_path >= 4) return true;
   if (g_tok_path != 0) return false;
-  if (C == 64) return ntile >= 1024 || (kern == 2 && ntile >= 512);
-  return kern != 1 && ntile >= 512;
+  if (ntile < 512) return false;
+  if (C == 64) return ntile >= 1024 || kern == 2 || (fed && kern == 0);
+  return kern != 1 || fed;
 }
 static bool use_wide(int C, long ntile) {
   if (C != 64 && C != 128) return false;
@@ -677,6 +680,12 @@
   if (g_tok_path == 2) return true;
   return C == 128 || ntile < 1024;
 }
+struct TokImg {
+  const void* m[3];
+  TokImg(const void* a, const void* b, const void* c) : m{a, b, c} {}
+  const void* const* get() const { return (g_tok_images && m[0] && m[1] && m[2]) ? m : nullptr; }
+  bool aligned() const { return !((uintptr_t)m[0] & 15) && !((uintptr_t)m[1] & 15) && !((uintptr_t)m[2] & 15); }
+};
 static unsigned chain_grid(int C, long ntile) {
   const long wg = (ntile + 3) / 4;
   const long cap = g_tok_max_wg > 0 ? g_tok_max_wg : (C > 64 ? 8192 : 1024);
@@ -692,20 +701,33 @@
 int afd_tok_supported(int C) { return tok_ok(C) ? 1 : 0; }
 int afd_debug_tok_grid(int max_workgroups) { g_tok_max_wg = max_workgroups; return AFD_OK; }
 int afd_debug_tok_path(int mode) {
-  AFD_REQUIRE(mode >= 0 && mode <= 6, "afd_debug_tok_path: mode %d not in 0..6", mode);
+  AFD_REQUIRE(mode >= 0 && mode <= 7, "afd_debug_tok_path: mode %d not in 0..7", mode);
   g_tok_path = mode;
-  tok_h2_debug_tpw(mode == 5 ? 2 : (mode == 6 ? 4 : 0));
+  tok_h2_debug_tpw(mode == 5 ? 2 : (mode == 6 ? 4 : (mode == 7 ? 1 : 0)));
   return AFD_OK;
+}
+
+int afd_debug_tok_images(int on) { g_tok_images = on ? 1 : 0; return AFD_OK; }
+size_t afd_tok_image_bytes(int B, int C, int P, int kern) {
+  if (B <= 0 || P <= 0 || kern < 0 || kern > 3) return 0;
+  return use_h2(C, ((long)B * P + 31) / 32, kern, true) ? tok_image_bytes(C) : 0;
 }
 
 int afd_tok_head_fwd(const float* x, const float* gamma, const float* beta, const float* w, const float* bias, float* h_out,
                      float* stats_out, float* qkv, int B, int C, int P, float eps, afd_stream_t st) {
+  return afd_tok_head_fwd_img(x, gamma, beta, w, bias, h_out, stats_out, qkv, B, C, P, eps, nullptr, nullptr, nullptr, st);
+}
+int afd_tok_head_fwd_img(const float* x, const float* gamma, const float* beta, const float* w, const float* bias, float* h_out,
+                         float* stats_out, float* qkv, int B, int C, int P, float eps, const void* img_q, const void* img_k,
+                         const void* img_v, afd_stream_t st) {
+  const TokImg im(img_q, img_k, img_v);
+  AFD_REQUIRE(im.aligned(), "afd_tok_head_fwd_img: an image is not 16-byte aligned");
   AFD_REQUIRE(x && gamma && beta && w && qkv && B > 0 && P > 0, "afd_tok_head_fwd: NULL pointer or empty shape");
   AFD_REQUIRE(tok_ok(C), "afd_tok_head_fwd: C=%d not covered (32, 64, 128)", C);
   AFD_REQUIRE((long)B * P * 3 * C < (1L << 31), "afd_tok_head_fwd: tensor too large for 32-bit offsets");
   const int N = 3 * C;
   const long ntile = ((long)B * P + 31) / 32, wg_tiles = (ntile + 3) / 4;
-  if (use_h2(C, ntile, 0)) return tok_h2_head_fwd(x, gamma, beta, w, bias, h_out, stats_out, qkv, B, C, P, eps, g_tok_max_wg, as_stream(st));
+  if (use_h2(C, ntile, 0, im.get() != nullptr)) return tok_h2_head_fwd(x, gamma, beta, w, bias, h_out, stats_out, qkv, B, C, P, eps, g_tok_max_wg, im.get(), as_stream(st));
   if (use_wide(C, ntile) && aligned16(w) && (ntile <= 256 || g_tok_path == 2)) {
     const long waves = ntile * (N / 32);
     const dim3 wgrid((unsigned)((waves + 3) / 4));
@@ -735,6 +757,15 @@
 int afd_tok_tail_fwd(const float* att, const float* x, const float* wo, const float* bo, const float* gamma, const float* beta,
                      const float* w1, const float* b1, const float* w2, const float* b2, float* a_out, float* stats_out,
                      float* f_out, float* u_out, float* g_out, float* out, int B, int C, int P, float eps, afd_stream_t st) {
+  return afd_tok_tail_fwd_img(att, x, wo, bo, gamma, beta, w1, b1, w2, b2, a_out, stats_out, f_out, u_out, g_out, out, B, C, P, eps,
+                              nullptr, nullptr, nullptr, st);
+}
+int afd_tok_tail_fwd_img(const float* att, const float* x, const float* wo, const float* bo, const float* gamma, const float* beta,
+                         const float* w1, const float* b1, const float* w2, const float* b2, float* a_out, float* stats_out,
+                         float* f_out, float* u_out, float* g_out, float* out, int B, int C, int P, float eps, const void* img_o,
+                         const void* img_1, const void* img_2, afd_stream_t st) {
+  const TokImg im(img_o, img_1, img_2);
+  AFD_REQUIRE(im.aligned(), "afd_tok_tail_fwd_img: an image is not 16-byte aligned");
   AFD_REQUIRE(att && x && wo && bo && gamma && beta && w1 && b1 && w2 && b2 && out && B > 0 && P > 0,
               "afd_tok_tail_fwd: NULL pointer or empty shape");
   AFD_REQUIRE(tok_ok(C), "afd_tok_tail_fwd: C=%d not covered (32, 64, 128)", C);
@@ -743,8 +774,8 @@
   AFD_REQUIRE(!train || (stats_out && f_out && u_out && g_out), "afd_tok_tail_fwd: a_out given but a saved-tensor pointer is NULL");
   const long ntile = ((long)B * P + 31) / 32;
   hipStream_t s = as_stream(st);
-  if (use_h2(C, ntile, 1))
-    return tok_h2_tail_fwd(att, x, wo, bo, gamma, beta, w1, b1, w2, b2, a_out, stats_out, f_out, u_out, g_out, out, B, C, P, eps, g_tok_max_wg, s);
+  if (use_h2(C, ntile, 1, im.get() != nullptr))
+    return tok_h2_tail_fwd(att, x, wo, bo, gamma, beta, w1, b1, w2, b2, a_out, stats_out, f_out, u_out, g_out, out, B, C, P, eps, g_tok_max_wg, im.get(), s);
   if (use_wide(C, ntile) && aligned16(wo) && aligned16(w1) && aligned16(w2)) {
     const dim3 wgrid((unsigned)((ntile + Wide<64>::TPW - 1) / Wide<64>::TPW)), wgrid128((unsigned)ntile);
 #define AFD_TAILW(C_, T_, G_) hipLaunchKernelGGL((tok_tail_fwd_wide<C_, T_>), G_, dim3(256), 0, s, att, x, wo, bo, gamma, beta, w1, b1, w2, b2, \
@@ -771,13 +802,20 @@
 int afd_tok_tail_bwd(const float* d_out, const float* u, const float* a, const float* stats, const float* gamma, const float* w2,
                      const float* w1, const float* wo, float* du_out, float* df_out, float* da_out, float* datt_out, int B, int C,
                      int P, afd_stream_t st) {
+  return afd_tok_tail_bwd_img(d_out, u, a, stats, gamma, w2, w1, wo, du_out, df_out, da_out, datt_out, B, C, P, nullptr, nullptr, nullptr, st);
+}
+int afd_tok_tail_bwd_img(const float* d_out, const float* u, const float* a, const float* stats, const float* gamma, const float* w2,
+                         const float* w1, const float* wo, float* du_out, float* df_out, float* da_out, float* datt_out, int B, int C,
+                         int P, const void* img_2t, const void* img_1t, const void* img_ot, afd_stream_t st) {
+  const TokImg im(img_2t, img_1t, img_ot);
+  AFD_REQUIRE(im.aligned(), "afd_tok_tail_bwd_img: an image is not 16-byte aligned");
   AFD_REQUIRE(d_out && u && a && stats && gamma && w2 && w1 && wo && du_out && df_out && da_out && datt_out && B > 0 && P > 0,
               "afd_tok_tail_bwd: NULL pointer or empty shape");
   AFD_REQUIRE(tok_ok(C), "afd_tok_tail_bwd: C=%d not covered (32, 64, 128)", C);
   AFD_REQUIRE((long)B * P * C < (1L << 31), "afd_tok_tail_bwd: tensor too large for 32-bit offsets");
   const long ntile = ((long)B * P + 31) / 32;
   hipStream_t s = as_stream(st);
-  if (use_h2(C, ntile, 2)) return tok_h2_tail_bwd(d_out, u, a, stats, gamma, w2, w1, wo, du_out, df_out, da_out, datt_out, B, C, P, g_tok_max_wg, s);
+  if (use_h2(C, ntile, 2, im.get() != nullptr)) return tok_h2_tail_bwd(d_out, u, a, stats, gamma, w2, w1, wo, du_out, df_out, da_out, datt_out, B, C, P, g_tok_max_wg, im.get(), s);
   if (use_wide(C, ntile)) {
     if (C == 64) hipLaunchKernelGGL(tok_tail_bwd_wide<64>, dim3((unsigned)((ntile + 1) / 2)), dim3(256), 0, s, d_out, u, a, stats, gamma, w2, w1, wo, du_out, df_out, da_out, datt_out, B, P);
     else         hipLaunchKernelGGL(tok_tail_bwd_wide<128>, dim3((unsigned)ntile), dim3(256), 0, s, d_out, u, a, stats, gamma, w2, w1, wo, du_out, df_out, da_out, datt_out, B, P);
@@ -794,12 +832,19 @@
 
 int afd_tok_head_bwd(const float* dqkv, const float* x, const float* stats, const float* gamma, const float* w_in,
                      const float* d_res, float* dh_out, float* dx_out, int B, int C, int P, afd_stream_t st) {
+  return afd_tok_head_bwd_img(dqkv, x, stats, gamma, w_in, d_res, dh_out, dx_out, B, C, P, nullptr, nullptr, nullptr, st);
+}
+int afd_tok_head_bwd_img(const float* dqkv, const float* x, const float* stats, const float* gamma, const float* w_in,
+                         const float* d_res, float* dh_out, float* dx_out, int B, int C, int P, const void* img_qt,
+                         const void* img_kt, const void* img_vt, afd_stream_t st) {
+  const TokImg im(img_qt, img_kt, img_vt);
+  AFD_REQUIRE(im.aligned(), "afd_tok_head_bwd_img: an image is not 16-byte aligned");
   AFD_REQUIRE(dqkv && x && stats && gamma && w_in && d_res && dx_out && B > 0 && P > 0, "afd_tok_head_bwd: NULL pointer or empty shape");
   AFD_REQUIRE(tok_ok(C), "afd_tok_head_bwd: C=%d not covered (32, 64, 128)", C);
   AFD_REQUIRE((long)B * P * 3 * C < (1L << 31), "afd_tok_head_bwd: tensor too large for 32-bit offsets");
   const long ntile = ((long)B * P + 31) / 32;
   hipStream_t s = as_stream(st);
-  if (use_h2(C, ntile, 3)) return tok_h2_head_bwd(dqkv, x, stats, gamma, w_in, d_res, dh_out, dx_out, B, C, P, g_tok_max_wg, s);
+  if (use_h2(C, ntile, 3, im.get() != nullptr)) return tok_h2_head_bwd(dqkv, x, stats, gamma, w_in, d_res, dh_out, dx_out, B, C, P, g_tok_max_wg, im.get(), s);
   if (use_wide(C, ntile)) {
     if (C == 64) hipLaunchKernelGGL(tok_head_bwd_wide<64>, dim3((unsigned)((ntile + 1) / 2)), dim3(256), 0, s, dqkv, x, stats, gamma, w_in, d_res, dh_out, dx_out, B, P);
     else         hipLaunchKernelGGL(tok_head_bwd_wide<128>, dim3((unsigned)ntile), dim3(256), 0, s, dqkv, x, stats, gamma, w_in, d_res, dh_out, dx_out, B, P);
diff --git a/aliasfree-diffusion-models-pytorch_amd/csrc/tok_h2.h b/aliasfree-diffusion-models-pytorch_amd/csrc/tok_h2.h
--- a/aliasfree-diffusion-models-pytorch_amd/csrc/tok_h2.h
+++ b/aliasfree-diffusion-models-pytorch_amd/csrc/tok_h2.h
@@ -4,15 +4,15 @@
 namespace afd {
 
 int tok_h2_head_fwd(const float* x, const float* gamma, const float* beta, const float* w, const float* bias, float* h_out,
-                    float* stats_out, float* qkv, int B, int C, int P, float eps, int max_wg, hipStream_t s);
+                    float* stats_out, float* qkv, int B, int C, int P, float eps, int max_wg, const void* const* img, hipStream_t s);
 int tok_h2_tail_fwd(const float* att, const float* x, const float* wo, const float* bo, const float* gamma, const float* beta,
                     const float* w1, const float* b1, const float* w2, const float* b2, float* a_out, float* stats_out,
-                    float* f_out, float* u_out, float* g_out, float* out, int B, int C, int P, float eps, int max_wg, hipStream_t s);
+                    float* f_out, float* u_out, float* g_out, float* out, int B, int C, int P, float eps, int max_wg, const void* const* img, hipStream_t s);
 int tok_h2_tail_bwd(const float* d_out, const float* u, const float* a, const float* stats, const float* gamma, const float* w2,
                     const float* w1, const float* wo, float* du_out, float* df_out, float* da_out, float* datt_out, int B, int C,
-                    int P, int max_wg, hipStream_t s);
+                    int P, int max_wg, const void* const* img, hipStream_t s);
 int tok_h2_head_bwd(const float* dqkv, const float* x, const float* stats, const float* gamma, const float* w_in,
-                    const float* d_res, float* dh_out, float* dx_out, int B, int C, int P, int max_wg, hipStream_t s);
+                    const float* d_res, float* dh_out, float* dx_out, int B, int C, int P, int max_wg, const void* const* img, hipStream_t s);
 void tok_h2_debug_tpw(int tpw);
 
 }
diff --git a/aliasfree-diffusion-models-pytorch_amd/csrc/tok_h2.hip b/aliasfree-diffusion-models-pytorch_amd/csrc/tok_h2.hip
--- a/aliasfree-diffusion-models-pytorch_amd/csrc/tok_h2.hip
+++ b/aliasfree-diffusion-models-pytorch_amd/csrc/tok_h2.hip
@@ -1,5 +1,6 @@
 #include "tok_common.h"
 #include "h2_common.h"
+#include "tok_image.h"
 #include "tok_h2.h"
 #include <algorithm>
 
@@ -80,8 +81,6 @@
   static size_t bytes(int nvec) { return (size_t)NSLOT * REC * 16 + (size_t)NSLOT * C * 8 + (size_t)nvec * C * 4; }
 };
 
-struct WSrc { const float* w; int ldw, n0, k0; };
-
 template <int C, int NT> struct Stg {
   static constexpr int NG = C / 8, NR = C * NG / NT;
   float x[NR][8];
@@ -99,12 +98,7 @@
     for (int r = 0; r < NR; ++r) {
       int n, G;
       rec(r, transposed, n, G);
-      const int kb = 16 * (G >> 1) + 4 * (G & 1);
-#pragma unroll
-      for (int e = 0; e < 8; ++e) {
-        const int k = kb + 8 * (e >> 2) + (e & 3);
-        x[r][e] = transposed ? q.w[(long)(q.k0 + k) * q.ldw + q.n0 + n] : q.w[(long)(q.n0 + n) * q.ldw + q.k0 + k];
-      }
+      timg_load8(q, transposed, n, G, x[r]);
     }
   }
   __device__ __forceinline__ void maxima(unsigned* __restrict__ rmax, bool transposed) const {
@@ -112,10 +106,7 @@
     for (int r = 0; r < NR; ++r) {
       int n, G;
       rec(r, transposed, n, G);
-      float m = 0.f;
-#pragma unroll
-      for (int e = 0; e < 8; ++e) m = fmaxf(m, fabsf(x[r][e]));
-      atomicMax(&rmax[n], __float_as_uint(m));
+      atomicMax(&rmax[n], __float_as_uint(timg_max8(x[r])));
     }
   }
   __device__ __forceinline__ void store(h8* __restrict__ img, float* __restrict__ winv, const unsigned* __restrict__ rmax,
@@ -125,10 +116,7 @@
       int n, G;
       rec(r, transposed, n, G);
       const float sc = h2_scale_for(__uint_as_float(rmax[n]));
-      h8 p0, p1;
-      h2_split8(x[r], sc, p0, p1);
-      img[G * C + n] = p0;
-      img[(NG + G) * C + n] = p1;
+      timg_put(img, C, n, G, x[r], sc);
       if (G == 0) winv[n] = h2_inv_pow2(sc);
     }
   }
@@ -151,13 +139,40 @@
   __builtin_amdgcn_sched_barrier(0);
 }
 template <int C, int NT>
-__device__ __forceinline__ void h2_stage_first(const H2Lds<C>& L, const WSrc* src, bool transposed) {
-  if (H2Lds<C>::RELOAD) h2_stage<C, NT, 0, 2>(L, src, transposed);
-  else h2_stage<C, NT, 0, 3>(L, src, transposed);
-}
-template <int C, int NT, int M>
-__device__ __forceinline__ void h2_stage_one(const H2Lds<C>& L, const WSrc* src, bool transposed) {
-  h2_stage<C, NT, M, 1>(L, src + M, transposed);
+__device__ __forceinline__ void h2_fetch(h8* __restrict__ img, float* __restrict__ winv, const void* __restrict__ g) {
+  constexpr int REC = H2Lds<C>::REC, NR = REC / NT, CH = NR < 8 ? NR : 8;
+  static_assert(REC % NT == 0 && NR % CH == 0, "whole records per thread");
+  const h8* __restrict__ gi = static_cast<const h8*>(g) + threadIdx.x;
+  h8* __restrict__ li = img + threadIdx.x;
+#pragma unroll 1
+  for (int r0 = 0; r0 < NR; r0 += CH) {
+    h8 v[CH];
+#pragma unroll
+    for (int r = 0; r < CH; ++r) v[r] = gi[(r0 + r) * NT];
+#pragma unroll
+    for (int r = 0; r < CH; ++r) li[(r0 + r) * NT] = v[r];
+  }
+  const float* __restrict__ gw = reinterpret_cast<const float*>(static_cast<const h8*>(g) + REC);
+  for (int c = threadIdx.x; c < C; c += NT) winv[c] = gw[c];
+}
+struct H2Img { const void* m[3]; };
+template <int C, int NT, bool IMG, int M0, int CNT>
+__device__ __forceinline__ void h2_get(const H2Lds<C>& L, const WSrc* src, bool transposed, const H2Img& im) {
+  if constexpr (IMG) {
+#pragma unroll
+    for (int i = 0; i < CNT; ++i) h2_fetch<C, NT>(L.img[M0 + i], L.winv[M0 + i], im.m[M0 + i]);
+  } else {
+    h2_stage<C, NT, M0, CNT>(L, src + M0, transposed);
+  }
+}
+template <int C, int NT, bool IMG>
+__device__ __forceinline__ void h2_stage_first(const H2Lds<C>& L, const WSrc* src, bool transposed, const H2Img& im) {
+  if (H2Lds<C>::RELOAD) h2_get<C, NT, IMG, 0, 2>(L, src, transposed, im);
+  else h2_get<C, NT, IMG, 0, 3>(L, src, transposed, im);
+}
+template <int C, int NT, bool IMG, int M>
+__device__ __forceinline__ void h2_stage_one(const H2Lds<C>& L, const WSrc* src, bool transposed, const H2Img& im) {
+  h2_get<C, NT, IMG, M, 1>(L, src, transposed, im);
 }
 
 struct Walk { int lane, wv, half, l31, ntile, tstride, t0, npass; unsigned total; };
@@ -174,12 +189,12 @@
 
 extern __shared__ __attribute__((aligned(16))) unsigned char h2_smem[];
 
-template <int C, int TPW>
+template <int C, int TPW, bool IMG>
 __global__ __launch_bounds__(64 * TPW) void tok_h2_head_fwd_k(const float* __restrict__ x, const float* __restrict__ gamma,
                                                                const float* __restrict__ beta, const float* __restrict__ w,
                                                                const float* __restrict__ bias, float* __restrict__ h_out,
                                                                float* __restrict__ stats_out, float* __restrict__ y, int B, int P,
-                                                               float eps) {
+                                                               float eps, const H2Img im) {
   using LD = H2Lds<C>;
   constexpr int KB = C / 32, NT = 64 * TPW;
   LD L;
@@ -188,14 +203,14 @@
   const Walk k = walk_of<TPW>(B, P);
   const int half = k.half, l31 = k.l31;
   const WSrc src[3] = {{w, C, 0, 0}, {w, C, C, 0}, {w, C, 2 * C, 0}};
-  h2_stage_first<C, NT>(L, src, false);
+  h2_stage_first<C, NT, IMG>(L, src, false, im);
   for (int i = threadIdx.x; i < C; i += NT) { vec[i] = gamma[i]; vec[C + i] = beta[i]; }
   for (int i = threadIdx.x; i < 3 * C; i += NT) vec[2 * C + i] = bias ? bias[i] : 0.f;
   __syncthreads();
   for (int pass = 0; pass < k.npass; ++pass) {
     const int t = k.t0 + k.wv + pass * k.tstride;
     const bool active = t < k.ntile;
-    if (LD::RELOAD && pass > 0) { __syncthreads(); h2_stage_one<C, NT, 0>(L, src, false); __syncthreads(); }
+    if (LD::RELOAD && pass > 0) { __syncthreads(); h2_stage_one<C, NT, IMG, 0>(L, src, false, im); __syncthreads(); }
     Pix pc = pix_of(active ? t : 0, l31, k.total, P);
     pc.live = pc.live && active;
     const unsigned yb = tbase(pc, 3 * C, P, half);
@@ -213,7 +228,7 @@
     }
 #pragma unroll
     for (int sl = 0; sl < 3; ++sl) {
-      if (LD::RELOAD && sl == 1) { __syncthreads(); h2_stage_one<C, NT, 2>(L, src, false); }
+      if (LD::RELOAD && sl == 1) { __syncthreads(); h2_stage_one<C, NT, IMG, 2>(L, src, false, im); }
       if (LD::RELOAD && sl == 2) __syncthreads();
       if (active) {
 #pragma unroll
@@ -232,7 +247,7 @@
   }
 }
 
-template <int C, int TPW, bool TRAIN>
+template <int C, int TPW, bool IMG, bool TRAIN>
 __global__ __launch_bounds__(64 * TPW) void tok_h2_tail_fwd_k(const float* __restrict__ att, const float* __restrict__ xres,
                                                                const float* __restrict__ wo, const float* __restrict__ bo,
                                                                const float* __restrict__ gamma, const float* __restrict__ beta,
@@ -241,7 +256,7 @@
                                                                float* __restrict__ a_out, float* __restrict__ stats_out,
                                                                float* __restrict__ f_out, float* __restrict__ u_out,
                                                                float* __restrict__ g_out, float* __restrict__ out, int B, int P,
-                                                               float eps) {
+                                                               float eps, const H2Img im) {
   using LD = H2Lds<C>;
   constexpr int KB = C / 32, NT = 64 * TPW;
   LD L;
@@ -250,7 +265,7 @@
   const Walk k = walk_of<TPW>(B, P);
   const int half = k.half, l31 = k.l31;
   const WSrc src[3] = {{wo, C, 0, 0}, {w1, C, 0, 0}, {w2, C, 0, 0}};
-  h2_stage_first<C, NT>(L, src, false);
+  h2_stage_first<C, NT, IMG>(L, src, false, im);
   for (int i = threadIdx.x; i < C; i += NT) {
     vec[i] = bo[i]; vec[C + i] = gamma[i]; vec[2 * C + i] = beta[i]; vec[3 * C + i] = b1[i]; vec[4 * C + i] = b2[i];
   }
@@ -258,7 +273,7 @@
   for (int pass = 0; pass < k.npass; ++pass) {
     const int t = k.t0 + k.wv + pass * k.tstride;
     const bool active = t < k.ntile;
-    if (LD::RELOAD && pass > 0) { __syncthreads(); h2_stage_one<C, NT, 0>(L, src, false); __syncthreads(); }
+    if (LD::RELOAD && pass > 0) { __syncthreads(); h2_stage_one<C, NT, IMG, 0>(L, src, false, im); __syncthreads(); }
     Pix pc = pix_of(active ? t : 0, l31, k.total, P);
     pc.live = pc.live && active;
     const unsigned base = tbase(pc, C, P, half);
@@ -288,7 +303,7 @@
       }
       is = hp_split<KB>(z, hp);
     }
-    if (LD::RELOAD) { __syncthreads(); h2_stage_one<C, NT, 2>(L, src, false); }
+    if (LD::RELOAD) { __syncthreads(); h2_stage_one<C, NT, IMG, 2>(L, src, false, im); }
     if (active) {
       TT<KB> g;
 #pragma unroll
@@ -326,14 +341,14 @@
   }
 }
 
-template <int C, int TPW>
+template <int C, int TPW, bool IMG>
 __global__ __launch_bounds__(64 * TPW) void tok_h2_tail_bwd_k(const float* __restrict__ dout, const float* __restrict__ u_in,
                                                                const float* __restrict__ a_in, const float* __restrict__ stats,
                                                                const float* __restrict__ gamma, const float* __restrict__ w2,
                                                                const float* __restrict__ w1, const float* __restrict__ wo,
                                                                float* __restrict__ du_out, float* __restrict__ df_out,
                                                                float* __restrict__ da_out, float* __restrict__ datt_out, int B,
-                                                               int P) {
+                                                               int P, const H2Img im) {
   using LD = H2Lds<C>;
   constexpr int KB = C / 32, NT = 64 * TPW;
   LD L;
@@ -342,13 +357,13 @@
   const Walk k = walk_of<TPW>(B, P);
   const int half = k.half, l31 = k.l31;
   const WSrc src[3] = {{w2, C, 0, 0}, {w1, C, 0, 0}, {wo, C, 0, 0}};
-  h2_stage_first<C, NT>(L, src, true);
+  h2_stage_first<C, NT, IMG>(L, src, true, im);
   for (int i = threadIdx.x; i < C; i += NT) gs[i] = gamma[i];
   __syncthreads();
   for (int pass = 0; pass < k.npass; ++pass) {
     const int t = k.t0 + k.wv + pass * k.tstride;
     const bool active = t < k.ntile;
-    if (LD::RELOAD && pass > 0) { __syncthreads(); h2_stage_one<C, NT, 0>(L, src, true); __syncthreads(); }
+    if (LD::RELOAD && pass > 0) { __syncthreads(); h2_stage_one<C, NT, IMG, 0>(L, src, true, im); __syncthreads(); }
     Pix pc = pix_of(active ? t : 0, l31, k.total, P);
     pc.live = pc.live && active;
     const unsigned base = tbase(pc, C, P, half);
@@ -369,7 +384,7 @@
       h_store(z, du_out, base, P, pc.live);
       is = hp_split<KB>(z, hp);
     }
-    if (LD::RELOAD) { __syncthreads(); h2_stage_one<C, NT, 2>(L, src, true); }
+    if (LD::RELOAD) { __syncthreads(); h2_stage_one<C, NT, IMG, 2>(L, src, true, im); }
     if (active) {
       TT<KB> df, aa, dd;
 #pragma unroll
@@ -401,12 +416,12 @@
   }
 }
 
-template <int C, int TPW>
+template <int C, int TPW, bool IMG>
 __global__ __launch_bounds__(64 * TPW) void tok_h2_head_bwd_k(const float* __restrict__ dqkv, const float* __restrict__ x,
                                                                const float* __restrict__ stats, const float* __restrict__ gamma,
                                                                const float* __restrict__ w_in, const float* __restrict__ dres,
                                                                float* __restrict__ dh_out, float* __restrict__ dx_out, int B,
-                                                               int P) {
+                                                               int P, const H2Img im) {
   using LD = H2Lds<C>;
   constexpr int KB = C / 32, NT = 64 * TPW;
   LD L;
@@ -415,13 +430,13 @@
   const Walk k = walk_of<TPW>(B, P);
   const int half = k.half, l31 = k.l31;
   const WSrc src[3] = {{w_in, C, 0, 0}, {w_in, C, 0, C}, {w_in, C, 0, 2 * C}};
-  h2_stage_first<C, NT>(L, src, true);
+  h2_stage_first<C, NT, IMG>(L, src, true, im);
   for (int i = threadIdx.x; i < C; i += NT) gs[i] = gamma[i];
   __syncthreads();
   for (int pass = 0; pass < k.npass; ++pass) {
     const int t = k.t0 + k.wv + pass * k.tstride;
     const bool active = t < k.ntile;
-    if (LD::RELOAD && pass > 0) { __syncthreads(); h2_stage_one<C, NT, 0>(L, src, true); __syncthreads(); }
+    if (LD::RELOAD && pass > 0) { __syncthreads(); h2_stage_one<C, NT, IMG, 0>(L, src, true, im); __syncthreads(); }
     Pix pc = pix_of(active ? t : 0, l31, k.total, P);
     pc.live = pc.live && active;
     const unsigned base = tbase(pc, C, P, half);
@@ -429,7 +444,7 @@
     TT<KB> dh;
 #pragma unroll
     for (int sl = 0; sl < 3; ++sl) {
-      if (LD::RELOAD && sl == 1) { __syncthreads(); h2_stage_one<C, NT, 2>(L, src, true); }
+      if (LD::RELOAD && sl == 1) { __syncthreads(); h2_stage_one<C, NT, IMG, 2>(L, src, true, im); }
       if (LD::RELOAD && sl == 2) __syncthreads();
       if (active) {
         TT<KB> z;
@@ -462,6 +477,11 @@
 static int g_h2_tpw = 0;
 void tok_h2_debug_tpw(int tpw) { g_h2_tpw = tpw; }
 static int h2_tpw(long ntile) { (void)ntile; return g_h2_tpw ? g_h2_tpw : 4; }
+static H2Img h2_img(const void* const* img) {
+  H2Img im = {{nullptr, nullptr, nullptr}};
+  if (img && img[0] && img[1] && img[2]) { im.m[0] = img[0]; im.m[1] = img[1]; im.m[2] = img[2]; }
+  return im;
+}
 static unsigned h2_grid(int C, long ntile, int tpw, int max_wg) {
   const long wg = (ntile + tpw - 1) / tpw;
   const long cap = max_wg > 0 ? max_wg : (C > 64 ? 256 : 768);
@@ -474,53 +494,67 @@
     if (int rc = lds_opt_in(KERN, lds)) return rc;                                                                  \
     hipLaunchKernelGGL(KERN, dim3(h2_grid(KC, ntile, KT, max_wg)), dim3(64 * KT), lds, s, __VA_ARGS__);             \
   } while (0)
-#define AFD_H2_SWITCH(BODY)                                                                                         \
+#define AFD_H2_WAVES(KR, ...) { constexpr int KT = KI ? KR : (KC == 128 ? 4 : (KR == 1 ? 2 : KR)); __VA_ARGS__; }
+#define AFD_H2_SWITCH_W(...)                                                                                        \
+  if (tpw == 4) AFD_H2_WAVES(4, __VA_ARGS__) else if (tpw == 2) AFD_H2_WAVES(2, __VA_ARGS__) else AFD_H2_WAVES(1, __VA_ARGS__)
+#define AFD_H2_SWITCH_CT(...)                                                                                       \
   do {                                                                                                              \
-    if (C == 64) { constexpr int KC = 64; if (tpw == 4) { constexpr int KT = 4; BODY; } else { constexpr int KT = 2; BODY; } } \
-    else         { constexpr int KC = 128; constexpr int KT = 4; BODY; }                                             \
+    if (C == 64) { constexpr int KC = 64; AFD_H2_SWITCH_W(__VA_ARGS__) }                                            \
+    else         { constexpr int KC = 128; AFD_H2_SWITCH_W(__VA_ARGS__) }                                           \
   } while (0)
+#define AFD_H2_SWITCH(...)                                                                                          \
+  do {                                                                                                              \
+    if (im.m[0]) { constexpr bool KI = true; AFD_H2_SWITCH_CT(__VA_ARGS__); } else { constexpr bool KI = false; AFD_H2_SWITCH_CT(__VA_ARGS__); } \
+  } while (0)
 
 int tok_h2_head_fwd(const float* x, const float* gamma, const float* beta, const float* w, const float* bias, float* h_out,
-                    float* stats_out, float* qkv, int B, int C, int P, float eps, int max_wg, hipStream_t s) {
+                    float* stats_out, float* qkv, int B, int C, int P, float eps, int max_wg, const void* const* img, hipStream_t s) {
+  const H2Img im = h2_img(img);
   const long ntile = ((long)B * P + 31) / 32;
   const int tpw = h2_tpw(ntile);
-  AFD_H2_SWITCH(AFD_H2_LAUNCH((tok_h2_head_fwd_k<KC, KT>), 5, x, gamma, beta, w, bias, h_out, stats_out, qkv, B, P, eps));
+  AFD_H2_SWITCH(AFD_H2_LAUNCH((tok_h2_head_fwd_k<KC, KT, KI>), 5, x, gamma, beta, w, bias, h_out, stats_out, qkv, B, P, eps, im));
   return check_launch("afd_tok_head_fwd");
 }
 
 int tok_h2_tail_fwd(const float* att, const float* x, const float* wo, const float* bo, const float* gamma, const float* beta,
                     const float* w1, const float* b1, const float* w2, const float* b2, float* a_out, float* stats_out,
-                    float* f_out, float* u_out, float* g_out, float* out, int B, int C, int P, float eps, int max_wg, hipStream_t s) {
+                    float* f_out, float* u_out, float* g_out, float* out, int B, int C, int P, float eps, int max_wg, const void* const* img, hipStream_t s) {
+  const H2Img im = h2_img(img);
   const long ntile = ((long)B * P + 31) / 32;
   const int tpw = h2_tpw(ntile);
   if (a_out)
-    AFD_H2_SWITCH(AFD_H2_LAUNCH((tok_h2_tail_fwd_k<KC, KT, true>), 5, att, x, wo, bo, gamma, beta, w1, b1, w2, b2, a_out, stats_out,
-                                f_out, u_out, g_out, out, B, P, eps));
+    AFD_H2_SWITCH(AFD_H2_LAUNCH((tok_h2_tail_fwd_k<KC, KT, KI, true>), 5, att, x, wo, bo, gamma, beta, w1, b1, w2, b2, a_out, stats_out,
+                                f_out, u_out, g_out, out, B, P, eps, im));
   else
-    AFD_H2_SWITCH(AFD_H2_LAUNCH((tok_h2_tail_fwd_k<KC, KT, false>), 5, att, x, wo, bo, gamma, beta, w1, b1, w2, b2, a_out, stats_out,
-                                f_out, u_out, g_out, out, B, P, eps));
+    AFD_H2_SWITCH(AFD_H2_LAUNCH((tok_h2_tail_fwd_k<KC, KT, KI, false>), 5, att, x, wo, bo, gamma, beta, w1, b1, w2, b2, a_out, stats_out,
+                                f_out, u_out, g_out, out, B, P, eps, im));
   return check_launch("afd_tok_tail_fwd");
 }
 
 int tok_h2_tail_bwd(const float* d_out, const float* u, const float* a, const float* stats, const float* gamma, const float* w2,
                     const float* w1, const float* wo, float* du_out, float* df_out, float* da_out, float* datt_out, int B, int C,
-                    int P, int max_wg, hipStream_t s) {
+                    int P, int max_wg, const void* const* img, hipStream_t s) {
+  const H2Img im = h2_img(img);
   const long ntile = ((long)B * P + 31) / 32;
   const int tpw = h2_tpw(ntile);
-  AFD_H2_SWITCH(AFD_H2_LAUNCH((tok_h2_tail_bwd_k<KC, KT>), 1, d_out, u, a, stats, gamma, w2, w1, wo, du_out, df_out, da_out, datt_out,
-                              B, P));
+  AFD_H2_SWITCH(AFD_H2_LAUNCH((tok_h2_tail_bwd_k<KC, KT, KI>), 1, d_out, u, a, stats, gamma, w2, w1, wo, du_out, df_out, da_out, datt_out,
+                              B, P, im));
   return check_launch("afd_tok_tail_bwd");
 }
 
 int tok_h2_head_bwd(const float* dqkv, const float* x, const float* stats, const float* gamma, const float* w_in,
-                    const float* d_res, float* dh_out, float* dx_out, int B, int C, int P, int max_wg, hipStream_t s) {
+                    const float* d_res, float* dh_out, float* dx_out, int B, int C, int P, int max_wg, const void* const* img, hipStream_t s) {
+  const H2Img im = h2_img(img);
   const long ntile = ((long)B * P + 31) / 32;
   const int tpw = h2_tpw(ntile);
-  AFD_H2_SWITCH(AFD_H2_LAUNCH((tok_h2_head_bwd_k<KC, KT>), 1, dqkv, x, stats, gamma, w_in, d_res, dh_out, dx_out, B, P));
+  AFD_H2_SWITCH(AFD_H2_LAUNCH((tok_h2_head_bwd_k<KC, KT, KI>), 1, dqkv, x, stats, gamma, w_in, d_res, dh_out, dx_out, B, P, im));
   return check_launch("afd_tok_head_bwd");
 }
 
 #undef AFD_H2_SWITCH
+#undef AFD_H2_SWITCH_CT
+#undef AFD_H2_SWITCH_W
+#undef AFD_H2_WAVES
 #undef AFD_H2_LAUNCH
 
 }
diff --git a/aliasfree-diffusion-models-pytorch_amd/csrc/tok_image.h b/aliasfree-diffusion-models-pytorch_amd/csrc/tok_image.h
--- /dev/null
+++ b/aliasfree-diffusion-models-pytorch_amd/csrc/tok_image.h
@@ -0,0 +1,60 @@
+#pragma once
+#include "h2_common.h"
+
+namespace afd {
+
+constexpr int kTokImageKind = 8;
+
+struct WSrc { const float* w; int ldw, n0, k0; };
+
+__host__ __device__ constexpr size_t tok_image_records(int C) { return (size_t)2 * (C / 8) * C; }
+__host__ __device__ constexpr size_t tok_image_bytes(int C) { return tok_image_records(C) * 16 + (size_t)C * 4; }
+
+__device__ __forceinline__ void timg_load8(const WSrc& q, bool transposed, int n, int G, float (&x)[8]) {
+  const int kb = 16 * (G >> 1) + 4 * (G & 1);
+#pragma unroll
+  for (int e = 0; e < 8; ++e) {
+    const int k = kb + 8 * (e >> 2) + (e & 3);
+    x[e] = transposed ? q.w[(long)(q.k0 + k) * q.ldw + q.n0 + n] : q.w[(long)(q.n0 + n) * q.ldw + q.k0 + k];
+  }
+}
+__device__ __forceinline__ float timg_max8(const float (&x)[8]) {
+  float m = 0.f;
+#pragma unroll
+  for (int e = 0; e < 8; ++e) m = fmaxf(m, fabsf(x[e]));
+  return m;
+}
+__device__ __forceinline__ void timg_put(h8* __restrict__ img, int C, int n, int G, const float (&x)[8], float sc) {
+  h8 p0, p1;
+  h2_split8(x, sc, p0, p1);
+  img[G * C + n] = p0;
+  img[(C / 8 + G) * C + n] = p1;
+}
+__device__ __forceinline__ float* timg_winv(void* img, int C) {
+  return reinterpret_cast<float*>(static_cast<h8*>(img) + tok_image_records(C));
+}
+
+__device__ __forceinline__ void timg_scale_rows(const float* __restrict__ w, void* If, void* It, int C, int wi, int nw, int lane) {
+  const int nf = If ? C : 0, nt = It ? C : 0;
+  for (int r = wi; r < nf + nt; r += nw) {
+    const bool fwd = r < nf;
+    const int n = fwd ? r : r - nf;
+    float m = 0.f;
+    for (int k = lane; k < C; k += 64) m = fmaxf(m, fabsf(fwd ? w[(long)n * C + k] : w[(long)k * C + n]));
+    m = wave_amax(m);
+    if (lane == 0) timg_winv(fwd ? If : It, C)[n] = h2_inv_pow2(h2_scale_for(m));
+  }
+}
+__device__ __forceinline__ void timg_build_record(const float* __restrict__ w, void* If, void* It, int C, int idx) {
+  const int pairs = C * (C / 8);
+  const bool transposed = idx >= pairs;
+  const int i = transposed ? idx - pairs : idx;
+  void* img = transposed ? It : If;
+  if (i >= pairs || !img) return;
+  const int n = i % C, G = i / C;
+  float x[8];
+  timg_load8(WSrc{w, C, 0, 0}, transposed, n, G, x);
+  timg_put(static_cast<h8*>(img), C, n, G, x, h2_inv_pow2(timg_winv(img, C)[n]));
+}
+
+}
diff --git a/aliasfree-diffusion-models-pytorch_amd/csrc/wino.hip b/aliasfree-diffusion-models-pytorch_amd/csrc/wino.hip
--- a/aliasfree-diffusion-models-pytorch_amd/csrc/wino.hip
+++ b/aliasfree-diffusion-models-pytorch_amd/csrc/wino.hip
@@ -2,6 +2,7 @@
 #include "conv_forms.h"
 #include "bf3_weights.h"
 #include "h2_common.h"
+#include "tok_image.h"
 
 namespace afd {
 
@@ -82,6 +83,10 @@
 
 __global__ __launch_bounds__(256) void wino_weights_batched(const afd_wino_desc* __restrict__ descs, const int* __restrict__ wg_desc) {
   const afd_wino_desc d = descs[wg_desc[blockIdx.x]];
+  if (d.kinds & kTokImageKind) {
+    timg_build_record(d.w, d.u_fwd, d.u_dgrad, d.Cin, (blockIdx.x - d.first_wg) * 256 + threadIdx.x);
+    return;
+  }
   const int blk = (blockIdx.x - d.first_wg) * 4 + (threadIdx.x >> 6), lane = threadIdx.x & 63;
   float* wf = (d.kinds & 1) ? nullptr : d.u_fwd; float* wd = (d.kinds & 2) ? nullptr : d.u_dgrad;
   if (wf || wd) wino_weights_block(d.w, wf, wd, d.Cin, d.Cout, blk, lane);
@@ -93,9 +98,13 @@
 }
 __global__ __launch_bounds__(256) void h2_wscale_batched(const afd_wino_desc* __restrict__ descs, const int* __restrict__ wg_desc) {
   const afd_wino_desc d = descs[wg_desc[blockIdx.x]];
+  const int nw = 4 * ((d.Cin * d.Cout / 64 + 3) / 4);
+  if (d.kinds & kTokImageKind) {
+    timg_scale_rows(d.w, d.u_fwd, d.u_dgrad, d.Cin, (blockIdx.x - d.first_wg) * 4 + (threadIdx.x >> 6), nw, threadIdx.x & 63);
+    return;
+  }
   if (d.kinds & 4) return;
   void* bf = (d.kinds & 1) ? d.u_fwd : nullptr; void* bd = (d.kinds & 2) ? d.u_dgrad : nullptr;
-  const int nw = 4 * ((d.Cin * d.Cout / 64 + 3) / 4);
   if (bf || bd) h2_wscale_rows(d.w, bf, bd, d.Cin, d.Cout, (blockIdx.x - d.first_wg) * 4 + (threadIdx.x >> 6), nw, threadIdx.x & 63);
 }
 
diff --git a/aliasfree-diffusion-models-pytorch_amd/ops.py b/aliasfree-diffusion-models-pytorch_amd/ops.py
--- a/aliasfree-diffusion-models-pytorch_amd/ops.py
+++ b/aliasfree-diffusion-models-pytorch_amd/ops.py
@@ -442,6 +442,9 @@
     return direct | (kinds & 4 if direct else 0)
 
 
+TOK_IMAGE_KIND = 8
+
+
 class _WinoWeights:
     epoch = 0
     store = {}
@@ -477,6 +480,18 @@
                 pass
         return u, 0
 
+    @classmethod
+    def tok(cls, w, nbytes, dgrad):
+        plan = cls.active_plan
+        if plan is not None:
+            u = plan.lookup(w, nbytes, dgrad, TOK_IMAGE_KIND)
+            if u is not None:
+                return u
+        if cls.recording is not None:
+            rec = cls.recording.setdefault(id(w), [w, 0, 0, TOK_IMAGE_KIND])
+            rec[1 + dgrad] = nbytes
+        return None
+
 
 class WinoStepPlan:
 
@@ -487,18 +502,25 @@
         if not self.ok:
             return
         dev = reqs[0][0].device
-        self.buf = torch.empty(sum(r[1] + r[2] for r in reqs) // 4, device=dev, dtype=torch.float32)
+        up = lambda n: (n // 4 + 3) // 4 * 4
+        self.buf = torch.empty(sum(up(r[1]) + up(r[2]) for r in reqs), device=dev, dtype=torch.float32)
         self.map, descs, wg, off = {}, b"", [], 0
-        for i, (w, nf, nd, kinds) in enumerate(reqs):
+        n_desc = 0
+        for w, nf, nd, kinds in reqs:
             Cout, Cin = w.shape[0], w.shape[1]
             uf = self.buf[off:off + nf // 4] if nf else None
-            off += nf // 4
+            off += up(nf)
             ud = self.buf[off:off + nd // 4] if nd else None
-            off += nd // 4
+            off += up(nd)
             self.map[id(w)] = (weakref.ref(w), w.data_ptr(), uf, ud, kinds)
+            slabs = Cout // Cin if kinds == TOK_IMAGE_KIND else 1
+            Cout //= slabs
             n_wg = (Cin * Cout // 64 + 3) // 4
-            descs += struct.pack("<QQQiiii", w.data_ptr(), uf.data_ptr() if nf else 0, ud.data_ptr() if nd else 0, Cin, Cout, len(wg), kinds)
-            wg += [i] * n_wg
+            for s in range(slabs):
+                descs += struct.pack("<QQQiiii", w.data_ptr() + 4 * s * Cin * Cout, uf.data_ptr() + s * nf // slabs if nf else 0,
+                                     ud.data_ptr() + s * nd // slabs if nd else 0, Cin, Cout, len(wg), kinds)
+                wg += [n_desc] * n_wg
+                n_desc += 1
         self.n_wg = len(wg)
         self.descs = torch.frombuffer(bytearray(descs), dtype=torch.uint8).to(dev)
         self.wg = torch.tensor(wg, dtype=torch.int32).to(dev)
@@ -512,6 +534,8 @@
     def lookup(self, w, nbytes, dgrad, kinds=0):
         e = self.map.get(id(w))
         if e is None or e[0]() is not w or _kind_of(e[4], dgrad) != _kind_of(kinds, dgrad):
+            return None
+        if (e[4] == TOK_IMAGE_KIND) != (kinds == TOK_IMAGE_KIND):
             return None
         u = e[3] if dgrad else e[2]
         return u if (u is not None and u.numel() * 4 == nbytes) else None
@@ -684,6 +708,21 @@
         return dqkv, None
 
 
+def _tok_images(ws, B, C, P, kern):
+    n = lib().afd_tok_image_bytes(B, C, P, kern)
+    out = []
+    for w in ws if n else ():
+        slabs = w.shape[0] // C
+        u = _WinoWeights.tok(w, n * slabs, 1 if kern >= 2 else 0)
+        if u is not None:
+            out += [u.data_ptr() + s * n for s in range(slabs)]
+    return out if len(out) == 3 else [None, None, None]
+
+
+def tok_image_bytes(C):
+    return 2 * (C // 8) * C * 16 + 4 * C
+
+
 def tok_supported(C):
     return bool(lib().afd_tok_supported(int(C)))
 
@@ -744,9 +783,11 @@
         qkv = torch.empty(B, 3 * C, H, W, device=x.device, dtype=torch.float32)
         h = torch.empty_like(x) if train else None
         stats = torch.empty(B, H * W, 2, device=x.device, dtype=torch.float32) if train else None
-        lib().afd_tok_head_fwd(_p(x), _p(gamma), _p(beta), _p(w_in), _p(b_in), _p(h), _p(stats), _p(qkv), B, C, H * W, LN_EPS, _stream())
+        lib().afd_tok_head_fwd_img(_p(x), _p(gamma), _p(beta), _p(w_in), _p(b_in), _p(h), _p(stats), _p(qkv), B, C, H * W, LN_EPS,
+                                   *_tok_images((w_in,), B, C, H * W, 0), _stream())
         ctx.save_for_backward(x, h, stats, gamma, w_in)
         ctx.params = (beta, b_in)
+        ctx.img_bwd = _tok_images((w_in,), B, C, H * W, 3) if train else None
         return qkv, x.view_as(x)
 
     @staticmethod
@@ -760,7 +801,8 @@
         dres = _c(dres)
         dx = torch.empty_like(x)
         dh = torch.empty_like(x)
-        lib().afd_tok_head_bwd(_p(dqkv), _p(x), _p(stats), _p(gamma), _p(w_in), _p(dres), _p(dh), _p(dx), B, C, H * W, _stream())
+        lib().afd_tok_head_bwd_img(_p(dqkv), _p(x), _p(stats), _p(gamma), _p(w_in), _p(dres), _p(dh), _p(dx), B, C, H * W,
+                                   *ctx.img_bwd, _stream())
         dw, db = _linear_grads(h, dqkv, w_in, b_in, B, C, 3 * C, H, W)
         dgamma, dbeta = _ln_param_grads(x, dh, stats, gamma, beta, B, C, H * W)
         return dx, dgamma, dbeta, dw, db
@@ -779,10 +821,12 @@
             stats = torch.empty(B, H * W, 2, device=att.device, dtype=torch.float32)
         else:
             a = f = u = g = stats = None
-        lib().afd_tok_tail_fwd(_p(att), _p(x), _p(wo), _p(bo), _p(gamma), _p(beta), _p(w1), _p(b1), _p(w2), _p(b2),
-                               _p(a), _p(stats), _p(f), _p(u), _p(g), _p(out), B, C, H * W, LN_EPS, _stream())
+        lib().afd_tok_tail_fwd_img(_p(att), _p(x), _p(wo), _p(bo), _p(gamma), _p(beta), _p(w1), _p(b1), _p(w2), _p(b2),
+                                   _p(a), _p(stats), _p(f), _p(u), _p(g), _p(out), B, C, H * W, LN_EPS,
+                                   *_tok_images((wo, w1, w2), B, C, H * W, 1), _stream())
         ctx.save_for_backward(att, a, stats, f, u, g, gamma, wo, w1, w2)
         ctx.params = (bo, beta, b1, b2)
+        ctx.img_bwd = _tok_images((w2, w1, wo), B, C, H * W, 2) if a is not None else None
         return out
 
     @staticmethod
@@ -792,8 +836,8 @@
         B, C, H, W = att.shape
         dout = _c(dout)
         du, df, da, datt = (torch.empty_like(att) for _ in range(4))
-        lib().afd_tok_tail_bwd(_p(dout), _p(u), _p(a), _p(stats), _p(gamma), _p(w2), _p(w1), _p(wo),
-                               _p(du), _p(df), _p(da), _p(datt), B, C, H * W, _stream())
+        lib().afd_tok_tail_bwd_img(_p(dout), _p(u), _p(a), _p(stats), _p(gamma), _p(w2), _p(w1), _p(wo),
+                                   _p(du), _p(df), _p(da), _p(datt), B, C, H * W, *ctx.img_bwd, _stream())
         dw2, db2 = _linear_grads(g, dout, w2, b2, B, C, C, H, W)
         dw1, db1 = _linear_grads(f, du, w1, b1, B, C, C, H, W)
         dwo, dbo = _linear_grads(att, da, wo, bo, B, C, C, H, W)
diff --git a/include/afd.h b/include/afd.h
--- a/include/afd.h
+++ b/include/afd.h
@@ -137,6 +137,22 @@
                      float* du_out, float* df_out, float* da_out, float* datt_out, int B, int C, int P, afd_stream_t stream);
 int afd_tok_head_bwd(const float* dqkv, const float* x, const float* stats, const float* gamma, const float* w_in,
                      const float* d_res, float* dh_out, float* dx_out, int B, int C, int P, afd_stream_t stream);
+size_t afd_tok_image_bytes(int B, int C, int P, int kern);
+int afd_debug_tok_images(int on);
+int afd_tok_head_fwd_img(const float* x, const float* gamma, const float* beta, const float* w_in, const float* b_in,
+                         float* h_out, float* stats_out, float* qkv, int B, int C, int P, float eps,
+                         const void* img_q, const void* img_k, const void* img_v, afd_stream_t stream);
+int afd_tok_tail_fwd_img(const float* att, const float* x, const float* w_o, const float* b_o, const float* gamma, const float* beta,
+                         const float* w_1, const float* b_1, const float* w_2, const float* b_2,
+                         float* a_out, float* stats_out, float* f_out, float* u_out, float* g_out, float* out,
+                         int B, int C, int P, float eps, const void* img_o, const void* img_1, const void* img_2, afd_stream_t stream);
+int afd_tok_tail_bwd_img(const float* d_out, const float* u, const float* a, const float* stats, const float* gamma,
+                         const float* w_2, const float* w_1, const float* w_o,
+                         float* du_out, float* df_out, float* da_out, float* datt_out, int B, int C, int P,
+                         const void* img_2t, const void* img_1t, const void* img_ot, afd_stream_t stream);
+int afd_tok_head_bwd_img(const float* dqkv, const float* x, const float* stats, const float* gamma, const float* w_in,
+                         const float* d_res, float* dh_out, float* dx_out, int B, int C, int P,
+                         const void* img_qt, const void* img_kt, const void* img_vt, afd_stream_t stream);
 
 int afd_gelu_fwd(const float* x, float* y, long n, afd_stream_t stream);
 int afd_gelu_bwd(const float* x, const float* dy, float* dx, long n, afd_stream_t stream);
```

Result: no change. 41050 images/s (median of 6 runs) (+0.2%).
